# AlgoLab/PIntron

Measured on AMD Instinct MI355X. Metric: ESTs aligned/sec (whole node) + DP Mcells/s; bit-exact factorizations vs ref, higher is better.
Workload: dtype u8/int32

## Files before the change

### pintron_amd/estfact.py

```python
import ctypes as C
import os

ROOT = os.path.dirname(os.path.dirname(os.path.abspath(__file__)))
OUTPUT_FILES = ("raw-multifasta-out.txt", "processed-ests.txt", "megs.txt", "processed-megs.txt",
                "processed-megs-info.txt", "meg-edges.txt")


class KernelStat(C.Structure):
    _fields_ = [("name", C.c_char * 48), ("ms", C.c_double), ("launches", C.c_size_t),
                ("jobs", C.c_size_t), ("cells", C.c_ulonglong), ("algo_bytes", C.c_ulonglong)]


class SchedStats(C.Structure):
    _fields_ = [(n, C.c_size_t) for n in ("threads", "units", "aligned", "dp_batches", "dp_jobs",
                                          "pairing_batches", "pairing_requests")] + \
               [(n, C.c_double) for n in ("load_s", "index_s", "prefetch_s", "workers_s", "host_s",
                                          "pairing_s", "dp_s")] + \
               [("n_kernels", C.c_int), ("kernels", KernelStat * 64), ("dp_busy_union_ms", C.c_double),
                ("suspensions_per_unit", C.c_double)]


def load_host_lib(path=None):
    path = path or os.environ.get("PINTRON_ESTFACT_LIB") or os.path.join(ROOT, "pintron_amd", "lib", "libestfact.so")
    if not os.path.exists(path):
        raise RuntimeError("%s missing: run __graft_entry__.build() (there is no CPU fallback)" % path)
    L = C.CDLL(path)
    L.ef_session_open.restype = C.c_void_p
    L.ef_session_open.argtypes = [C.c_int, C.POINTER(C.c_char_p)]
    L.ef_session_step.argtypes = [C.c_void_p, C.POINTER(SchedStats)]
    L.ef_session_output.restype = C.c_void_p
    L.ef_session_output.argtypes = [C.c_void_p, C.c_int, C.POINTER(C.c_size_t)]
    L.ef_session_n_ests.restype = C.c_size_t
    L.ef_session_n_ests.argtypes = [C.c_void_p]
    L.ef_session_write_outputs.argtypes = [C.c_void_p]
    L.ef_session_close.argtypes = [C.c_void_p]
    return L


class Session:

    def __init__(self, L, directory):
        self.L, self.dir = L, directory
        cwd = os.getcwd()
        os.chdir(directory)
        try:
            argv = (C.c_char_p * 2)(b"est-fact", None)
            self.h = L.ef_session_open(1, argv)
        finally:
            os.chdir(cwd)
        if not self.h:
            raise RuntimeError("est-fact session could not start (no MI355X / libpintron_gpu.so?)")

    def step(self) -> SchedStats:
        st = SchedStats()
        if self.L.ef_session_step(self.h, C.byref(st)) != 0:
            raise RuntimeError("est-fact step failed")
        return st

    def n_ests(self) -> int:
        return int(self.L.ef_session_n_ests(self.h))

    def output(self, which: int) -> bytes:
        n = C.c_size_t()
        p = self.L.ef_session_output(self.h, which, C.byref(n))
        data = C.string_at(p, n.value)
        C.CDLL(None).free(C.c_void_p(p))
        return data

    def records(self) -> bytes:
        return self.output(0)

    def output_tensor(self, which: int):
        import torch
        n = C.c_size_t()
        p = self.L.ef_session_output(self.h, which, C.byref(n))
        try:
            if n.value == 0:
                return torch.empty(0, dtype=torch.uint8)
            view = (C.c_ubyte * n.value).from_address(p)
            return torch.frombuffer(view, dtype=torch.uint8).clone()
        finally:
            C.CDLL(None).free(C.c_void_p(p))

    def close(self):
        if self.h:
            self.L.ef_session_close(self.h)
            self.h = None


RECORDS = 6


def parse_factorization_records(data: bytes):
    import struct
    out, pos = [], 0
    while pos < len(data):
        est_index, n_fact = struct.unpack_from("<II", data, pos)
        pos += 8
        facts = []
        for _ in range(n_fact):
            polya, polyad, n_exons = struct.unpack_from("<BBH", data, pos)
            pos += 4
            exons = [struct.unpack_from("<4i", data, pos + 16 * k) for k in range(n_exons)]
            pos += 16 * n_exons
            facts.append((polya, polyad, exons))
        out.append((est_index, facts))
    return out


def format_raw_multifasta(records, processed_ests: bytes, genomic_seq: bytes) -> bytes:
    ests = []
    lines = processed_ests.split(b"\n")
    for k in range(0, len(lines) - 1, 2):
        ests.append((lines[k][1:], lines[k + 1]))
    out = []
    for (est_index, facts), (header, seq) in zip(records, ests):
        for polya, polyad, exons in facts:
            out.append(b">" + header + b"\n#polya=%d\n#polyad=%d\n" % (polya, polyad))
            for es, ee, gs, ge in exons:
                out.append(b"%d %d %d %d %s %s\n" % (es, ee, gs, ge, seq[es - 1:ee], genomic_seq[gs - 1:ge]))
    return b"".join(out)


def read_multifasta_records(path):
    recs, cur = [], []
    with open(path, "rb") as f:
        for line in f:
            if line.startswith(b">") and cur:
                recs.append(b"".join(cur))
                cur = []
            if line.strip() or cur:
                cur.append(line)
    if cur:
        recs.append(b"".join(cur))
    return recs


def partition(weights, world):
    total, n = sum(weights), len(weights)
    bounds, acc, i = [0], 0, 0
    for r in range(1, world):
        while i < n and acc * world < total * r:
            acc += weights[i]
            i += 1
        bounds.append(i)
    bounds.append(n)
    return [(bounds[r], bounds[r + 1]) for r in range(world)]


def gather_tensor(t, dist, rank, world, device):
    import torch
    n = torch.tensor([t.numel()], dtype=torch.int64, device=device)
    sizes = [torch.zeros_like(n) for _ in range(world)]
    dist.all_gather(sizes, n)
    sizes = [int(s.item()) for s in sizes]
    pad = torch.empty(max(max(sizes), 1), dtype=torch.uint8, device=device)
    pad[: t.numel()] = t.to(device)
    outl = [torch.empty_like(pad) for _ in range(world)] if rank == 0 else None
    dist.gather(pad, outl, dst=0)
    if rank != 0:
        return None
    return [o[: sizes[r]] for r, o in enumerate(outl)]


def gather_bytes(data: bytes, dist, rank, world, device):
    import torch
    t = torch.frombuffer(bytearray(data), dtype=torch.uint8) if data else torch.empty(0, dtype=torch.uint8)
    parts = gather_tensor(t, dist, rank, world, device)
    if parts is None:
        return None
    return [bytes(o.cpu().numpy().tobytes()) for o in parts]


def run_sharded(directory, workdir, dist, rank, world, device, L=None, files=(0, 1)):
    import shutil
    L = L or load_host_lib()
    recs = read_multifasta_records(os.path.join(directory, "ests.txt"))
    lo, hi = partition([len(r) for r in recs], world)[rank]
    os.makedirs(workdir, exist_ok=True)
    shutil.copy(os.path.join(directory, "genomic.txt"), os.path.join(workdir, "genomic.txt"))
    if os.path.exists(os.path.join(directory, "config.ini")):
        shutil.copy(os.path.join(directory, "config.ini"), os.path.join(workdir, "config.ini"))
    with open(os.path.join(workdir, "ests.txt"), "wb") as f:
        f.write(b"".join(recs[lo:hi]))
    texts = {k: b"" for k in files}
    stats = {"ests": 0, "aligned": 0, "dp_jobs": 0}
    error = None
    if hi > lo:
        try:
            sess = Session(L, workdir)
            try:
                st = sess.step()
                for k in files:
                    texts[k] = sess.output(k)
                stats = {"ests": hi - lo, "aligned": int(st.aligned), "dp_jobs": int(st.dp_jobs)}
            finally:
                sess.close()
        except Exception as e:
            error = e
    import torch
    ok = torch.tensor([0 if error else 1], dtype=torch.int32, device=device)
    dist.all_reduce(ok, op=dist.ReduceOp.MIN)
    if int(ok.item()) == 0:
        raise RuntimeError("est-fact failed on rank %d: %s" % (rank, error) if error
                           else "est-fact failed on another rank")
    for k in files:
        parts = gather_bytes(texts[k], dist, rank, world, device)
        if rank == 0:
            with open(os.path.join(directory, OUTPUT_FILES[k]), "wb") as f:
                f.write(b"".join(parts))
    return stats
```

### pintron_amd/host/ef_fact.c

```c
#include <math.h>
#include <stdlib.h>
#include <string.h>

#include "estfact.h"

typedef struct { int p, t, l; } ptl;

static size_t view_len(const char* s, int index, int length) {
  if (length <= 0) return 0;
  const char* z = (const char*)memchr(s + index, 0, (size_t)length);
  return z ? (size_t)(z - (s + index)) : (size_t)length;
}

char* ef_real_substring(int index, int length, const char* s) {
  if (index < 0) { length += index; index = 0; }
  if (length < 0) length = 0;
  char* r = (char*)malloc((size_t)length + 1);
  strncpy(r, s + index, (size_t)length);
  r[length] = '\0';
  return r;
}

static ef_factor* factor_new(int es, int ee, int gs, int ge) {
  ef_factor* f = (ef_factor*)malloc(sizeof(ef_factor));
  f->EST_start = es; f->EST_end = ee; f->GEN_start = gs; f->GEN_end = ge;
  return f;
}

void ef_factorization_free(void* fact) { efl_free((ef_list*)fact, free); }

void ef_est_free(ef_est* e) {
  if (!e) return;
  efl_free(e->factorizations, ef_factorization_free);
  efl_free(e->polyA_signals, NULL);
  efl_free(e->polyadenil_signals, NULL);
  free(e);
}

static void ahead_note(ef_ahead* ah, const ef_dp_req* q) {
  for (int k = 0; k < ah->n_pending; ++k) if (ef_req_same(&ah->q[ah->n + k], q)) return;
  if (ah->n + ah->n_pending < EF_AHEAD_MAX) ah->q[ah->n + ah->n_pending++] = *q;
}

int ef_dp_many_ahead(ef_backend* be, const ef_dp_req* reqs, ef_dp_res* res, size_t n) {
  ef_ahead* ah = be->ahead;
  enum { CAP = 32 };
  if (n > CAP) return ah->collecting ? EF_DP_PENDING : ef_backend_ask(be, reqs, res, n);
  size_t miss[CAP], nm = 0;
  for (size_t k = 0; k < n; ++k) {
    const int32_t* v = ef_ahead_find(ah, &reqs[k]);
    if (v) memcpy(res[k].v, v, sizeof res[k].v);
    else miss[nm++] = k;
  }
  if (ef_prof_on) { ef_prof.ahead_hits += n - nm; ef_prof.ahead_misses += ah->collecting ? 0 : nm; }
  if (nm == 0) return 0;
  if (ah->collecting) {
    for (size_t k = 0; k < nm; ++k) if (ef_req_keepable(&reqs[miss[k]])) ahead_note(ah, &reqs[miss[k]]);
    return EF_DP_PENDING;
  }
  if (nm == n) return ef_backend_ask(be, reqs, res, n);
  ef_dp_req mq[CAP]; ef_dp_res mr[CAP];
  for (size_t k = 0; k < nm; ++k) mq[k] = reqs[miss[k]];
  memset(mr, 0, nm * sizeof(ef_dp_res));
  const int rc = ef_backend_ask(be, mq, mr, nm);
  if (rc != 0) return rc;
  for (size_t k = 0; k < nm; ++k) res[miss[k]] = mr[k];
  return 0;
}

int ef_ahead_flush(ef_backend* be) {
  ef_ahead* ah = be->ahead;
  if (!ah || ah->n_pending == 0) return 0;
  const bool was = ah->collecting;
  ah->collecting = false;
  const int np = ah->n_pending;
  ef_dp_res r[EF_AHEAD_MAX];
  memset(r, 0, (size_t)np * sizeof(ef_dp_res));
  const int rc = ef_backend_ask(be, ah->q + ah->n, r, (size_t)np);
  if (rc == 0)
    for (int k = 0; k < np; ++k) ef_ahead_keep_next(ah, r[k].v);
  if (ef_prof_on) ef_prof.ahead_asked += (unsigned long long)np;
  ah->n_pending = 0;
  ah->collecting = was;
  return rc;
}

static int run_dp(ef_backend* be, int kind, const char* a, size_t la, const char* b, size_t lb,
                  uint32_t p0, uint32_t p1, uint32_t p2, uint32_t tail, bool temp, ef_dp_res* res) {
  ef_dp_req rq = { kind, a, la, b, lb, p0, p1, p2, tail, temp ? 1u : 0u };
  const int rc = ef_dp_one(be, &rq, res);
  if (rc != 0 && rc != EF_DP_PENDING) {
    fprintf(stderr, "* FATAL dynamic-programming backend failed (kind %d, %zu x %zu)\n", kind, la, lb);
    abort();
  }
  return rc;
}

uint32_t ef_edit_distance(ef_backend* be, const char* a, size_t la, const char* b, size_t lb) {
  ef_dp_res r;
  run_dp(be, EF_DP_ED, a, la, b, lb, 0, 0, 0, 0, true, &r);
  return (uint32_t)r.v[0];
}

uint32_t ef_compute_edit_distance(ef_backend* be, const char* a, size_t la, const char* b, size_t lb) {
  if (la == lb && strncmp(a, b, la) == 0) return 0;
  return ef_edit_distance(be, a, la, b, lb);
}

typedef struct { uint32_t n; ptl e[]; } emb;
static emb* emb_new(uint32_t n) { emb* x = (emb*)malloc(sizeof(emb) + (size_t)n * sizeof(ptl)); x->n = n; return x; }
static void embedding_free(void* e) { free(e); }

static emb* embedding_copy(const emb* e) {
  emb* c = emb_new(e->n);
  memcpy(c->e, e->e, (size_t)e->n * sizeof(ptl));
  return c;
}

static emb* update_embedding(const emb* embedding, const ef_pairing* node, const char* GEN,
                             const ef_config* cfg) {
  const ptl* head = &embedding->e[0];
  if (head->p == EF_SINK_START) {
    if (node->p < 0) return NULL;
    emb* e = emb_new(1);
    e->e[0].p = node->p; e->e[0].t = node->t; e->e[0].l = node->l;
    return e;
  }
  if (node->p < 0) return embedding_copy(embedding);
  const int small_delta = (head->p + head->l) - node->p;
  const int big_delta = (head->t + head->l) - node->t;
  const int min_fl = (int)cfg->min_factor_len;
  const int fl = 2 * min_fl;
  if (!(small_delta >= fl && big_delta >= fl)) return NULL;
  if (!(small_delta - (node->l + head->l) <= fl)) return NULL;
  if (!(small_delta - big_delta <= fl)) return NULL;
  int head_l, head_p, head_t, node_l;
  if (small_delta >= (node->l + head->l) && big_delta >= (node->l + head->l)) {
    head_p = head->p; head_t = head->t; head_l = head->l; node_l = node->l;
  } else {
    const int ref_delta = small_delta < big_delta ? small_delta : big_delta;
    int len_node = ref_delta / 2;
    int len_head = ref_delta - len_node;
    if (len_node > node->l) { len_node = node->l; len_head = ref_delta - len_node; }
    else if (len_head > head->l) { len_head = head->l; len_node = ref_delta - len_head; }
    head_l = len_head;
    head_p = head->p + head->l - head_l;
    head_t = head->t + head->l - head_l;
    node_l = len_node;
  }
  const bool overlap_on_p = small_delta < (node->l + head->l);
  const int gap_on_p = head_p - node->p - node_l - 1;
  const int gap_on_t = head_t - node->t - node_l - 1;
  const int intron_len = gap_on_t - (gap_on_p > 0 ? gap_on_p : 0);
  const bool intron_on_t = intron_len >= 0 && (cfg->min_intron_length == 0 || intron_len >= cfg->min_intron_length);
  if (overlap_on_p && intron_on_t) {
    int best_freq = -1, best_cut = 0;
    const int lo = (node->p + min_fl > head->p) ? node->p + min_fl : head->p;
    const int hi = (head->p + head->l - min_fl < node->p + node->l) ? head->p + head->l - min_fl : node->p + node->l;
    for (int cut = lo; cut <= hi; ++cut) {
      const int f = ef_burset_adaptor(GEN, (size_t)(cut - node->p + node->t), (size_t)(cut - head->p + head->t));
      if (f >= best_freq) { best_freq = f; best_cut = cut; }
    }
    const int dH = best_cut - head->p;
    head_l = head->l - dH; head_p = head->p + dH; head_t = head->t + dH;
    node_l = node->l - (node->p + node->l - best_cut);
  }
  if (!(gap_on_t <= fl || intron_on_t)) return NULL;
  emb* c = emb_new(embedding->n + 1);
  c->e[0].p = node->p; c->e[0].t = node->t; c->e[0].l = node_l;
  c->e[1].p = head_p; c->e[1].t = head_t; c->e[1].l = head_l;
  memcpy(c->e + 2, embedding->e + 1, (size_t)(embedding->n - 1) * sizeof(ptl));
  return c;
}

static bool pair_inside(const ptl* inner, const ptl* outer) {
  if (inner->p < outer->p || (inner->p + inner->l > outer->p + outer->l)) return false;
  if (inner->t < outer->t || (inner->t + inner->l > outer->t + outer->l)) return false;
  return true;
}

static int maximality_relation(const emb* add, const emb* cmp) {
  if (add->n > cmp->n) {
    bool check = true;
    for (uint32_t i = 0; i < cmp->n && check; ++i) check = pair_inside(&cmp->e[i], &add->e[i]);
    return check ? 2 : 1;
  }
  if (add->n < cmp->n) {
    bool check = true;
    for (uint32_t i = 0; i < add->n && check; ++i) check = pair_inside(&add->e[i], &cmp->e[i]);
    return check ? 0 : 1;
  }
  bool check = true;
  for (uint32_t i = 0; i < add->n && check; ++i) check = pair_inside(&add->e[i], &cmp->e[i]);
  if (check) return 0;
  check = true;
  for (uint32_t i = 0; i < add->n && check; ++i) check = pair_inside(&cmp->e[i], &add->e[i]);
  return check ? 2 : 1;
}

#define EF_WORK_PER_SECOND 1000000ull
typedef struct { unsigned long long used, limit; } ef_work;
static unsigned long long work_high_water;
unsigned long long ef_work_high_water(void) { return __atomic_load_n(&work_high_water, __ATOMIC_RELAXED); }
extern unsigned long long ef_work_budget_override;
static unsigned long long work_limit(const ef_config* cfg) {
  if (ef_work_budget_override) return ef_work_budget_override;
  return cfg->max_single_factorization_time ? (unsigned long long)cfg->max_single_factorization_time * EF_WORK_PER_SECOND : ~0ull;
}

static ef_list* subtree_embeddings(ef_pairing* root, const ef_config* cfg, const char* GEN, ef_work* wk) {
  if (root->emb_memo) return root->emb_memo;
  if (++wk->used > wk->limit) return NULL;
  ef_list* out = efl_new();
  root->visited = true;
  if (efl_empty(root->adjs)) {
    emb* e = emb_new(1);
    e->e[0].p = root->p; e->e[0].t = root->t; e->e[0].l = root->l;
    efl_push_front(out, e);
  } else {
    ef_iter ai = efl_begin(root->adjs);
    while (efi_has_next(&ai)) {
      ef_pairing* adj = (ef_pairing*)efi_next(&ai);
      ef_list* sub = subtree_embeddings(adj, cfg, GEN, wk);
      if (!sub) { efl_free(out, embedding_free); return NULL; }
      ef_iter si = efl_begin(sub);
      while (efi_has_next(&si)) {
        emb* add = update_embedding((const emb*)efi_next(&si), root, GEN, cfg);
        if (!add) continue;
        if (++wk->used > wk->limit) { embedding_free(add); efl_free(out, embedding_free); return NULL; }
        int is_max = 2;
        ef_iter ci = efl_begin(out);
        while (efi_has_next(&ci) && is_max >= 1) {
          const emb* cmp = (const emb*)efi_next(&ci);
          is_max = maximality_relation(add, cmp);
          if (is_max == 2) efi_remove(&ci, embedding_free);
        }
        if (is_max >= 1) efl_push_back(out, add); else embedding_free(add);
      }
    }
  }
  root->emb_memo = out;
  return out;
}

static ef_list* factorizations_from_embeddings(ef_list* embeddings, const ef_config* cfg) {
  ef_list* out = efl_new();
  const int fl = 2 * (int)cfg->min_factor_len;
  ef_iter ei = efl_begin(embeddings);
  while (efi_has_next(&ei)) {
    const emb* em = (const emb*)efi_next(&ei);
    ef_list* fact = efl_new();
    ef_factor* last = NULL;
    for (uint32_t q = 0; q < em->n; ++q) {
      const ptl* x = &em->e[q];
      if (efl_empty(fact) || (x->t - last->GEN_end - 1) > fl) {
        last = factor_new(x->p, x->p + x->l - 1, x->t, x->t + x->l - 1);
        efl_push_back(fact, last);
      } else {
        last = (ef_factor*)efl_tail(fact);
        last->EST_end = x->p + x->l - 1;
        last->GEN_end = x->t + x->l - 1;
      }
    }
    efl_push_back(out, fact);
  }
  return out;
}

static bool not_source_sink(ef_list* fact, int est_len) {
  if (efl_size(fact) > 1) return true;
  const ef_factor* h = (const ef_factor*)efl_head(fact);
  return !(h->EST_start < 0 || h->EST_start >= est_len);
}

static bool exon_start_end_ok(ef_list* fact) {
  int prev_e = -1, prev_g = -1;
  ef_iter it = efl_begin(fact);
  while (efi_has_next(&it)) {
    const ef_factor* x = (const ef_factor*)efi_next(&it);
    if (x->EST_start > x->EST_end || x->GEN_start > x->GEN_end) return false;
    if (x->EST_start < prev_e || x->GEN_start < prev_g) return false;
    prev_e = x->EST_end; prev_g = x->GEN_end;
  }
  return true;
}

static void endpoint_head_apply(ef_list* fact, ef_factor* head, const ef_dp_res* r) {
  const char* ea = r->s0; const char* ga = r->s1;
  const int dim = r->v[1];
  int j = 0, matches = 0, cut_factor = head->EST_start, cut_exon = head->GEN_start;
  bool stop = false;
  while (j < dim && !stop) {
    if (matches > 5) stop = true;
    else {
      if (ea[j] == ga[j]) { ++cut_factor; ++cut_exon; ++matches; }
      else { if (ea[j] != '-') ++cut_factor; if (ga[j] != '-') ++cut_exon; matches = 0; }
      ++j;
    }
  }
  if (!stop) free(efl_pop_front(fact));
  else { head->EST_start = cut_factor - matches; head->GEN_start = cut_exon - matches; }
}

static void endpoint_tail_apply(ef_list* fact, ef_factor* tail, const ef_dp_res* r) {
  char* ea = r->s0; char* ga = r->s1;
  const int dim = r->v[1];
  int j = dim - 1, matches = 0, cut_factor = tail->EST_end, cut_exon = tail->GEN_end;
  bool stop = false;
  while (j >= 0 && !stop) {
    if (matches > 10) stop = true;
    else {
      if (ea[j] == ga[j]) { --cut_factor; --cut_exon; ++matches; }
      else { if (ea[j] != '-') --cut_factor; if (ga[j] != '-') --cut_exon; matches = 0; }
      --j;
    }
  }
  int est_cleavage = cut_factor + matches, gen_cleavage = cut_exon + matches;
  int cursor = j + matches + 1;
  stop = false;
  while (((ea[cursor] == '-' || ga[cursor] == '-') && cursor < dim - 1) && !stop) {
    if (ea[cursor] == '-') {
      int tr = cursor + 1;
      while (ea[tr] == '-') ++tr;
      if (tr < dim && ea[tr] == ga[cursor]) { ea[cursor] = ea[tr]; ea[tr] = '-'; ++est_cleavage; ++gen_cleavage; }
      else stop = true;
    } else {
      int tr = cursor + 1;
      while (ga[tr] == '-') ++tr;
      if (tr < dim && ga[tr] == ea[cursor]) { ga[cursor] = ga[tr]; ga[tr] = '-'; ++est_cleavage; ++gen_cleavage; }
      else stop = true;
    }
    ++cursor;
  }
  if (gen_cleavage >= tail->GEN_start) { tail->EST_end = est_cleavage; tail->GEN_end = gen_cleavage; }
  else free(efl_pop_back(fact));
}

static void endpoint_request(ef_dp_req* q, const ef_factor* x, const char* gen, const char* est) {
  const ef_dp_req r = { EF_DP_ALIGN, est + x->EST_start, view_len(est, x->EST_start, x->EST_end - x->EST_start + 1),
                        gen + x->GEN_start, view_len(gen, x->GEN_start, x->GEN_end - x->GEN_start + 1), 0, 0, 0, 0, 0 };
  *q = r;
}
static void endpoint_release(ef_dp_req* q, ef_dp_res* r) {
  (void)q;
  ef_dp_res_release(r);
}

static unsigned max_edit_for_exon(size_t exon_length);
static bool exon_check_request(ef_dp_req* q, const ef_factor* x, const char* gen, const char* est, const ef_config* cfg) {
  if (x->GEN_start > x->GEN_end) return false;
  uint32_t w[2];
  memcpy(w, &cfg->complexity_threshold, 8);
  const ef_dp_req r = { EF_DP_KBAND, gen + x->GEN_start, view_len(gen, x->GEN_start, x->GEN_end - x->GEN_start + 1),
                        est + x->EST_start, view_len(est, x->EST_start, x->EST_end - x->EST_start + 1),
                        max_edit_for_exon((size_t)(x->GEN_end - x->GEN_start + 1)), w[0], w[1], 1, 0 };
  *q = r;
  return true;
}

static ef_list* handle_endpoints(ef_list* fact, const char* gen, const char* est, const ef_config* cfg, ef_backend* be) {
  ef_factor* head = (ef_factor*)efl_head(fact);
  ef_dp_req q[2]; ef_dp_res r[2];
  if (efl_size(fact) >= 2) {
    ef_factor* tail = (ef_factor*)efl_tail(fact);
    enum { INNER_MAX = 22 };
    ef_dp_req qq[2 + INNER_MAX]; ef_dp_res rr[2 + INNER_MAX]; size_t nq = 2;
    endpoint_request(&qq[0], head, gen, est);
    endpoint_request(&qq[1], tail, gen, est);
    if (be->ahead && ef_endpoint_checks) {
      uint32_t w[2];
      memcpy(w, &cfg->complexity_threshold, 8);
      qq[0].p0 = 1; qq[0].p1 = w[0]; qq[0].p2 = w[1];
      qq[1].p0 = 2; qq[1].p1 = w[0]; qq[1].p2 = w[1];
    }
    if (be->ahead && efl_size(fact) >= 3 && efl_size(fact) <= INNER_MAX) {
      ef_iter it = efl_begin(fact);
      efi_next(&it);
      while (efi_has_next(&it)) {
        const ef_factor* x = (const ef_factor*)efi_next(&it);
        if (x == tail) break;
        if (exon_check_request(&qq[nq], x, gen, est, cfg)) ++nq;
      }
    }
    if (ef_dp_many(be, qq, rr, nq) != 0) { fprintf(stderr, "* FATAL alignment backend failed\n"); abort(); }
    for (size_t k = 2; k < nq; ++k) ef_ahead_put(be->ahead, &qq[k], rr[k].v);
    if (be->ahead) {
      for (int k = 0; k < 2; ++k) {
        const int32_t* v = rr[k].v;
        if (!(v[4] & 8)) continue;
        const ef_factor* x = k == 0 ? head : tail;
        ef_factor y = *x;
        if (k == 0) { y.EST_start += v[2]; y.GEN_start += v[3]; }
        else { y.EST_end = y.EST_start + v[2] - 1; y.GEN_end = y.GEN_start + v[3] - 1; }
        ef_dp_req cq;
        if (y.EST_start > y.EST_end || !exon_check_request(&cq, &y, gen, est, cfg) || cq.p0 != ((uint32_t)v[4] >> 8)) continue;
        if (cq.la != (size_t)(y.GEN_end - y.GEN_start + 1) || cq.lb != (size_t)(y.EST_end - y.EST_start + 1)) continue;
        const int32_t answer[6] = { v[4] & 1, 0, (v[4] >> 1) & 3, 0, 0, 0 };
        ef_ahead_put(be->ahead, &cq, answer);
        if (ef_prof_on) ++ef_prof.ahead_asked;
      }
    }
    endpoint_head_apply(fact, head, &rr[0]);
    endpoint_tail_apply(fact, tail, &rr[1]);
    endpoint_release(&qq[0], &rr[0]); endpoint_release(&qq[1], &rr[1]);
    return fact;
  }
  endpoint_request(&q[0], head, gen, est);
  if (ef_dp_many(be, q, r, 1) != 0) { fprintf(stderr, "* FATAL alignment backend failed\n"); abort(); }
  endpoint_head_apply(fact, head, &r[0]);
  endpoint_release(&q[0], &r[0]);
  if (efl_empty(fact)) return fact;
  ef_factor* tail = (ef_factor*)efl_tail(fact);
  endpoint_request(&q[0], tail, gen, est);
  if (ef_dp_many(be, q, r, 1) != 0) { fprintf(stderr, "* FATAL alignment backend failed\n"); abort(); }
  endpoint_tail_apply(fact, tail, &r[0]);
  endpoint_release(&q[0], &r[0]);
  return fact;
}

static bool is_ch(char c, char up) { return c == up || c == (char)(up + 32); }

ef_list* ef_clean_external_exons(ef_list* fact, const char* gen, const char* est, ef_backend* be) {
  if (efl_empty(fact)) return fact;
  ef_factor* head = (ef_factor*)efl_pop_front(fact);
  const int hl = head->GEN_end - head->GEN_start + 1;
  bool ok = hl >= 10;
  if (ok && hl < 20) {
    if (!is_ch(gen[head->GEN_end + 1], 'G')) ok = false;
    else if (!is_ch(gen[head->GEN_end + 2], 'T') && !is_ch(gen[head->GEN_end + 2], 'C')) ok = false;
    else if (efl_size(fact) >= 1) {
      const ef_factor* nx = (const ef_factor*)efl_head(fact);
      if (!is_ch(gen[nx->GEN_start - 2], 'A')) ok = false;
      else if (!is_ch(gen[nx->GEN_start - 1], 'G')) ok = false;
    } else ok = false;
    if (ok) {
      char* g = ef_real_substring(head->GEN_start, head->GEN_end - head->GEN_start + 1, gen);
      char* e = ef_real_substring(head->EST_start, head->EST_end - head->EST_start + 1, est);
      if ((int)ef_edit_distance(be, g, strlen(g), e, strlen(e)) > 0) ok = false;
      free(g); free(e);
    }
  }
  if (ok) efl_push_front(fact, head); else free(head);
  if (efl_empty(fact)) return fact;
  ef_factor* tail = (ef_factor*)efl_pop_back(fact);
  const int tl = tail->GEN_end - tail->GEN_start + 1;
  ok = tl >= 10;
  if (ok && tl < 20) {
    if (!is_ch(gen[tail->GEN_start - 2], 'A')) ok = false;
    else if (!is_ch(gen[tail->GEN_start - 1], 'G')) ok = false;
    else if (efl_size(fact) >= 1) {
      const ef_factor* pv = (const ef_factor*)efl_tail(fact);
      if (!is_ch(gen[pv->GEN_end + 1], 'G')) ok = false;
      else if (!is_ch(gen[pv->GEN_end + 2], 'T') && !is_ch(gen[pv->GEN_end + 2], 'C')) ok = false;
    } else ok = false;
    if (ok) {
      char* g = ef_real_substring(tail->GEN_start, tail->GEN_end - tail->GEN_start + 1, gen);
      char* e = ef_real_substring(tail->EST_start, tail->EST_end - tail->EST_start + 1, est);
      if ((int)ef_edit_distance(be, g, strlen(g), e, strlen(e)) > 0) ok = false;
      free(g); free(e);
    }
  }
  if (ok) efl_push_back(fact, tail); else free(tail);
  return fact;
}

static ef_list* keep_best_run(ef_list* fact, const int* split_idx, int n_split) {
  if (n_split == 0) return fact;
  int best_l = -1, best_r = -1, best_cover = -1;
  ef_iter fi = efl_begin(fact);
  int left = 1;
  for (int k = 0; k < n_split; ++k) {
    const int right = split_idx[k];
    const ef_factor* le = (const ef_factor*)efi_next(&fi);
    const ef_factor* re = le;
    if (left < right) {
      for (int times = right - left - 1; times > 0; --times) re = (const ef_factor*)efi_next(&fi);
      const int cover = re->EST_end - le->EST_start + 1;
      if (cover > best_cover) { best_l = left; best_r = right - 1; best_cover = cover; }
      efi_next(&fi);
    }
    left = right + 1;
  }
  const int size = (int)efl_size(fact);
  if (left <= size) {
    const ef_factor* le = (const ef_factor*)efi_next(&fi);
    const ef_factor* re = le;
    for (int times = size - left; times > 0; --times) re = (const ef_factor*)efi_next(&fi);
    const int cover = re->EST_end - le->EST_start + 1;
    if (cover > best_cover) { best_l = left; best_r = size; best_cover = cover; }
  }
  if (best_l == -1 || best_r == -1) {
    for (int k = size; k > 0; --k) free(efl_pop_back(fact));
  } else {
    for (int k = best_l - 1; k > 0; --k) free(efl_pop_front(fact));
    for (int k = best_r + 1; k <= size; ++k) free(efl_pop_back(fact));
  }
  return fact;
}

static unsigned max_edit_for_exon(size_t exon_length) {
  const double rate = exon_length > 100 ? 0.030 : (exon_length > 50 ? 0.035 : 0.040);
  const double c = ceil(exon_length * rate);
  return (unsigned)(c > 1.0 ? c : 1.0);
}

ef_list* ef_clean_noisy_exons(ef_list* fact, const char* gen, const char* est, bool only_internals, ef_backend* be) {
  const size_t size = efl_size(fact);
  enum { SMALL = 24 };
  int idx_small[SMALL], slot_small[SMALL]; ef_dp_req rq_small[SMALL]; ef_dp_res rs_small[SMALL];
  const bool small = size < SMALL;
  int* idx = small ? idx_small : (int*)malloc((size + 1) * sizeof(int));
  ef_dp_req* rq = small ? rq_small : (ef_dp_req*)malloc((size + 1) * sizeof(ef_dp_req));
  ef_dp_res* rs = small ? rs_small : (ef_dp_res*)malloc((size + 1) * sizeof(ef_dp_res));
  int* slot = small ? slot_small : (int*)malloc((size + 1) * sizeof(int));
  size_t nrq = 0, nvis = 0;
  int index = only_internals ? 2 : 1;
  const int first_index = index;
  const int last = only_internals ? (int)(size - 1) : (int)size;
  ef_iter it = efl_begin(fact);
  if (only_internals) efi_next(&it);
  while (efi_has_next(&it) && index <= last) {
    const ef_factor* x = (const ef_factor*)efi_next(&it);
    const unsigned max_err = max_edit_for_exon((size_t)(x->GEN_end - x->GEN_start + 1));
    slot[nvis] = -1;
    if (x->GEN_start <= x->GEN_end) {
      const ef_dp_req q = { EF_DP_KBAND, gen + x->GEN_start, view_len(gen, x->GEN_start, x->GEN_end - x->GEN_start + 1),
                            est + x->EST_start, view_len(est, x->EST_start, x->EST_end - x->EST_start + 1), max_err, 0, 0, 0, 0 };
      slot[nvis] = (int)nrq;
      rq[nrq++] = q;
    }
    ++nvis; ++index;
  }
  if (ef_dp_many(be, rq, rs, nrq) != 0) { fprintf(stderr, "* FATAL dynamic-programming backend failed (K-band)\n"); abort(); }
  int n = 0;
  for (size_t v = 0; v < nvis; ++v) {
    const bool ok = slot[v] >= 0 && rs[slot[v]].v[0] != 0;
    if (!ok) idx[n++] = first_index + (int)v;
  }
  fact = keep_best_run(fact, idx, n);
  if (!small) { free(idx); free(rq); free(rs); free(slot); }
  return fact;
}

static bool est_coverage_ok(ef_list* fact, const char* est) {
  const size_t len = strlen(est);
  const ef_factor* h = (const ef_factor*)efl_head(fact);
  const ef_factor* t = (const ef_factor*)efl_tail(fact);
  const double cov = (double)(t->EST_end - h->EST_start + 1) / (double)len;
  return cov >= 0.35f;
}

static int relaxed_factor_compare(const ef_factor* p1, const ef_factor* p2, int cfr_type, int allowed, ef_list* l1) {
  if (p1->GEN_start < p2->GEN_start && p1->GEN_end < p2->GEN_start) return 1;
  if (p2->GEN_start < p1->GEN_start && p2->GEN_end < p1->GEN_start) return 1;
  const int max_unconf = 20;
  if (cfr_type == 0) {
    if (abs(p1->GEN_end - p2->GEN_end) <= allowed && abs(p1->GEN_start - p2->GEN_start) <= allowed) return 0;
  }
  if (abs(cfr_type) == 2) {
    if (abs(p1->GEN_end - p2->GEN_end) <= allowed) {
      if (cfr_type == 2) {
        if (p1->GEN_start - p2->GEN_start > max_unconf) return 1;
        if (p1->GEN_start - p2->GEN_start > 0) {
          int tot = 0; bool stop = false;
          ef_iter it = efl_begin(l1);
          while (efi_has_next(&it) && !stop) {
            const ef_factor* f = (const ef_factor*)efi_next(&it);
            if (p1->GEN_start == f->GEN_start) stop = true; else tot += f->GEN_end - f->GEN_start + 1;
          }
          if (abs(p1->GEN_start - p2->GEN_start - tot) < 10) return 1;
        }
      }
      return 0;
    }
  }
  if (abs(cfr_type) == 1) {
    if (abs(p1->GEN_start - p2->GEN_start) <= allowed) {
      if (cfr_type == 1) {
        if (p2->GEN_end - p1->GEN_end > max_unconf) return 1;
        if (p2->GEN_end - p1->GEN_end > 0) {
          int tot = 0; bool stop = false;
          ef_iter it = efl_end(l1);
          while (efi_has_prev(&it) && !stop) {
            const ef_factor* f = (const ef_factor*)efi_prev(&it);
            if (p1->GEN_start == f->GEN_start) stop = true; else tot += f->GEN_end - f->GEN_start + 1;
          }
          if (abs(p2->GEN_end - p1->GEN_end - tot) < 20) return 1;
        }
      }
      return 0;
    }
  }
  return 1;
}

static int relaxed_list_compare(ef_list* l1, ef_list* l2, int allowed_diff) {
  if (efl_size(l1) != efl_size(l2) || efl_size(l1) == 1) return 0;
  ef_iter i1 = efl_begin(l1), i2 = efl_begin(l2);
  const int actual = allowed_diff == -1 ? 0 : allowed_diff;
  int count = 1;
  while (efi_has_next(&i1) && efi_has_next(&i2)) {
    const int type = allowed_diff == -1 ? 0 : (count == 1 ? -2 : (count == (int)efl_size(l1) ? -1 : 0));
    if (relaxed_factor_compare((const ef_factor*)i1.next->el, (const ef_factor*)i2.next->el, type, actual, l1) != 0) return 0;
    efi_next(&i1); efi_next(&i2);
    ++count;
  }
  return -2;
}

static int relaxed_list_contained(ef_list* l1, ef_list* l2, int allowed_diff) {
  if (efl_size(l1) == efl_size(l2)) return relaxed_list_compare(l1, l2, allowed_diff);
  if (efl_size(l1) == 1 || efl_size(l2) == 1) return 0;
  const int actual = allowed_diff == -1 ? 0 : allowed_diff;
  ef_iter i1 = efl_begin(l1), i2 = efl_begin(l2);
  bool found = false;
  int type = allowed_diff == -1 ? 0 : -2;
  unsigned count_long = 1;
  const bool l1_longer = efl_size(l1) > efl_size(l2);
  ef_list* lng = l1_longer ? l1 : l2;
  ef_iter* il = l1_longer ? &i1 : &i2;
  ef_iter* is = l1_longer ? &i2 : &i1;
  while (efi_has_next(il) && !found) {
    if (relaxed_factor_compare((const ef_factor*)il->next->el, (const ef_factor*)is->next->el, type, actual, lng) == 0) { found = true; efi_next(is); }
    else ++count_long;
    efi_next(il);
    if (type == -2) type = 2;
  }
  if (!found) return 0;
  unsigned count_factors = 1;
  bool stop = false;
  const size_t short_size = l1_longer ? efl_size(l2) : efl_size(l1);
  const size_t long_size = l1_longer ? efl_size(l1) : efl_size(l2);
  while (efi_has_next(&i1) && efi_has_next(&i2) && !stop) {
    type = allowed_diff == -1 ? 0 : ((count_factors + 1 == short_size) ? ((count_long + 1 == long_size) ? -1 : 1) : 0);
    if (relaxed_factor_compare((const ef_factor*)il->next->el, (const ef_factor*)is->next->el, type, actual, lng) == 0) { efi_next(&i1); efi_next(&i2); }
    else stop = true;
    ++count_factors; ++count_long;
  }
  if (stop) return 0;
  if (efl_size(l1) >= efl_size(l2)) return count_factors == efl_size(l2) ? 1 : 0;
  return count_factors == efl_size(l1) ? -1 : 0;
}

ef_list* ef_add_if_not_exists(ef_list* to_add, ef_list* list, const ef_config* cfg, bool* added) {
  ef_iter ci = efl_begin(list);
  bool found = false;
  while (efi_has_next(&ci) && !found) {
    ef_list* cmp = (ef_list*)efi_next(&ci);
    int res = 0;
    if (efl_size(cmp) == efl_size(to_add) && efl_size(cmp) == 1) {
      const ef_factor* h1 = (const ef_factor*)efl_head(to_add); const ef_factor* h2 = (const ef_factor*)efl_head(cmp);
      if (h1->GEN_start == h2->GEN_start && h1->GEN_end == h2->GEN_end) res = -2;
      else if (h1->GEN_start >= h2->GEN_start && h1->GEN_end <= h2->GEN_end) res = -1;
      else if (h1->GEN_start <= h2->GEN_start && h1->GEN_end >= h2->GEN_end) res = 1;
    } else {
      res = relaxed_list_contained(to_add, cmp, (int)cfg->max_site_difference);
    }
    if (res < 0) {
      if (res == -2) {
        const ef_factor* h1 = (const ef_factor*)efl_head(to_add); ef_factor* h2 = (ef_factor*)efl_head(cmp);
        if (h1->EST_start < h2->EST_start) { h2->EST_start = h1->EST_start; h2->GEN_start = h1->GEN_start; }
        const ef_factor* t1 = (const ef_factor*)efl_tail(to_add); ef_factor* t2 = (ef_factor*)efl_tail(cmp);
        if (t1->EST_end > t2->EST_end) { t2->EST_end = t1->EST_end; t2->GEN_end = t1->GEN_end; }
      }
      found = true;
    } else if (res == 1) {
      efi_remove(&ci, ef_factorization_free);
    }
  }
  if (!found) efl_push_back(list, to_add);
  *added = !found;
  return list;
}

static double coverage_of(ef_list* fact, unsigned length) {
  const ef_factor* h = (const ef_factor*)efl_head(fact); const ef_factor* t = (const ef_factor*)efl_tail(fact);
  const int cover = (int)length - (h->EST_start + ((int)length - t->EST_end - 1));
  return ((double)cover) / (double)length;
}

static int gap_length_of(ef_list* fact) {
  if (efl_size(fact) == 1) return 0;
  int g = 0;
  ef_iter it = efl_begin(fact);
  const ef_factor* d = (const ef_factor*)efi_next(&it);
  while (efi_has_next(&it)) { const ef_factor* a = (const ef_factor*)efi_next(&it); g += a->EST_start - d->EST_end - 1; d = a; }
  return g;
}

static bool check_gap_errors(ef_list* fact, const char* est, const char* gen, const ef_config* cfg, ef_backend* be) {
  (void)cfg;
  const unsigned threshold_ed = 20;
  unsigned tot = 0;
  bool ok = true;
  ef_iter it = efl_begin(fact);
  ef_factor* d = (ef_factor*)efi_next(&it);
  while (efi_has_next(&it) && ok) {
    ef_factor* a = (ef_factor*)efi_next(&it);
    const size_t gapP = (size_t)(a->EST_start - d->EST_end - 1);
    if (gapP > 0) {
      const size_t gapT = (size_t)(a->GEN_start - d->GEN_end - 1);
      const int max_errs = (int)gapP;
      char *pc = NULL, *tc = NULL;
      const char* p = est + d->EST_end + 1;
      const char* t = gen + d->GEN_end + 1;
      if (d->EST_end + 1 < 0 || view_len(est, d->EST_end + 1, (int)gapP) != gapP) p = pc = ef_real_substring(d->EST_end + 1, (int)gapP, est);
      if (d->GEN_end + 1 < 0 || (int)gapT < 0 || (size_t)(d->GEN_end + 1) + gapT > ef_genomic_len(gen)) t = tc = ef_real_substring(d->GEN_end + 1, (int)gapT, gen);
      ef_dp_res r;
      const int asked = run_dp(be, EF_DP_BORDERS, p, gapP, t, gapT, 0, (uint32_t)gapP, (uint32_t)max_errs, 0, pc || tc, &r);
      free(pc); free(tc);
      if (asked == EF_DP_PENDING) { d = a; continue; }
      if (ef_collecting(be)) { d = a; continue; }
      ok = r.v[0] != 0;
      if (ok) {
        tot += (unsigned)r.v[4];
        d->EST_end += r.v[1];
        a->EST_start = d->EST_end + 1;
        d->GEN_end += r.v[2];
        a->GEN_start -= (int)gapT - r.v[3];
      }
    }
    d = a;
  }
  if (ef_collecting(be)) return true;
  if (ok && tot > threshold_ed) ok = false;
  if (ok) {
    it = efl_begin(fact);
    d = (ef_factor*)efi_next(&it);
    while (efi_has_next(&it)) {
      ef_factor* a = (ef_factor*)efi_next(&it);
      if (a->GEN_start - d->GEN_end - 1 <= 3) { d->EST_end = a->EST_end; d->GEN_end = a->GEN_end; efi_remove(&it, free); }
      else d = a;
    }
  }
  return ok;
}

static void correct_tail(ef_list* fact, const char* gen, const char* est) {
  ef_factor* tail = (ef_factor*)efl_tail(fact);
  size_t i = (size_t)(tail->EST_end + 1), j = (size_t)(tail->GEN_end + 1);
  const size_t el = strlen(est), gl = ef_genomic_len(gen);
  while (i < el && j < gl && gen[j] == est[i]) { ++i; ++j; }
  tail->EST_end = (int)i - 1; tail->GEN_end = (int)j - 1;
}

static bool detect_polyA(ef_list* fact, const char* gen, const char* est, bool* polyadenil) {
  const ef_factor* tail = (const ef_factor*)efl_tail(fact);
  const size_t el = strlen(est);
  const char* cl = est + tail->EST_end + 1;
  const int cll = (tail->EST_end + 1 <= (int)el) ? (int)(el - (size_t)tail->EST_end - 1) : 0;
  int i = 0, matches = 0;
  bool stop = false;
  while (i < cll && !stop) {
    if (cl[i] == 'a' || cl[i] == 'A') { if (matches >= 8) stop = true; else { ++matches; ++i; } }
    else { if (matches >= 8) stop = true; else i = cll; }
  }
  *polyadenil = false;
  if (stop) {
    i = tail->GEN_end - 39 > 0 ? tail->GEN_end - 39 : 0;
    while (i <= tail->GEN_end && !*polyadenil) {
      if (gen[i] == 'a' || gen[i] == 'A') {
        char pas[8];
        const size_t pl = view_len(gen, i, 6);
        memcpy(pas, gen + i, pl); pas[pl] = '\0';
        if (!strcmp(pas, "aataaa") || !strcmp(pas, "AATAAA") || !strcmp(pas, "attaaa") || !strcmp(pas, "ATTAAA")) *polyadenil = true;
      }
      ++i;
    }
    i = tail->GEN_end - 9 > 0 ? tail->GEN_end - 9 : 0;
    matches = 0;
    while (i <= tail->GEN_end + 10 && stop && gen[i] != '\0') {
      if (matches >= 6) stop = false;
      else { if (gen[i] == 'a' || gen[i] == 'A') ++matches; else matches = 0; ++i; }
    }
    if (stop) {
      i = tail->GEN_end + 1;
      int count = 0;
      while (i <= tail->GEN_end + 10 && stop && gen[i] != '\0') {
        if (count >= 7) stop = false;
        else { if (gen[i] == 'a' || gen[i] == 'A') ++count; ++i; }
      }
    }
  }
  return stop;
}

static ef_list* clean_complexity_and_noise(ef_list* fact, const char* gen, const char* est, const ef_config* cfg, ef_backend* be) {
  const size_t size = efl_size(fact);
  enum { SMALL = 24 };
  const ef_factor* x_small[SMALL]; int slot_small[SMALL], idx_small[SMALL]; ef_dp_req rq_small[SMALL]; ef_dp_res rs_small[SMALL];
  const bool small = size < SMALL;
  const ef_factor** xs = small ? x_small : (const ef_factor**)malloc((size + 1) * sizeof(ef_factor*));
  int* slot = small ? slot_small : (int*)malloc((size + 1) * sizeof(int));
  int* idx = small ? idx_small : (int*)malloc((size + 1) * sizeof(int));
  ef_dp_req* rq = small ? rq_small : (ef_dp_req*)malloc((size + 1) * sizeof(ef_dp_req));
  ef_dp_res* rs = small ? rs_small : (ef_dp_res*)malloc((size + 1) * sizeof(ef_dp_res));
  size_t nx = 0, nrq = 0;
  ef_iter it = efl_begin(fact);
  while (efi_has_next(&it)) {
    const ef_factor* x = (const ef_factor*)efi_next(&it);
    xs[nx] = x;
    slot[nx] = exon_check_request(&rq[nrq], x, gen, est, cfg) ? (int)nrq++ : -1;
    ++nx;
  }
  if (ef_dp_many(be, rq, rs, nrq) != 0) { fprintf(stderr, "* FATAL dynamic-programming backend failed (exon checks)\n"); abort(); }
  int n = 0;
  for (size_t v = 0; v < nx; ++v) if (slot[v] >= 0 && rs[slot[v]].v[2] != 0) idx[n++] = (int)v + 1;
  fact = keep_best_run(fact, idx, n);
  if (!efl_empty(fact)) {
    ef_phase(EFP_NOISY);
    n = 0;
    int index = 1;
    size_t v = 0;
    it = efl_begin(fact);
    while (efi_has_next(&it)) {
      const ef_factor* x = (const ef_factor*)efi_next(&it);
      while (v < nx && xs[v] != x) ++v;
      const bool ok = v < nx && slot[v] >= 0 && rs[slot[v]].v[0] != 0;
      if (!ok) idx[n++] = index;
      ++index;
    }
    fact = keep_best_run(fact, idx, n);
  }
  if (!small) { free(xs); free(slot); free(idx); free(rq); free(rs); }
  return fact;
}

static ef_list* clean_candidates(ef_list* cands, ef_list* flist, unsigned est_len, const char* GEN, const char* EST,
                                 const ef_config* cfg, ef_backend* be) {
  ef_iter ci = efl_begin(cands);
  while (efi_has_next(&ci)) {
    ef_list* f = (ef_list*)efi_next(&ci);
    bool ok = not_source_sink(f, (int)est_len);
    if (ok) ok = exon_start_end_ok(f);
    if (ok) { ef_phase(EFP_ENDPOINTS); f = handle_endpoints(f, GEN, EST, cfg, be); if (efl_empty(f)) ok = false; }
    if (ok) { ef_phase(EFP_EXTERNAL); f = ef_clean_external_exons(f, GEN, EST, be); if (efl_empty(f)) ok = false; }
    if (ok) { ef_phase(EFP_DUST); f = clean_complexity_and_noise(f, GEN, EST, cfg, be); if (efl_empty(f)) ok = false; }
    ef_phase(EFP_ADD);
    if (ok) ok = est_coverage_ok(f, EST);
    if (ok) {
      bool added;
      flist = ef_add_if_not_exists(f, flist, cfg, &added);
      if (!added) ef_factorization_free(f);
    } else {
      ef_factorization_free(f);
    }
  }
  efl_free(cands, NULL);
  return flist;
}

static bool chain_embedding(const void* rec, const ef_config* cfg, const char* GEN, ef_work* wk, emb** out) {
  const uint32_t* head = (const uint32_t*)rec;
  const uint32_t nv = head[0];
  if (nv < 2 || nv > 64) return false;
  const int32_t* vt = (const int32_t*)((const char*)rec + 16);
  const uint16_t* first = (const uint16_t*)((const char*)rec + 16 + 12 * (size_t)nv);
  const uint8_t* tgt = (const uint8_t*)rec + 16 + 12 * (size_t)nv + 2 * ((size_t)nv + 1);
  if (vt[0] != EF_SOURCE_START) return false;
  uint8_t path[64];
  uint64_t seen = 0;
  uint32_t k = 0, n = 0;
  for (;;) {
    if (seen >> k & 1u) return false;
    seen |= 1ull << k; path[n++] = (uint8_t)k;
    const uint32_t deg = (uint32_t)first[k + 1] - first[k];
    if (deg == 0) break;
    if (deg != 1) return false;
    k = tgt[first[k]];
    if (k >= nv) return false;
  }
  if (n != nv || vt[3 * (size_t)path[n - 1]] != EF_SINK_START) return false;
  wk->used += nv;
  ef_pairing node;
  memset(&node, 0, sizeof node);
  emb* e = emb_new(1);
  { const int32_t* s3 = vt + 3 * (size_t)path[n - 1]; e->e[0].p = s3[0]; e->e[0].t = s3[1]; e->e[0].l = s3[2]; }
  for (uint32_t q = n - 1; q-- > 0 && e;) {
    const int32_t* v3 = vt + 3 * (size_t)path[q];
    node.p = v3[0]; node.t = v3[1]; node.l = v3[2];
    emb* nx = update_embedding(e, &node, GEN, cfg);
    embedding_free(e);
    e = nx;
    if (e) ++wk->used;
  }
  *out = e;
  return true;
}

unsigned ef_chain_candidate(const void* rec, const ef_config* cfg, const char* GEN, ef_factor* out_exons, size_t cap,
                            unsigned* n_exons, unsigned* n_pairs, unsigned* work) {
  *n_exons = 0; *n_pairs = 0; *work = 0;
  if (((const uint32_t*)rec)[2] & 3u) return 0;
  ef_work wk = { 0, ~0ull };
  emb* chain = NULL;
  if (!chain_embedding(rec, cfg, GEN, &wk, &chain)) return 1;
  *work = (unsigned)wk.used;
  if (!chain) return 2;
  *n_pairs = chain->n;
  ef_list* embs = efl_new();
  efl_push_back(embs, chain);
  ef_list* cands = factorizations_from_embeddings(embs, cfg);
  efl_free(embs, embedding_free);
  ef_list* fact = (ef_list*)efl_head(cands);
  ef_iter it = efl_begin(fact);
  while (efi_has_next(&it)) {
    const ef_factor* x = (const ef_factor*)efi_next(&it);
    if (*n_exons < cap) out_exons[*n_exons] = *x;
    ++*n_exons;
  }
  ef_factorization_free(fact);
  efl_free(cands, NULL);
  return 3;
}

static ef_list* filter_and_refine(ef_list* flist, unsigned est_len, const ef_seq* est_info, const ef_seq* gen_info,
                                  const ef_config* cfg, ef_backend* be) {
  const char* GEN = gen_info->seq;
  const char* EST = est_info->seq;
  ef_phase(EFP_FILTERS);
  {
    const size_t nf = efl_size(flist);
    double cov_small[32];
    double* cov = nf < 32 ? cov_small : (double*)malloc((nf + 1) * sizeof(double));
    double max_cov = 0.0;
    size_t k = 0;
    ef_iter it = efl_begin(flist);
    while (efi_has_next(&it)) {
      ef_list* f = (ef_list*)efi_next(&it);
      bool src_sink = false;
      if (efl_size(f) == 1) {
        const ef_factor* h = (const ef_factor*)efl_head(f);
        if (h->EST_start < 0 || h->EST_start >= (int)est_len) { cov[k] = -1.0; src_sink = true; }
      }
      if (!src_sink) { cov[k] = coverage_of(f, est_len); if (max_cov < cov[k]) max_cov = cov[k]; }
      ++k;
    }
    k = 0;
    it = efl_begin(flist);
    const int slen = (int)strlen(EST);
    while (efi_has_next(&it)) {
      efi_next(&it);
      const double c = cov[k++];
      if (c == -1.0 || max_cov - c > cfg->max_coverage_diff) efi_remove(&it, ef_factorization_free);
      else if ((max_cov - c) * slen > 100) efi_remove(&it, ef_factorization_free);
    }
    if (cov != cov_small) free(cov);
  }
  {
    const size_t nf = efl_size(flist);
    int gl_small[32];
    int* gl = nf < 32 ? gl_small : (int*)malloc((nf + 1) * sizeof(int));
    int min_gl = -1;
    size_t k = 0;
    ef_iter it = efl_begin(flist);
    while (efi_has_next(&it)) {
      gl[k] = gap_length_of((ef_list*)efi_next(&it));
      if (min_gl == -1 || min_gl > gl[k]) min_gl = gl[k];
      ++k;
    }
    k = 0;
    it = efl_begin(flist);
    while (efi_has_next(&it)) {
      efi_next(&it);
      const int g = gl[k++];
      if (cfg->max_gapLength_diff != -1 && g - min_gl > cfg->max_gapLength_diff) efi_remove(&it, ef_factorization_free);
    }
    if (gl != gl_small) free(gl);
  }
  ef_phase(EFP_GAPERR);
  if (be->ahead) {
    ef_ahead_collect(be, true);
    ef_iter it = efl_begin(flist);
    while (efi_has_next(&it)) check_gap_errors((ef_list*)efi_next(&it), EST, GEN, cfg, be);
    ef_ahead_collect(be, false);
    if (ef_ahead_flush(be) != 0) { fprintf(stderr, "* FATAL dynamic-programming backend failed\n"); abort(); }
  }
  {
    ef_iter it = efl_begin(flist);
    while (efi_has_next(&it)) {
      ef_list* f = (ef_list*)efi_next(&it);
      if (!check_gap_errors(f, EST, GEN, cfg, be)) efi_remove(&it, ef_factorization_free);
    }
  }
  if (cfg->max_number_of_factorizations != 0 && (int)efl_size(flist) > cfg->max_number_of_factorizations) {
    efl_free(flist, ef_factorization_free);
    flist = efl_new();
  }
  ef_phase(EFP_INTRON);
  {
    enum { GAP_AHEAD_MAX = 24 };
    ef_gap_ahead* pre = NULL; size_t n_pre = 0;
    if (be->ahead && be->dp_many) {
      size_t total = 0;
      ef_iter it = efl_begin(flist);
      while (efi_has_next(&it)) { const size_t k = efl_size((ef_list*)efi_next(&it)); total += k ? k - 1 : 0; }
      if (total >= 2 && total <= GAP_AHEAD_MAX) {
        pre = (ef_gap_ahead*)malloc(total * sizeof(ef_gap_ahead));
        ef_dp_req rq[GAP_AHEAD_MAX]; ef_dp_res rs[GAP_AHEAD_MAX];
        it = efl_begin(flist);
        while (efi_has_next(&it)) {
          ef_list* f = (ef_list*)efi_next(&it);
          if (efl_empty(f)) continue;
          ef_iter fi = efl_begin(f);
          const ef_factor* donor = (const ef_factor*)efi_next(&fi);
          while (efi_has_next(&fi)) {
            const ef_factor* acc = (const ef_factor*)efi_next(&fi);
            ef_gap_window_build(cfg, gen_info, est_info, donor, acc, &pre[n_pre].w);
            pre[n_pre].donor = *donor; pre[n_pre].acceptor = *acc;
            const ef_dp_req q = { EF_DP_GAP, pre[n_pre].w.seq_est, pre[n_pre].w.le, pre[n_pre].w.seq_gen, pre[n_pre].w.lg, 0, 0, 0, 0, 1 };
            rq[n_pre++] = q;
            donor = acc;
          }
        }
        memset(rs, 0, n_pre * sizeof(ef_dp_res));
        if (be->dp_many(be->self, rq, rs, n_pre) != 0) { fprintf(stderr, "* FATAL gap alignment backend failed\n"); abort(); }
        for (size_t k = 0; k < n_pre; ++k) pre[k].res = rs[k];
        if (ef_prof_on) ef_prof.ahead_asked += n_pre;
      }
    }
    size_t at = 0;
    ef_iter it = efl_begin(flist);
    while (efi_has_next(&it)) {
      ef_list* f = (ef_list*)efi_next(&it);
      if (efl_empty(f)) continue;
      ef_iter fi = efl_begin(f);
      ef_factor* donor = (ef_factor*)efi_next(&fi);
      bool first = true;
      while (efi_has_next(&fi)) {
        ef_factor* acc = (ef_factor*)efi_next(&fi);
        ef_refine_intron(cfg, gen_info, est_info, donor, acc, first, be, pre && at < n_pre ? &pre[at] : NULL);
        ++at;
        first = false;
        donor = acc;
      }
      fi = efl_begin(f);
      const ef_factor* e1 = (const ef_factor*)efi_next(&fi);
      if (efi_has_next(&fi)) {
        const ef_factor* e2 = (const ef_factor*)efi_next(&fi);
        if (e1->EST_start == e2->EST_start) free(efl_pop_front(f));
      }
    }
    for (size_t k = 0; k < n_pre; ++k) { ef_gap_window_release(&pre[k].w); ef_dp_res_release(&pre[k].res); }
    free(pre);
  }
  return flist;
}

unsigned ef_chain_factorization(const void* rec, const ef_config* cfg, const char* EST, const char* GEN, ef_backend* be,
                                ef_factor* out_exons, size_t cap, unsigned* n_exons) {
  *n_exons = 0;
  if (((const uint32_t*)rec)[2] & 3u) return 0;
  ef_work wk = { 0, ~0ull };
  emb* chain = NULL;
  if (!chain_embedding(rec, cfg, GEN, &wk, &chain)) return 0;
  if (!chain) return 1;
  ef_seq est_info, gen_info;
  memset(&est_info, 0, sizeof est_info); memset(&gen_info, 0, sizeof gen_info);
  est_info.seq = est_info.original_seq = (char*)EST;
  gen_info.seq = gen_info.original_seq = (char*)GEN;
  const unsigned est_len = (unsigned)strlen(EST);
  ef_list* embs = efl_new();
  efl_push_back(embs, chain);
  ef_list* cands = factorizations_from_embeddings(embs, cfg);
  efl_free(embs, embedding_free);
  ef_list* flist = clean_candidates(cands, efl_new(), est_len, GEN, EST, cfg, be);
  flist = filter_and_refine(flist, est_len, &est_info, &gen_info, cfg, be);
  unsigned outcome = 1;
  if (!efl_empty(flist)) {
    outcome = 2;
    ef_iter it = efl_begin((ef_list*)efl_head(flist));
    while (efi_has_next(&it)) {
      const ef_factor* x = (const ef_factor*)efi_next(&it);
      if (*n_exons < cap) out_exons[*n_exons] = *x;
      ++*n_exons;
    }
  }
  efl_free(flist, ef_factorization_free);
  return outcome;
}

ef_est* ef_get_est_factorizations(const ef_seq* est_info, ef_meg* V, const ef_config* cfg,
                                  const ef_seq* gen_info, ef_backend* be) {
  ef_phase(EFP_EMBED);
  ef_est* est = (ef_est*)calloc(1, sizeof(ef_est));
  est->info = est_info;
  const char* GEN = gen_info->seq;
  const char* EST = est_info->seq;
  const unsigned est_len = (unsigned)V->n - 2;
  ef_list* flist = efl_new();
  ef_work wk = { 0, work_limit(cfg) };
  emb* chain = NULL;
  if (V->rec && !V->v && ef_chain_fast_path && chain_embedding(V->rec, cfg, GEN, &wk, &chain)) {
    if (ef_prof_on) ++ef_prof.chain_graphs;
    if (wk.used > wk.limit) {
      if (chain) embedding_free(chain);
      efl_free(flist, ef_factorization_free);
      free(est);
      return NULL;
    }
    if (chain) {
      ef_list* embs = efl_new();
      efl_push_back(embs, chain);
      ef_list* cands = factorizations_from_embeddings(embs, cfg);
      efl_free(embs, embedding_free);
      flist = clean_candidates(cands, flist, est_len, GEN, EST, cfg, be);
    }
  } else {
  if (ef_prof_on) ++ef_prof.other_graphs;
  V = ef_meg_lists(V);
  EF_MEG_FOR_POS(V, i, 0, V->n) {
    ef_iter it = efl_begin(V->v[i]);
    while (efi_has_next(&it)) { ef_pairing* p = (ef_pairing*)efi_next(&it); p->visited = false; p->emb_memo = NULL; }
  }
  EF_MEG_FOR_POS(V, i, 0, V->n) {
    ef_iter it = efl_begin(V->v[i]);
    while (efi_has_next(&it)) {
      ef_pairing* root = (ef_pairing*)efi_next(&it);
      if (root->visited) continue;
      ef_phase(EFP_EMBED);
      ef_list* embs = subtree_embeddings(root, cfg, GEN, &wk);
      if (!embs) {
        EF_MEG_FOR_POS(V, j, 0, V->n) {
          ef_iter jt = efl_begin(V->v[j]);
          while (efi_has_next(&jt)) { ef_pairing* q = (ef_pairing*)efi_next(&jt); if (q->emb_memo) { efl_free(q->emb_memo, embedding_free); q->emb_memo = NULL; } }
        }
        efl_free(flist, ef_factorization_free);
        free(est);
        return NULL;
      }
      flist = clean_candidates(factorizations_from_embeddings(embs, cfg), flist, est_len, GEN, EST, cfg, be);
    }
  }
  EF_MEG_FOR_POS(V, i, 0, V->n) {
    ef_iter it = efl_begin(V->v[i]);
    while (efi_has_next(&it)) { ef_pairing* p = (ef_pairing*)efi_next(&it); if (p->emb_memo) { efl_free(p->emb_memo, embedding_free); p->emb_memo = NULL; } }
  }
  }
  {
    unsigned long long hw = __atomic_load_n(&work_high_water, __ATOMIC_RELAXED);
    while (wk.used > hw && !__atomic_compare_exchange_n(&work_high_water, &hw, wk.used, true, __ATOMIC_RELAXED, __ATOMIC_RELAXED)) { }
  }

  flist = filter_and_refine(flist, est_len, est_info, gen_info, cfg, be);
  ef_phase(EFP_TAIL);
  est->polyA_signals = efl_new();
  est->polyadenil_signals = efl_new();
  {
    ef_iter it = efl_begin(flist);
    while (efi_has_next(&it)) {
      ef_list* f = (ef_list*)efi_next(&it);
      correct_tail(f, GEN, est_info->original_seq);
      bool polyadenil = false;
      const bool polyA = detect_polyA(f, GEN, est_info->original_seq, &polyadenil);
      efl_push_back(est->polyA_signals, polyA ? (void*)1 : (void*)2);
      efl_push_back(est->polyadenil_signals, polyadenil ? (void*)1 : (void*)2);
    }
  }
  est->factorizations = flist;
  return est;
}
```

### pintron_amd/host/ef_sched.c

```c
#define _GNU_SOURCE
#include <malloc.h>
#include <pthread.h>
#include <sys/uio.h>
#include <errno.h>
#include <sys/prctl.h>
#include <sys/syscall.h>
#include <linux/futex.h>
#include <sys/resource.h>
#include <sched.h>
#include <dirent.h>
#include <time.h>
#include <stdlib.h>
#include <string.h>
#include <stdint.h>
#include <ucontext.h>
#include <sys/mman.h>

#if defined(__x86_64__) && !defined(EF_USE_UCONTEXT)
typedef struct { void* sp; } ef_ctx;
void ef_ctx_switch(void** save_sp, void* new_sp);
void ef_ctx_entry(void);
__asm__(
  ".text\n"
  ".globl ef_ctx_switch\n.type ef_ctx_switch,@function\n"
  "ef_ctx_switch:\n"
  "  pushq %rbp\n  pushq %rbx\n  pushq %r12\n  pushq %r13\n  pushq %r14\n  pushq %r15\n"
  "  movq %rsp, (%rdi)\n  movq %rsi, %rsp\n"
  "  popq %r15\n  popq %r14\n  popq %r13\n  popq %r12\n  popq %rbx\n  popq %rbp\n"
  "  ret\n"
  ".size ef_ctx_switch,.-ef_ctx_switch\n"
  ".globl ef_ctx_entry\n.type ef_ctx_entry,@function\n"
  "ef_ctx_entry:\n"
  "  movq %r12, %rdi\n  callq *%r13\n  ud2\n"
  ".size ef_ctx_entry,.-ef_ctx_entry\n");
static inline void ctx_switch(ef_ctx* from, ef_ctx* to) { ef_ctx_switch(&from->sp, to->sp); }
static void ctx_make(ef_ctx* c, char* stack, size_t size, void (*fn)(void*), void* arg) {
  uintptr_t top = ((uintptr_t)stack + size) & ~(uintptr_t)15;
  void** S = (void**)(top - 16);
  S[-1] = (void*)ef_ctx_entry;
  S[-2] = NULL;
  S[-3] = NULL;
  S[-4] = arg;
  S[-5] = (void*)fn;
  S[-6] = NULL;
  S[-7] = NULL;
  c->sp = (void*)(S - 7);
}
#else
typedef struct { ucontext_t uc; } ef_ctx;
static inline void ctx_switch(ef_ctx* from, ef_ctx* to) { swapcontext(&from->uc, &to->uc); }
static void ctx_tramp(unsigned fh, unsigned fl, unsigned ah, unsigned al) {
  void (*fn)(void*) = (void (*)(void*))(((uintptr_t)fh << 32) | (uintptr_t)fl);
  fn((void*)(((uintptr_t)ah << 32) | (uintptr_t)al));
}
static void ctx_make(ef_ctx* c, char* stack, size_t size, void (*fn)(void*), void* arg) {
  getcontext(&c->uc);
  c->uc.uc_stack.ss_sp = stack; c->uc.uc_stack.ss_size = size; c->uc.uc_link = NULL;
  const uintptr_t f = (uintptr_t)fn, a = (uintptr_t)arg;
  makecontext(&c->uc, (void (*)(void))ctx_tramp, 4, (unsigned)(f >> 32), (unsigned)(f & 0xffffffffu), (unsigned)(a >> 32), (unsigned)(a & 0xffffffffu));
}
#endif
#if defined(__SANITIZE_THREAD__)
void* __tsan_get_current_fiber(void);
void* __tsan_create_fiber(unsigned flags);
void __tsan_destroy_fiber(void* fiber);
void __tsan_switch_to_fiber(void* fiber, unsigned flags);
#define EF_TSAN 1
#else
#define EF_TSAN 0
#endif
#include <unistd.h>

#include "estfact.h"
#include "ef_gpu.h"
#include "ef_sched.h"

enum { F_RUNNABLE, F_WAIT_DP, F_WAIT_PAIR, F_DONE };

#if EF_TSAN
static inline void tsan_to(void* fiber) { __tsan_switch_to_fiber(fiber, 0); }
#else
static inline void tsan_to(void* fiber) { (void)fiber; }
#endif

static double now_s(void) { struct timespec ts; clock_gettime(CLOCK_MONOTONIC, &ts); return ts.tv_sec + 1e-9 * ts.tv_nsec; }

struct worker;
#define EF_N_OUT 7

typedef struct fiber {
  ef_ctx ctx;
  void* tsan;
  char* stack; bool guarded;
  struct worker* w;
  int state;
  size_t unit;
  size_t cur_entry;
  int lane;
  int phase;
  const ef_dp_req* reqs; ef_dp_res* ress; size_t nreq;
  ef_dp_req req1; int rc;
  const char* pat; size_t pat_len; unsigned pat_L; double pat_rate; ef_triple** pat_out; size_t* pat_n;
  ef_backend be;
  struct fiber* pool_next;
  ef_sink out[EF_N_OUT];
} fiber;

static const char FIBER_SENTINEL[16] = "pintron-fibre-s";

static inline void fiber_prefetch(const fiber* f) {
#if defined(__x86_64__) && !defined(EF_USE_UCONTEXT)
  const char* sp = (const char*)f->ctx.sp;
  for (int k = 0; k < 12; ++k) __builtin_prefetch(sp + 64 * k, 0, 3);
#endif
  __builtin_prefetch(f->ress, 0, 3);
  __builtin_prefetch(f->reqs, 0, 3);
}

#define EF_GUARD_BYTES 4096u
static char* stack_alloc(size_t size, bool* guarded) {
  void* m = mmap(NULL, size + EF_GUARD_BYTES, PROT_READ | PROT_WRITE, MAP_PRIVATE | MAP_ANONYMOUS | MAP_STACK, -1, 0);
  if (m != MAP_FAILED && mprotect(m, EF_GUARD_BYTES, PROT_NONE) == 0) { *guarded = true; return (char*)m + EF_GUARD_BYTES; }
  if (m != MAP_FAILED) munmap(m, size + EF_GUARD_BYTES);
  *guarded = false;
  return (char*)malloc(size);
}
static void stack_free(char* stack, size_t size, bool guarded) {
  if (!stack) return;
  if (guarded) munmap(stack - EF_GUARD_BYTES, size + EF_GUARD_BYTES); else free(stack);
}

typedef struct {
  size_t first; bool has_sibling;
  char* buf[EF_N_OUT]; size_t len[EF_N_OUT];
} unit;

typedef struct merged_batch {
  pgpu_dp_result* results; char* strings;
  int refs;
} merged_batch;

typedef struct dp_request {
  const pgpu_dp_job* jobs; size_t n; const char* arena; size_t arena_len;
  merged_batch* batch; size_t base;
  int rc;
  uint32_t done;
  uint32_t* wake;
  struct dp_request* next;
} dp_request;

static inline void request_publish(dp_request* rq) {
  uint32_t* wake = rq->wake;
  __atomic_store_n(&rq->done, 1u, __ATOMIC_RELEASE);
  __atomic_add_fetch(wake, 1u, __ATOMIC_RELEASE);
  syscall(SYS_futex, wake, FUTEX_WAKE_PRIVATE, 1, NULL, NULL, 0);
}
static inline void worker_sleep(uint32_t* wake, uint32_t seen) {
  syscall(SYS_futex, wake, FUTEX_WAIT_PRIVATE, seen, NULL, NULL, 0);
}

#define MAX_SERVICES 8
#define EF_MAX_WORKERS 256
typedef struct service_thread {
  pthread_t thread;
  struct service* sv;
  pgpu_ctx* ctx;
  ef_sched_stats stats;
  double* iv; size_t n_iv, cap_iv;
  double phase_s[6];
} service_thread;

typedef struct service {
  pthread_mutex_t mu;
  pthread_cond_t posted, finished;
  dp_request *head, *tail;
  bool stop;
  struct shared* sh;
  int n_threads;
  long coalesce_us;
  service_thread threads[MAX_SERVICES];
} service;

#define PRE_CHUNKS 16
typedef struct shared {
  ef_inputs* in;
  pgpu_index* idx;
  unit* units; size_t n_units; size_t units_cap;
  size_t next_unit;
  pthread_mutex_t mu;
  size_t max_fibers, stack_size;
  int n_pre;
  size_t pre_lo[PRE_CHUNKS + 1];
  pgpu_pairing* pre_tri[PRE_CHUNKS]; uint64_t* pre_first[PRE_CHUNKS];
  bool use_meg;
  pgpu_meg_params meg_prm;
  unsigned char* pre_meg[PRE_CHUNKS]; size_t pre_meg_cap[PRE_CHUNKS]; uint64_t* pre_meg_first[PRE_CHUNKS];
  unsigned char* pre_slab; size_t pre_slab_cap, pre_slab_used;
  bool pre_own[PRE_CHUNKS], pre_first_own[PRE_CHUNKS];
  char* up_stage; size_t up_stage_cap;
  size_t ready_entries;
  pthread_cond_t ready_cv;
  bool kernel_timing;
  size_t gen_len;
  int n_lanes;
  service svc;
  int failed;
  ef_sched_stats stats;
  fiber* fiber_pool;
  fiber* worker_pool[EF_MAX_WORKERS];
  struct out_chunk* chunks;
  struct out_chunk* spare_chunks;
  unsigned long long prof_cyc[EFP_N], prof_susp[EFP_N], prof_jobs[EFP_N];
  unsigned long long prof_ahead[5];
  double prof_t0; double prof_sleep_bins[64];
} shared;

typedef struct out_chunk { struct out_chunk* next; size_t cap, used; char data[]; } out_chunk;

#define MAX_LANES 16
typedef struct lane {
  fiber** fibers; size_t n_fibers;
  ef_jobbuf jb;
  dp_request rq; bool posted;
  fiber** inflight; size_t n_inflight;
} lane;

typedef struct worker {
  shared* sh;
  size_t index;
  double sleep_bins[64];
  size_t suspensions;
  ef_ctx sched;
  void* tsan_sched;
  fiber* free_fibers;
  out_chunk* chunk;
  lane lanes[MAX_LANES];
  uint32_t wake;
  pgpu_ctx* ctx;
  size_t held_unit; bool holding;
  ef_sched_stats stats;
} worker;

static void kstat_add(ef_sched_stats* st, const ef_kernel_stat* k) {
  for (int i = 0; i < st->n_kernels; ++i)
    if (!strcmp(st->kernels[i].name, k->name)) {
      st->kernels[i].ms += k->ms; st->kernels[i].launches += k->launches; st->kernels[i].jobs += k->jobs;
      st->kernels[i].cells += k->cells; st->kernels[i].algo_bytes += k->algo_bytes;
      return;
    }
  if (st->n_kernels < EF_MAX_KERNELS) st->kernels[st->n_kernels++] = *k;
}

static int fiber_dp_many(void* self, const ef_dp_req* reqs, ef_dp_res* res, size_t n) {
  fiber* f = (fiber*)self;
  if (n == 0) return 0;
  f->reqs = reqs; f->ress = res; f->nreq = n; f->state = F_WAIT_DP;
  ++f->w->suspensions;
  if (ef_prof_on) { ef_prof.susp[f->phase]++; ef_prof.jobs[f->phase] += n; }
  if (EF_TSAN) tsan_to(f->w->tsan_sched);
  ctx_switch(&f->ctx, &f->w->sched);
  return f->rc;
}

static int fiber_dp(void* self, const ef_dp_req* q, ef_dp_res* res) {
  fiber* f = (fiber*)self;
  f->req1 = *q;
  return fiber_dp_many(self, &f->req1, res, 1);
}

static int fiber_pairings(void* self, const char* pattern, size_t m, unsigned L, double rate, ef_triple** out, size_t* n) {
  fiber* f = (fiber*)self;
  const shared* sh = f->w->sh;
  int c = 0;
  if (sh->n_pre) while (f->cur_entry >= sh->pre_lo[c + 1]) ++c;
  if (sh->n_pre && sh->pre_tri[c] && L == sh->in->cfg.min_factor_len && rate == sh->in->cfg.min_string_depth_rate &&
      pattern == sh->in->list[f->cur_entry]->seq) {
    const size_t e = f->cur_entry - sh->pre_lo[c];
    const uint64_t a = sh->pre_first[c][e], b = sh->pre_first[c][e + 1];
    ef_triple* t = (ef_triple*)malloc((size_t)(b - a + 1) * sizeof(ef_triple));
    memcpy(t, sh->pre_tri[c] + a, (size_t)(b - a) * sizeof(ef_triple));
    *out = t; *n = (size_t)(b - a);
    return 0;
  }
  f->pat = pattern; f->pat_len = m; f->pat_L = L; f->pat_rate = rate; f->pat_out = out; f->pat_n = n;
  f->state = F_WAIT_PAIR;
  if (EF_TSAN) tsan_to(f->w->tsan_sched);
  ctx_switch(&f->ctx, &f->w->sched);
  return f->rc;
}

static const void* fiber_meg(void* self, const char* pattern, size_t m, const ef_config* cfg) {
  (void)m;
  fiber* f = (fiber*)self;
  const shared* sh = f->w->sh;
  if (!sh->use_meg || !sh->n_pre || cfg->min_factor_len != sh->in->cfg.min_factor_len ||
      cfg->min_string_depth_rate != sh->in->cfg.min_string_depth_rate || pattern != sh->in->list[f->cur_entry]->seq)
    return NULL;
  int c = 0;
  while (f->cur_entry >= sh->pre_lo[c + 1]) ++c;
  if (!sh->pre_meg[c]) return NULL;
  return sh->pre_meg[c] + sh->pre_meg_first[c][f->cur_entry - sh->pre_lo[c]];
}

static char* out_alloc(worker* w, size_t n) {
  out_chunk* c = w->chunk;
  if (!c || c->used + n > c->cap) {
    const size_t cap = n > (1u << 20) ? n : (1u << 20);
    shared* sh = w->sh;
    c = NULL;
    pthread_mutex_lock(&sh->mu);
    if (sh->spare_chunks && sh->spare_chunks->cap >= n) { c = sh->spare_chunks; sh->spare_chunks = c->next; }
    pthread_mutex_unlock(&sh->mu);
    if (!c) { c = (out_chunk*)malloc(sizeof(out_chunk) + cap); c->cap = cap; }
    c->used = 0;
    pthread_mutex_lock(&sh->mu);
    c->next = sh->chunks; sh->chunks = c;
    pthread_mutex_unlock(&sh->mu);
    w->chunk = c;
  }
  char* r = c->data + c->used;
  c->used += n;
  return r;
}

static void fiber_main(void* arg) {
  fiber* f = (fiber*)arg;
  shared* sh = f->w->sh;
  unit* u = &sh->units[f->unit];
  ef_sink* fs = f->out;
  for (int k = 0; k < EF_N_OUT; ++k) { fs[k].f = NULL; fs[k].len = 0; }
  ef_side_files side = { &fs[2], &fs[3], &fs[4], &fs[5] };
  const ef_inputs* in = sh->in;
  for (size_t k = u->first; k <= u->first + (u->has_sibling ? 1 : 0); ++k) {
    f->cur_entry = k;
    ef_est* fe = ef_compute_est_fact(in->gen, in->list[k], &f->be, &in->cfg, &side);
    const bool aligned = !efl_empty(fe->factorizations);
    ef_phase(EFP_OUTPUT);
    if (aligned) {
      ef_write_multifasta_output(in->gen, fe, &fs[0], in->cfg.retain_externals);
      ef_write_factorization_records(in->gen, fe, &fs[6], in->cfg.retain_externals, (uint32_t)f->unit);
      ef_write_single_est_info(&fs[1], fe->info);
    }
    ef_phase(EFP_FREE);
    ef_est_free(fe);
    ef_phase(EFP_OTHER);
    if (aligned) break;
  }
  ef_phase(EFP_OUTPUT);
  for (int k = 0; k < EF_N_OUT; ++k) {
    u->len[k] = fs[k].len;
    u->buf[k] = fs[k].len ? out_alloc(f->w, fs[k].len) : NULL;
    if (fs[k].len) memcpy(u->buf[k], fs[k].mem, fs[k].len);
  }
  f->state = F_DONE;
  if (EF_TSAN) tsan_to(f->w->tsan_sched);
  ctx_switch(&f->ctx, &f->w->sched);
}

static inline bool unit_ready(const shared* sh, size_t u) {
  if (!sh->n_pre) return true;
  const size_t last = sh->units[u].first + (sh->units[u].has_sibling ? 1 : 0);
  return last < __atomic_load_n(&sh->ready_entries, __ATOMIC_ACQUIRE);
}
static void wait_unit_ready(shared* sh, size_t u) {
  const size_t last = sh->units[u].first + (sh->units[u].has_sibling ? 1 : 0);
  const int was = ef_phase(EFP_WAIT_PREFETCH);
  pthread_mutex_lock(&sh->mu);
  while (last >= sh->ready_entries && !sh->failed) pthread_cond_wait(&sh->ready_cv, &sh->mu);
  pthread_mutex_unlock(&sh->mu);
  ef_phase(was);
}
static inline bool worker_has_work(const worker* w) {
  for (int k = 0; k < w->sh->n_lanes; ++k) if (w->lanes[k].n_fibers > 0 || w->lanes[k].posted) return true;
  return false;
}

enum { START_NONE = 0, START_OK = 1, START_LATER = 2 };
static int start_fiber(worker* w, int li) {
  shared* sh = w->sh;
  lane* ln = &w->lanes[li];
  fiber* f = w->free_fibers;
  size_t u;
  if (w->holding) u = w->held_unit;
  else {
    u = __atomic_fetch_add(&sh->next_unit, 1, __ATOMIC_RELAXED);
    if (u >= sh->n_units) return START_NONE;
  }
  if (!unit_ready(sh, u)) {
    if (worker_has_work(w)) { w->held_unit = u; w->holding = true; return START_LATER; }
    wait_unit_ready(sh, u);
  }
  w->holding = false;
  if (__atomic_load_n(&sh->failed, __ATOMIC_RELAXED)) return START_NONE;
  if (f) w->free_fibers = f->pool_next;
  else if (__atomic_load_n(&sh->fiber_pool, __ATOMIC_RELAXED)) {
    pthread_mutex_lock(&sh->mu);
    if (sh->fiber_pool) {
      f = sh->fiber_pool;
      fiber* last = f;
      for (int k = 0; k < 32 && last->pool_next; ++k) last = last->pool_next;
      sh->fiber_pool = last->pool_next;
      last->pool_next = NULL;
      w->free_fibers = f->pool_next; f->pool_next = NULL;
    }
    pthread_mutex_unlock(&sh->mu);
  }
  if (f) {
    char* st = f->stack;
    const bool gd = f->guarded;
    void* ts = f->tsan;
    ef_sink keep[EF_N_OUT];
    memcpy(keep, f->out, sizeof keep);
    memset(f, 0, sizeof(fiber));
    f->stack = st; f->guarded = gd; f->tsan = ts;
    memcpy(f->out, keep, sizeof keep);
  }
  else { f = (fiber*)calloc(1, sizeof(fiber)); f->stack = stack_alloc(sh->stack_size, &f->guarded); }
  f->w = w; f->unit = u; f->state = F_RUNNABLE; f->lane = li;
  f->be.self = f; f->be.pairings = fiber_pairings; f->be.dp = fiber_dp; f->be.dp_many = fiber_dp_many; f->be.meg = fiber_meg;
  memcpy(f->stack, FIBER_SENTINEL, sizeof FIBER_SENTINEL);
#if EF_TSAN
  if (f->tsan) __tsan_destroy_fiber(f->tsan);
  f->tsan = __tsan_create_fiber(0);
  w->tsan_sched = __tsan_get_current_fiber();
#endif
  ctx_make(&f->ctx, f->stack, sh->stack_size, fiber_main, f);
  ln->fibers[ln->n_fibers++] = f;
  return START_OK;
}

static int submit_pairings(worker* w, lane* ln) {
  fiber** wait = (fiber**)malloc((ln->n_fibers + 1) * sizeof(fiber*));
  size_t nw = 0;
  for (size_t i = 0; i < ln->n_fibers; ++i) if (ln->fibers[i]->state == F_WAIT_PAIR) wait[nw++] = ln->fibers[i];
  int rc = 0;
  while (nw > 0 && rc == 0) {
    const unsigned L = wait[0]->pat_L; const double rate = wait[0]->pat_rate;
    size_t ng = 0, total = 0;
    for (size_t i = 0; i < nw; ++i) if (wait[i]->pat_L == L && wait[i]->pat_rate == rate) { ++ng; total += wait[i]->pat_len; }
    char* blob = (char*)malloc(total + 1);
    uint64_t* off = (uint64_t*)malloc((ng + 1) * sizeof(uint64_t));
    fiber** grp = (fiber**)malloc(ng * sizeof(fiber*));
    size_t g = 0, pos = 0, rest = 0;
    for (size_t i = 0; i < nw; ++i) {
      fiber* f = wait[i];
      if (f->pat_L == L && f->pat_rate == rate) { off[g] = pos; memcpy(blob + pos, f->pat, f->pat_len); pos += f->pat_len; grp[g++] = f; }
      else wait[rest++] = f;
    }
    off[ng] = pos;
    pgpu_pairing_plan* plan = NULL;
    pgpu_pairing_params prm = { L, 0, rate };
    if (!w->ctx && pgpu_init(ef_gpu_device_from_env(), &w->ctx) != PGPU_OK) { free(blob); free(off); free(grp); free(wait); return 1; }
    rc = pgpu_pairing_plan_create(w->ctx, w->sh->idx, blob, off, ng, &plan);
    if (rc == PGPU_OK) rc = pgpu_pairing_plan_run(w->ctx, plan, &prm);
    if (rc == PGPU_OK) {
      const size_t cnt = (size_t)pgpu_pairing_plan_count(plan);
      pgpu_pairing* out = (pgpu_pairing*)malloc((cnt + 1) * sizeof(pgpu_pairing));
      uint64_t* first = (uint64_t*)malloc((ng + 1) * sizeof(uint64_t));
      rc = pgpu_pairing_plan_fetch(w->ctx, plan, out, cnt, first);
      if (rc == PGPU_OK) {
        for (size_t i = 0; i < ng; ++i) {
          const size_t n = (size_t)(first[i + 1] - first[i]);
          ef_triple* t = (ef_triple*)malloc((n + 1) * sizeof(ef_triple));
          memcpy(t, out + first[i], n * sizeof(ef_triple));
          *grp[i]->pat_out = t; *grp[i]->pat_n = n;
          grp[i]->rc = 0; grp[i]->state = F_RUNNABLE;
        }
        w->stats.pairing_batches++; w->stats.pairing_requests += ng;
      }
      free(out); free(first);
    }
    if (plan) pgpu_pairing_plan_destroy(w->ctx, plan);
    if (rc != PGPU_OK) fprintf(stderr, "* FATAL pairing batch failed: %s\n", pgpu_last_error(w->ctx));
    free(blob); free(off); free(grp);
    nw = rest;
  }
  free(wait);
  return rc;
}

static void kstat_add(ef_sched_stats* st, const ef_kernel_stat* k);

static void* service_main(void* arg) {
  pthread_setname_np(pthread_self(), "ef-gpu-service");
  prctl(PR_SET_TIMERSLACK, 1000UL, 0, 0, 0);
  service_thread* me = (service_thread*)arg;
  service* sv = me->sv;
  shared* sh = sv->sh;
  pgpu_dp_part* parts = NULL; size_t parts_cap = 0;
  for (;;) {
    pthread_mutex_lock(&sv->mu);
    const double t_idle = now_s();
    while (!sv->head && !sv->stop) pthread_cond_wait(&sv->posted, &sv->mu);
    me->phase_s[0] += now_s() - t_idle;
    if (sv->coalesce_us > 0 && sv->head && !sv->stop) {
      pthread_mutex_unlock(&sv->mu);
      struct timespec ts = { 0, sv->coalesce_us * 1000L };
      nanosleep(&ts, NULL);
      pthread_mutex_lock(&sv->mu);
    }
    dp_request* list = sv->head;
    sv->head = sv->tail = NULL;
    const bool stop = sv->stop;
    pthread_mutex_unlock(&sv->mu);
    if (!list) { if (stop) break; else continue; }
    size_t nj = 0; int nreq = 0;
    for (dp_request* r = list; r; r = r->next) ++nreq;
    if ((size_t)nreq > parts_cap) { parts_cap = (size_t)nreq * 2; parts = (pgpu_dp_part*)realloc(parts, parts_cap * sizeof(pgpu_dp_part)); }
    {
      size_t q = 0;
      for (dp_request* r = list; r; r = r->next, ++q) {
        r->base = nj;
        parts[q].jobs = r->jobs; parts[q].n_jobs = r->n; parts[q].arena = r->arena; parts[q].arena_len = r->arena_len;
        nj += r->n;
      }
    }
    merged_batch* mb = (merged_batch*)calloc(1, sizeof(merged_batch));
    mb->refs = nreq;
    mb->results = (pgpu_dp_result*)malloc((nj + 1) * sizeof(pgpu_dp_result));
    pgpu_dp_plan* plan = NULL;
    const double t_a = now_s();
    me->phase_s[1] += t_a - t_idle - 0;
    pgpu_range_push("dp batch (create, launch, sync, fetch)");
    int rc = pgpu_dp_plan_create_parts(me->ctx, sh->idx, parts, (size_t)nreq, &plan);
    const double t_b = now_s();
    if (rc == PGPU_OK) rc = pgpu_dp_plan_launch(me->ctx, plan);
    const double t_c = now_s();
    if (rc == PGPU_OK) rc = pgpu_dp_plan_sync(me->ctx, plan);
    const double t_d = now_s();
    me->phase_s[2] += t_b - t_a; me->phase_s[3] += t_c - t_b; me->phase_s[4] += t_d - t_c;
    if (rc == PGPU_OK) {
      const size_t sb = pgpu_dp_plan_string_bytes(plan);
      mb->strings = (char*)malloc(sb + 16);
      rc = pgpu_dp_plan_fetch(me->ctx, plan, mb->results, mb->strings, sb + 16);
    }
    if (rc == PGPU_OK && sh->kernel_timing) {
      const int ng = pgpu_dp_plan_n_groups(plan);
      for (int g = 0; g < ng; ++g) {
        pgpu_group_info gi;
        if (pgpu_dp_plan_group_info(plan, g, &gi) != PGPU_OK || gi.jobs == 0) continue;
        ef_kernel_stat ks; memset(&ks, 0, sizeof ks);
        snprintf(ks.name, sizeof ks.name, "%s", gi.name);
        ks.ms = gi.ms; ks.launches = 1; ks.jobs = gi.jobs; ks.cells = gi.cells; ks.algo_bytes = gi.algo_bytes;
        kstat_add(&me->stats, &ks);
        if (gi.t0_ms >= 0 && gi.ms > 0) {
          if (me->n_iv + 2 > me->cap_iv) { me->cap_iv = me->cap_iv ? me->cap_iv * 2 : 4096; me->iv = (double*)realloc(me->iv, me->cap_iv * sizeof(double)); }
          me->iv[me->n_iv++] = gi.t0_ms; me->iv[me->n_iv++] = gi.t0_ms + gi.ms;
        }
      }
    }
    if (plan) pgpu_dp_plan_destroy(me->ctx, plan);
    pgpu_range_pop();
    me->phase_s[5] += now_s() - t_d;
    if (rc != PGPU_OK) fprintf(stderr, "* FATAL DP batch failed: %s\n", pgpu_last_error(me->ctx));
    me->stats.dp_batches++; me->stats.dp_jobs += nj;
    for (dp_request* r = list; r;) { dp_request* nx = r->next; r->batch = mb; r->rc = rc; request_publish(r); r = nx; }
  }
  free(parts);
  return NULL;
}

static int launch_dp(worker* w, lane* ln) {
  shared* sh = w->sh;
  service* sv = &sh->svc;
  const char* gen = sh->in->gen->seq;
  ef_jobbuf_reset(&ln->jb);
  ln->n_inflight = 0;
  for (size_t i = 0; i < ln->n_fibers; ++i) {
    fiber* f = ln->fibers[i];
    if (f->state != F_WAIT_DP) continue;
    for (size_t k = 0; k < f->nreq; ++k) ef_jobbuf_add(&ln->jb, &f->reqs[k], gen, sh->gen_len);
    ln->inflight[ln->n_inflight++] = f;
  }
  if (ln->n_inflight == 0) return 0;
  dp_request* rq = &ln->rq;
  memset(rq, 0, sizeof *rq);
  rq->wake = &w->wake;
  rq->jobs = ln->jb.jobs; rq->n = ln->jb.n; rq->arena = ln->jb.arena; rq->arena_len = ln->jb.arena_len;
  pthread_mutex_lock(&sv->mu);
  if (sv->tail) sv->tail->next = rq; else sv->head = rq;
  sv->tail = rq;
  pthread_cond_signal(&sv->posted);
  pthread_mutex_unlock(&sv->mu);
  ln->posted = true;
  return 0;
}

static int collect_dp(worker* w, lane* ln) {
  if (!ln->posted) return 0;
  dp_request* rq = &ln->rq;
  for (;;) {
    const uint32_t seen = __atomic_load_n(&w->wake, __ATOMIC_ACQUIRE);
    if (__atomic_load_n(&rq->done, __ATOMIC_ACQUIRE)) break;
    ef_phase(EFP_SLEEP);
    worker_sleep(&w->wake, seen);
    ef_phase(EFP_SCHED_COLLECT);
  }
  ln->posted = false;
  const int rc = rq->rc;
  const bool tracing = ef_dp_trace_enabled() != 0;
  if (rc == PGPU_OK) {
    size_t j = rq->base;
    for (size_t i = 0; i < ln->n_inflight; ++i) {
      fiber* f = ln->inflight[i];
      f->rc = 0;
      for (size_t k = 0; k < f->nreq; ++k, ++j) {
        const int drc = ef_decode_result(f->reqs[k].kind, &rq->batch->results[j], rq->batch->strings, &f->ress[k]);
        if (drc != 0) {
          fprintf(stderr, "* FATAL DP job of kind %d (%zu x %zu) exceeds the device limits\n", f->reqs[k].kind, f->reqs[k].la, f->reqs[k].lb);
          f->rc = drc;
        }
        else if (tracing) ef_dp_trace(&f->reqs[k], &f->ress[k], (uint32_t)f->unit);
      }
      f->state = F_RUNNABLE;
    }
  }
  const bool last = __atomic_sub_fetch(&rq->batch->refs, 1, __ATOMIC_ACQ_REL) == 0;
  if (last) { free(rq->batch->results); free(rq->batch->strings); free(rq->batch); }
  ln->n_inflight = 0;
  return rc;
}

static void* worker_main(void* arg) {
  pthread_setname_np(pthread_self(), "ef-worker");
  worker* w = (worker*)arg;
  shared* sh = w->sh;
  const int n_lanes = sh->n_lanes;
  const size_t per_lane = sh->max_fibers / n_lanes ? sh->max_fibers / n_lanes : 1;
  for (int li = 0; li < n_lanes; ++li) {
    lane* ln = &w->lanes[li];
    ln->fibers = (fiber**)malloc(per_lane * sizeof(fiber*));
    ln->inflight = (fiber**)malloc(per_lane * sizeof(fiber*));
    ef_jobbuf_init(&ln->jb);
  }
  if (ef_prof_on) { memset(&ef_prof, 0, sizeof ef_prof); ef_prof.dummy = EFP_SCHED; ef_prof.last = ef_prof_now(); }
  if (w->index < EF_MAX_WORKERS) { w->free_fibers = sh->worker_pool[w->index]; sh->worker_pool[w->index] = NULL; }
  bool more = true;
  int cursor = 0;
  const bool prefetch_on = !getenv("PINTRON_NO_FIBER_PREFETCH");
  while (!sh->failed) {
    int li = -1, first_posted = -1;
    const bool can_start = more && (!w->holding || unit_ready(sh, w->held_unit));
    for (int k = 0; k < n_lanes; ++k) {
      const int idx = (cursor + k) % n_lanes;
      lane* c = &w->lanes[idx];
      if (c->posted) {
        if (__atomic_load_n(&c->rq.done, __ATOMIC_ACQUIRE)) { li = idx; break; }
        if (first_posted < 0) first_posted = idx;
      } else if (c->n_fibers > 0 || can_start) { li = idx; break; }
    }
    if (li < 0 && first_posted < 0 && more && w->holding) {
      wait_unit_ready(sh, w->held_unit);
      if (sh->failed) break;
      continue;
    }
    if (li < 0 && first_posted >= 0) {
      const double tw = now_s();
      ef_phase(EFP_SLEEP);
      for (;;) {
        const uint32_t seen = __atomic_load_n(&w->wake, __ATOMIC_ACQUIRE);
        for (int k = 0; k < n_lanes && li < 0; ++k) {
          const int idx = (cursor + k) % n_lanes;
          if (w->lanes[idx].posted && __atomic_load_n(&w->lanes[idx].rq.done, __ATOMIC_ACQUIRE)) li = idx;
        }
        if (li >= 0 || sh->failed) break;
        worker_sleep(&w->wake, seen);
      }
      w->stats.dp_s += now_s() - tw;
      if (ef_prof_on) {
        const double t1 = now_s();
        int b = (int)((tw - sh->prof_t0) / 0.005); if (b < 0) b = 0; if (b > 63) b = 63;
        w->sleep_bins[b] += t1 - tw;
      }
      ef_phase(EFP_SCHED);
      if (li < 0) break;
    }
    if (li < 0) break;
    cursor = (li + 1) % n_lanes;
    lane* ln = &w->lanes[li];
    double t0 = now_s();
    ef_phase(EFP_SCHED_COLLECT);
    if (collect_dp(w, ln) != 0) { sh->failed = 1; break; }
    w->stats.dp_s += now_s() - t0;
    ef_phase(EFP_SCHED_START);
    while (more && ln->n_fibers < per_lane) {
      const int sr = start_fiber(w, li);
      if (sr == START_LATER) break;
      more = sr == START_OK;
    }
    ef_phase(EFP_SCHED);
    if (ln->n_fibers > 0) {
      t0 = now_s();
      for (size_t i = 0; i < ln->n_fibers; ++i) {
        fiber* f = ln->fibers[i];
        if (prefetch_on && i + 2 < ln->n_fibers) fiber_prefetch(ln->fibers[i + 2]);
        if (f->state == F_RUNNABLE) {
          if (EF_TSAN) tsan_to(f->tsan);
          if (ef_prof_on) { ef_phase(EFP_SCHED); ef_prof.cur = &f->phase; }
          ctx_switch(&w->sched, &f->ctx);
          if (ef_prof_on) { ef_phase(f->phase); ef_prof.cur = NULL; ef_prof.dummy = EFP_SCHED; }
        }
      }
      size_t keep = 0;
      for (size_t i = 0; i < ln->n_fibers; ++i) {
        fiber* f = ln->fibers[i];
        if (f->state == F_DONE) {
          if (memcmp(f->stack, FIBER_SENTINEL, sizeof FIBER_SENTINEL) != 0) {
            fprintf(stderr, "* FATAL fibre stack overflow (raise PINTRON_FIBER_STACK_KB, now %zu)\n", sh->stack_size / 1024);
            abort();
          }
          f->pool_next = w->free_fibers; w->free_fibers = f; w->stats.units++;
        }
        else ln->fibers[keep++] = f;
      }
      ln->n_fibers = keep;
      w->stats.host_s += now_s() - t0;
      t0 = now_s();
      int brc = submit_pairings(w, ln);
      w->stats.pairing_s += now_s() - t0;
      t0 = now_s();
      ef_phase(EFP_SCHED_LAUNCH);
      if (brc == 0) brc = launch_dp(w, ln);
      ef_phase(EFP_SCHED);
      w->stats.dp_s += now_s() - t0;
      if (brc != 0) { sh->failed = 1; break; }
    }
  }
  for (int li = 0; li < n_lanes; ++li) {
    lane* ln = &w->lanes[li];
    collect_dp(w, ln);
    ef_jobbuf_free(&ln->jb);
    free(ln->fibers); free(ln->inflight);
  }
  if (w->ctx) pgpu_destroy(w->ctx);
  if (w->free_fibers && w->index < EF_MAX_WORKERS) { sh->worker_pool[w->index] = w->free_fibers; w->free_fibers = NULL; }
  if (w->free_fibers) {
    fiber* last = w->free_fibers;
    while (last->pool_next) last = last->pool_next;
    pthread_mutex_lock(&sh->mu);
    last->pool_next = sh->fiber_pool; sh->fiber_pool = w->free_fibers;
    pthread_mutex_unlock(&sh->mu);
    w->free_fibers = NULL;
  }
  ef_cell_release_all();
  if (ef_prof_on) {
    ef_phase(EFP_SCHED);
    pthread_mutex_lock(&sh->mu);
    for (int k = 0; k < EFP_N; ++k) { sh->prof_cyc[k] += ef_prof.cyc[k]; sh->prof_susp[k] += ef_prof.susp[k]; sh->prof_jobs[k] += ef_prof.jobs[k]; }
    for (int k = 0; k < 64; ++k) sh->prof_sleep_bins[k] += w->sleep_bins[k];
    sh->prof_ahead[0] += ef_prof.ahead_asked; sh->prof_ahead[1] += ef_prof.ahead_hits; sh->prof_ahead[2] += ef_prof.ahead_misses;
    sh->prof_ahead[3] += ef_prof.chain_graphs; sh->prof_ahead[4] += ef_prof.other_graphs;
    pthread_mutex_unlock(&sh->mu);
  }
  return NULL;
}

static bool env_flag(const char* name) {
  const char* v = getenv(name);
  return v && !(v[0] == '0' && v[1] == '\0');
}

static size_t env_size(const char* name, size_t dflt) {
  const char* v = getenv(name);
  return (v && atol(v) > 0) ? (size_t)atol(v) : dflt;
}

static size_t host_core_share(void) {
  long n = sysconf(_SC_NPROCESSORS_ONLN);
  cpu_set_t set;
  if (sched_getaffinity(0, sizeof set, &set) == 0 && CPU_COUNT(&set) > 0 && CPU_COUNT(&set) < n) n = CPU_COUNT(&set);
  long long quota = -1, period = 0;
  FILE* f = fopen("/sys/fs/cgroup/cpu.max", "r");
  if (f) {
    char q[32];
    if (fscanf(f, "%31s %lld", q, &period) == 2 && strcmp(q, "max") != 0) quota = atoll(q);
    fclose(f);
  } else if ((f = fopen("/sys/fs/cgroup/cpu/cpu.cfs_quota_us", "r")) != NULL) {
    if (fscanf(f, "%lld", &quota) != 1) quota = -1;
    fclose(f);
    if ((f = fopen("/sys/fs/cgroup/cpu/cpu.cfs_period_us", "r")) != NULL) {
      if (fscanf(f, "%lld", &period) != 1) period = 0;
      fclose(f);
    }
  }
  if (quota > 0 && period > 0) {
    const long q = (long)((quota + period - 1) / period);
    if (q < n) n = q;
  }
  const char* lws = getenv("LOCAL_WORLD_SIZE");
  if (lws && atol(lws) > 1) n /= atol(lws);
  if (n > 16) n = 16;
  return n > 0 ? (size_t)n : 1;
}

static size_t default_workers(void) {
  const size_t c = host_core_share();
  return c + c / 8;
}

static cpu_set_t numa_original;
static int numa_bound = -2;
static int open_sessions;

static int guess_gpu_numa_node(int dev) {
  if (getenv("HIP_VISIBLE_DEVICES") || getenv("ROCR_VISIBLE_DEVICES") || getenv("CUDA_VISIBLE_DEVICES")) return -1;
  int minors[64], n = 0;
  DIR* d = opendir("/dev/dri");
  if (!d) return -1;
  for (struct dirent* e; (e = readdir(d)) != NULL && n < 64;)
    if (strncmp(e->d_name, "renderD", 7) == 0) minors[n++] = atoi(e->d_name + 7);
  closedir(d);
  for (int i = 1; i < n; ++i) for (int j = i; j > 0 && minors[j - 1] > minors[j]; --j) { const int t = minors[j]; minors[j] = minors[j - 1]; minors[j - 1] = t; }
  if (dev < 0 || dev >= n) return -1;
  char path[96];
  snprintf(path, sizeof path, "/sys/class/drm/renderD%d/device/numa_node", minors[dev]);
  FILE* f = fopen(path, "r");
  if (!f) return -1;
  int node = -1;
  if (fscanf(f, "%d", &node) != 1) node = -1;
  fclose(f);
  return node;
}

static void restore_affinity(void) {
  if (numa_bound >= -1) sched_setaffinity(0, sizeof numa_original, &numa_original);
  numa_bound = -2;
}

static void bind_to_numa_node(int node) {
  const char* sw = getenv("PINTRON_NUMA");
  if (sw && sw[0] == '0' && sw[1] == '\0') return;
  const char* forced = getenv("PINTRON_NUMA_NODE");
  if (forced && forced[0]) node = atoi(forced);
  if (node < 0 || node == numa_bound) return;
  if (numa_bound == -2 && sched_getaffinity(0, sizeof numa_original, &numa_original) != 0) return;
  char path[96];
  snprintf(path, sizeof path, "/sys/devices/system/node/node%d/cpulist", node);
  FILE* f = fopen(path, "r");
  if (!f) return;
  cpu_set_t want;
  CPU_ZERO(&want);
  const char* lws = getenv("LOCAL_WORLD_SIZE");
  const bool several_ranks = (lws && atoi(lws) > 1) || env_flag("PINTRON_SMT");
  int lo, hi, n = 0;
  for (;;) {
    if (fscanf(f, "%d", &lo) != 1) break;
    hi = lo;
    int ch = fgetc(f);
    if (ch == '-') { if (fscanf(f, "%d", &hi) != 1) break; ch = fgetc(f); }
    for (int c = lo; c <= hi && c < CPU_SETSIZE; ++c) {
      if (!CPU_ISSET(c, &numa_original)) continue;
      if (several_ranks) { CPU_SET(c, &want); ++n; continue; }
      char sp[112];
      snprintf(sp, sizeof sp, "/sys/devices/system/cpu/cpu%d/topology/thread_siblings_list", c);
      FILE* sf = fopen(sp, "r");
      int first = c;
      if (sf) { if (fscanf(sf, "%d", &first) != 1) first = c; fclose(sf); }
      if (first != c && CPU_ISSET(first, &numa_original)) continue;
      CPU_SET(c, &want); ++n;
    }
    if (ch != ',') break;
  }
  fclose(f);
  if (numa_bound == -2) numa_bound = -1;
  if (n >= 2 && sched_setaffinity(0, sizeof want, &want) == 0) numa_bound = node;
}

static size_t default_fibers(const ef_inputs* in) {
  size_t total = 0;
  const size_t n = in->n < 4096 ? in->n : 4096;
  for (size_t k = 0; k < n; ++k) total += strlen(in->list[k]->seq);
  return (n && total / n < 300) ? 1024 : 768;
}

static struct {
  pthread_mutex_t mu;
  fiber* fibers; size_t stack_size;
  out_chunk* chunks;
  pgpu_ctx* ctx[2 * MAX_SERVICES + 2]; int ctx_device[2 * MAX_SERVICES + 2]; int n_ctx;
  unsigned char* pre_slab; size_t pre_slab_cap; char* up_stage; size_t up_stage_cap;
  void* units; size_t units_cap;
} kept = { PTHREAD_MUTEX_INITIALIZER, NULL, 0, NULL, { NULL }, { 0 }, 0, NULL, 0, NULL, 0, NULL, 0 };
static bool keep_on(void) { const char* e = getenv("PINTRON_KEEP"); return !(e && e[0] == '0' && e[1] == '\0'); }

static int ctx_take(int device, pgpu_ctx** out) {
  pthread_mutex_lock(&kept.mu);
  for (int k = 0; k < kept.n_ctx; ++k)
    if (kept.ctx_device[k] == device) {
      *out = kept.ctx[k];
      kept.ctx[k] = kept.ctx[kept.n_ctx - 1]; kept.ctx_device[k] = kept.ctx_device[kept.n_ctx - 1]; --kept.n_ctx;
      pthread_mutex_unlock(&kept.mu);
      return PGPU_OK;
    }
  pthread_mutex_unlock(&kept.mu);
  return pgpu_init(device, out);
}
static void ctx_give(pgpu_ctx* ctx, int device) {
  if (!ctx) return;
  if (keep_on()) {
    pthread_mutex_lock(&kept.mu);
    if (kept.n_ctx < (int)(sizeof kept.ctx / sizeof kept.ctx[0])) {
      kept.ctx[kept.n_ctx] = ctx; kept.ctx_device[kept.n_ctx] = device; ++kept.n_ctx;
      pthread_mutex_unlock(&kept.mu);
      return;
    }
    pthread_mutex_unlock(&kept.mu);
  }
  pgpu_destroy(ctx);
}

struct ef_session {
  ef_inputs in;
  pgpu_ctx* ctx0;
  shared sh;
  pgpu_pairing_plan* pplan[PRE_CHUNKS];
  pthread_t pre_thread;
  double pre_kernel_ms[6], pre_meg_ms, pre_t0, pre_wall;
  size_t nthreads;
  double load_s, index_s;
  int device;
  pthread_t pool_thread[2]; int n_pool_threads;
  struct pool_job { shared* sh; size_t count; } pool_job[2];
};

static void* pool_builder_main(void* arg) {
  pthread_setname_np(pthread_self(), "ef-fibre-pool");
  struct pool_job* job = (struct pool_job*)arg;
  shared* sh = job->sh;
  for (size_t i = 0; i < job->count && !sh->failed; ++i) {
    fiber* f = (fiber*)calloc(1, sizeof(fiber));
    if (!f) break;
    f->stack = stack_alloc(sh->stack_size, &f->guarded);
    if (!f->stack) { free(f); break; }
    memcpy(f->stack, FIBER_SENTINEL, sizeof FIBER_SENTINEL);
    ((volatile char*)f->stack)[sh->stack_size - 64] = 0;
    ((volatile char*)f->stack)[sh->stack_size - 4096 - 64] = 0;
    pthread_mutex_lock(&sh->mu);
    f->pool_next = sh->fiber_pool; sh->fiber_pool = f;
    pthread_mutex_unlock(&sh->mu);
  }
  return NULL;
}

typedef struct {
  pgpu_ctx* ctx; int rc; const char* gen; size_t gen_len; pgpu_index* idx; int idx_rc;
  int n_svc; pgpu_ctx* svc[MAX_SERVICES]; int svc_rc;
  double t_init, t_index, t_svc;
} gpu_boot;
static void boot_service_contexts(gpu_boot* b) {
  b->svc_rc = PGPU_OK;
  for (int k = 0; k < b->n_svc && b->svc_rc == PGPU_OK; ++k) {
    b->svc_rc = ctx_take(ef_gpu_device_from_env(), &b->svc[k]);
    if (b->svc_rc == PGPU_OK) pgpu_set_timing(b->svc[k], env_flag("PINTRON_KERNEL_TIMING") ? 1 : 0);
  }
}
static void* boot_service_contexts_main(void* arg) {
  gpu_boot* b = (gpu_boot*)arg;
  const double t0 = now_s();
  boot_service_contexts(b);
  b->t_svc = now_s() - t0;
  return NULL;
}
static void* genomic_tables_main(void* arg) {
  pthread_setname_np(pthread_self(), "ef-gene-tables");
  ef_prepare_genomic_tables((ef_inputs*)arg);
  return NULL;
}

static void* gpu_boot_main(void* arg) {
  pthread_setname_np(pthread_self(), "ef-gpu-boot");
  gpu_boot* b = (gpu_boot*)arg;
  const double tb0 = now_s();
  b->rc = ctx_take(ef_gpu_device_from_env(), &b->ctx);
  b->t_init = now_s() - tb0;
  if (b->rc == PGPU_OK) {
    pgpu_set_timing(b->ctx, env_flag("PINTRON_KERNEL_TIMING") ? 1 : 0);
    pthread_t svc_thread;
    const bool svc_started = pthread_create(&svc_thread, NULL, boot_service_contexts_main, b) == 0;
    const char* cache = getenv("PINTRON_INDEX_CACHE");
    char path[1200];
    bool loaded = false;
    const double tb1 = now_s();
    if (cache && cache[0]) {
      unsigned long long h = 1469598103934665603ull;
      for (size_t i = 0; i < b->gen_len; ++i) { h ^= (unsigned char)b->gen[i]; h *= 1099511628211ull; }
      snprintf(path, sizeof path, "%s/pintron-index-%016llx-%zu.bin", cache, h, b->gen_len);
      b->idx_rc = pgpu_index_load(b->ctx, path, b->gen, b->gen_len, &b->idx);
      loaded = b->idx_rc == PGPU_OK;
    }
    ef_info_mark("gst-construction-begin");
    if (!loaded) {
      b->idx_rc = pgpu_index_build(b->ctx, b->gen, b->gen_len, &b->idx);
      if (b->idx_rc == PGPU_OK && cache && cache[0] && ef_shard_rank == 0 && pgpu_index_save(b->ctx, b->idx, b->gen, path) != PGPU_OK)
        fprintf(stderr, "* WARN the index could not be saved to %s\n", path);
    }
    b->t_index = now_s() - tb1;
    ef_info_mark("gst-preprocessing-begin");
    if (svc_started) pthread_join(svc_thread, NULL); else boot_service_contexts_main(b);
    ef_info_mark("gst-preprocessing-end");
  }
  return NULL;
}

ef_session* ef_session_open(int argc, char** argv) {
  const double t_start = now_s();
  ef_info_mark("start");
  mallopt(M_TRIM_THRESHOLD, 512 << 20);
  mallopt(M_TOP_PAD, 16 << 20);
  bind_to_numa_node(guess_gpu_numa_node(ef_gpu_device_from_env()));
  ef_session* s = (ef_session*)calloc(1, sizeof(ef_session));
  ++open_sessions;
  pthread_mutex_init(&s->sh.mu, NULL);
  pthread_cond_init(&s->sh.ready_cv, NULL);
  pthread_mutex_init(&s->sh.svc.mu, NULL);
  pthread_cond_init(&s->sh.svc.posted, NULL);
  pthread_cond_init(&s->sh.svc.finished, NULL);
  int load_rc = ef_load_genomic_sequence(argc, argv, &s->in);
  if (load_rc != 0) { ef_session_close(s); return NULL; }
  gpu_boot boot;
  memset(&boot, 0, sizeof boot);
  boot.rc = boot.idx_rc = boot.svc_rc = PGPU_EDEVICE;
  boot.gen = s->in.gen->seq; boot.gen_len = strlen(s->in.gen->seq);
  {
    size_t dflt = host_core_share() * 3 / 8;
    if (dflt < 1) dflt = 1;
    if (dflt > 6) dflt = 6;
    boot.n_svc = (int)env_size("PINTRON_SERVICES", dflt);
  }
  if (boot.n_svc > MAX_SERVICES) boot.n_svc = MAX_SERVICES;
  pthread_t boot_thread;
  const bool booting = pthread_create(&boot_thread, NULL, gpu_boot_main, &boot) == 0;
  ef_parse_threads = (int)env_size("PINTRON_PARSE_THREADS", host_core_share());
  {
    pthread_t tab_thread;
    const bool tab_started = pthread_create(&tab_thread, NULL, genomic_tables_main, &s->in) == 0;
    if (!tab_started) ef_prepare_genomic_tables(&s->in);
    load_rc = ef_load_ests(&s->in);
    if (tab_started) pthread_join(tab_thread, NULL);
  }
  ef_classify_init();
  const double t_loaded = now_s();
  ef_info_mark("data-io-end");
  s->device = ef_gpu_device_from_env();
  size_t kept_fibers = 0;
  {
    const size_t stack_size = env_size("PINTRON_FIBER_STACK_KB", 256) * 1024;
    pthread_mutex_lock(&kept.mu);
    if (kept.fibers && kept.stack_size == stack_size) { s->sh.fiber_pool = kept.fibers; kept.fibers = NULL; }
    s->sh.spare_chunks = kept.chunks; kept.chunks = NULL;
    s->sh.pre_slab = kept.pre_slab; s->sh.pre_slab_cap = kept.pre_slab_cap; kept.pre_slab = NULL; kept.pre_slab_cap = 0;
    s->sh.up_stage = kept.up_stage; s->sh.up_stage_cap = kept.up_stage_cap; kept.up_stage = NULL; kept.up_stage_cap = 0;
    pthread_mutex_unlock(&kept.mu);
    for (fiber* f = s->sh.fiber_pool; f; f = f->pool_next) ++kept_fibers;
  }
  if (load_rc == 0 && !getenv("PINTRON_NO_FIBER_POOL")) {
    s->sh.stack_size = env_size("PINTRON_FIBER_STACK_KB", 256) * 1024;
    size_t want = env_size("PINTRON_THREADS", default_workers()) * env_size("PINTRON_FIBERS", default_fibers(&s->in));
    if (want > s->in.n) want = s->in.n;
    want = want > kept_fibers ? want - kept_fibers : 0;
    if (want >= 64) {
      for (int t = 0; t < 2; ++t) {
        s->pool_job[t].sh = &s->sh; s->pool_job[t].count = want / 2;
        if (pthread_create(&s->pool_thread[s->n_pool_threads], NULL, pool_builder_main, &s->pool_job[t]) == 0) ++s->n_pool_threads;
      }
    }
  }
  if (booting) pthread_join(boot_thread, NULL); else gpu_boot_main(&boot);
  const double t_booted = now_s();
  if (boot.rc == PGPU_OK) { s->ctx0 = boot.ctx; s->sh.idx = boot.idx_rc == PGPU_OK ? boot.idx : NULL; }
  for (int k = 0; k < boot.n_svc; ++k) s->sh.svc.threads[k].ctx = boot.svc[k];
  if (load_rc != 0) { ef_session_close(s); return NULL; }
  if (boot.rc != PGPU_OK) {
    fprintf(stderr, "* FATAL no usable MI355X (gfx950) device / libpintron_gpu.so: est-fact has no CPU fallback\n");
    ef_session_close(s); return NULL;
  }
  bind_to_numa_node(pgpu_device_numa_node(s->ctx0));
  ef_inputs* in = &s->in;
  shared* sh = &s->sh;
  sh->in = in;
  if (boot.idx_rc != PGPU_OK) {
    fprintf(stderr, "* FATAL pgpu_index_build: %s\n", pgpu_last_error(s->ctx0));
    ef_session_close(s); return NULL;
  }
  {
    pthread_mutex_lock(&kept.mu);
    if (kept.units && kept.units_cap >= in->n + 1) { sh->units = (unit*)kept.units; sh->units_cap = kept.units_cap; kept.units = NULL; kept.units_cap = 0; }
    pthread_mutex_unlock(&kept.mu);
    if (sh->units) memset(sh->units, 0, (in->n + 1) * sizeof(unit));
    else { sh->units = (unit*)calloc(in->n + 1, sizeof(unit)); sh->units_cap = in->n + 1; }
  }
  for (size_t k = 0; k < in->n;) {
    unit* u = &sh->units[sh->n_units++];
    u->first = k;
    u->has_sibling = in->has_rev ? in->has_rev[k] != 0 : !in->list[k]->fixed_strand;
    k += u->has_sibling ? 2 : 1;
  }
  if (!getenv("PINTRON_NO_PREFETCH") && in->n > 0) {
    size_t want = env_size("PINTRON_PRE_CHUNKS", 10);
    if (!getenv("PINTRON_PRE_CHUNKS")) { const size_t by_size = sh->n_units / 4096 + 1; if (by_size < want) want = by_size; }
    if (want > PRE_CHUNKS) want = PRE_CHUNKS;
    sh->n_pre = sh->n_units < want ? (int)sh->n_units : (int)want;
    double wts[PRE_CHUNKS]; int nw = 0;
    const char* ramp = getenv("PINTRON_PRE_RAMP");
    if (ramp && ramp[0]) {
      for (const char* q = ramp; *q && nw < PRE_CHUNKS;) {
        char* end = NULL;
        const double v = strtod(q, &end);
        if (end == q) break;
        if (v > 0) wts[nw++] = v;
        if (*end != ',' && *end != ':') break;
        q = end + 1;
      }
    }
    if (nw > 0 && (size_t)nw <= sh->n_units) sh->n_pre = nw;
    else { nw = sh->n_pre; for (int k = 0; k < nw; ++k) wts[k] = 1.0; }
    double tot = 0, acc = 0;
    for (int k = 0; k < nw; ++k) tot += wts[k];
    for (int cidx = 0; cidx <= sh->n_pre; ++cidx) {
      size_t u = cidx == sh->n_pre ? sh->n_units : (size_t)((double)sh->n_units * (acc / tot));
      if (cidx > 0 && cidx < sh->n_pre) {
        size_t prev_u = 0;
        while (prev_u < sh->n_units && sh->units[prev_u].first < sh->pre_lo[cidx - 1]) ++prev_u;
        if (u <= prev_u) u = prev_u + 1;
      }
      if (u > sh->n_units) u = sh->n_units;
      sh->pre_lo[cidx] = u < sh->n_units ? sh->units[u].first : in->n;
      if (cidx < sh->n_pre) acc += wts[cidx];
    }
  }
  sh->svc.n_threads = boot.n_svc;
  sh->svc.coalesce_us = getenv("PINTRON_COALESCE_US") ? atol(getenv("PINTRON_COALESCE_US")) : 0;
  if (boot.svc_rc != PGPU_OK) {
    fprintf(stderr, "* FATAL the GPU contexts of the service threads could not be created\n");
    ef_session_close(s); return NULL;
  }
  if (getenv("PINTRON_VERBOSE"))
    fprintf(stderr, "* open: load %.3fs, then GPU runtime + index + service contexts still %.3fs, rest %.3fs (GPU side: runtime + first context %.3fs, index %.3fs, service contexts %.3fs)\n",
            t_loaded - t_start, t_booted - t_loaded, now_s() - t_booted, boot.t_init, boot.t_index, boot.t_svc);
  s->nthreads = env_size("PINTRON_THREADS", default_workers());
  if (s->nthreads > sh->n_units) s->nthreads = sh->n_units ? sh->n_units : 1;
  sh->max_fibers = env_size("PINTRON_FIBERS", default_fibers(in));
  sh->stack_size = env_size("PINTRON_FIBER_STACK_KB", 256) * 1024;
  sh->kernel_timing = env_flag("PINTRON_KERNEL_TIMING");
  sh->gen_len = strlen(in->gen->seq);
  {
    const char* gm = getenv("PINTRON_GPU_MEG");
    sh->use_meg = !(gm && gm[0] == '0' && gm[1] == '\0');
    const ef_config* c = &in->cfg;
    const pgpu_meg_params mp = { c->min_factor_len, c->min_intron_length, c->max_intron_length, c->max_pairings_in_MEG,
                                 c->max_prefix_discarded_rate, c->max_suffix_discarded_rate, c->max_freq_shortest_pairing,
                                 c->trans_red ? 1u : 0u, c->short_edge_comp ? 1u : 0u };
    sh->meg_prm = mp;
  }
  sh->n_lanes = (int)env_size("PINTRON_LANES", 8);
  if (sh->n_lanes > MAX_LANES) sh->n_lanes = MAX_LANES;
  s->load_s = t_loaded - t_start;
  s->index_s = now_s() - t_loaded;
  return s;
}

static void merge_worker_pools(shared* sh) {
  for (size_t t = 0; t < EF_MAX_WORKERS; ++t) {
    fiber* f = sh->worker_pool[t];
    sh->worker_pool[t] = NULL;
    while (f) { fiber* nx = f->pool_next; f->pool_next = sh->fiber_pool; sh->fiber_pool = f; f = nx; }
  }
}

static void free_unit_buffers(shared* sh, bool release) {
  for (size_t u = 0; u < sh->n_units; ++u)
    for (int k = 0; k < EF_N_OUT; ++k) { sh->units[u].buf[k] = NULL; sh->units[u].len[k] = 0; }
  while (sh->chunks) { out_chunk* nx = sh->chunks->next; sh->chunks->next = sh->spare_chunks; sh->spare_chunks = sh->chunks; sh->chunks = nx; }
  if (release) while (sh->spare_chunks) { out_chunk* nx = sh->spare_chunks->next; free(sh->spare_chunks); sh->spare_chunks = nx; }
}

typedef struct { ef_session* s; int c; uint64_t* off; size_t total; char* blob; bool own_blob; int rc; pthread_t th; bool started; } stage_job;
static void* stage_main(void* arg) {
  stage_job* j = (stage_job*)arg;
  ef_session* s = j->s;
  shared* sh = &s->sh;
  ef_inputs* in = &s->in;
  const size_t lo = sh->pre_lo[j->c], hi = sh->pre_lo[j->c + 1];
  j->rc = PGPU_OK; j->blob = NULL; j->own_blob = false;
  j->off = (uint64_t*)malloc((hi - lo + 1) * sizeof(uint64_t));
  if (!j->off) { j->rc = PGPU_ENOMEM; return NULL; }
  size_t total = 0;
  for (size_t k = lo; k < hi; ++k) { j->off[k - lo] = total; total += strlen(in->list[k]->seq); }
  j->off[hi - lo] = total;
  j->total = total;
  if (total + 1 > sh->up_stage_cap) {
    if (sh->up_stage) pgpu_host_free(s->ctx0, sh->up_stage);
    sh->up_stage = NULL; sh->up_stage_cap = 0;
    void* q = NULL;
    const size_t want = total + total / 4 + 4096;
    if (pgpu_host_alloc(s->ctx0, want, &q) == PGPU_OK) { sh->up_stage = (char*)q; sh->up_stage_cap = want; }
  }
  j->blob = sh->up_stage ? sh->up_stage : (char*)malloc(total + 1);
  j->own_blob = j->blob != sh->up_stage;
  if (!j->blob) { j->rc = PGPU_ENOMEM; return NULL; }
  for (size_t k = lo; k < hi; ++k) memcpy(j->blob + j->off[k - lo], in->list[k]->seq, (size_t)(j->off[k - lo + 1] - j->off[k - lo]));
  return NULL;
}
static void stage_start(stage_job* j, ef_session* s, int c) {
  memset(j, 0, sizeof *j);
  j->s = s; j->c = c;
  j->started = pthread_create(&j->th, NULL, stage_main, j) == 0;
  if (!j->started) stage_main(j);
}
static int stage_finish(stage_job* j) {
  if (j->started) { pthread_join(j->th, NULL); j->started = false; }
  ef_session* s = j->s;
  int prc = j->rc;
  if (prc == PGPU_OK) {
    const size_t lo = s->sh.pre_lo[j->c], hi = s->sh.pre_lo[j->c + 1];
    prc = pgpu_pairing_plan_create_resident(s->ctx0, s->sh.idx, j->blob, j->off, hi - lo, &s->pplan[j->c]);
  }
  if (j->own_blob) free(j->blob);
  free(j->off);
  j->off = NULL; j->blob = NULL;
  return prc;
}

static void* prefetch_main(void* arg) {
  pthread_setname_np(pthread_self(), "ef-pairings");
  ef_session* s = (ef_session*)arg;
  shared* sh = &s->sh;
  pgpu_pairing_params prm = { s->in.cfg.min_factor_len, 0, s->in.cfg.min_string_depth_rate };
  stage_job stage; bool staging = false;
  memset(&stage, 0, sizeof stage);
  for (int c = 0; c < sh->n_pre; ++c) {
    char rname[48];
    snprintf(rname, sizeof rname, "prefetch chunk %d (pairings + MEGs)", c);
    pgpu_range_push(rname);
    const double tc0 = now_s();
    int prc = PGPU_OK;
    if (!s->pplan[c]) {
      if (!staging) { stage_start(&stage, s, c); staging = true; }
      prc = stage_finish(&stage);
      staging = false;
      if (prc == PGPU_OK && c + 1 < sh->n_pre && !s->pplan[c + 1]) { stage_start(&stage, s, c + 1); staging = true; }
    }
    const double tc1 = now_s();
    if (prc == PGPU_OK) prc = pgpu_pairing_plan_run(s->ctx0, s->pplan[c], &prm);
    const double tc2 = now_s();
    bool have_meg = false;
    if (prc == PGPU_OK && sh->use_meg) {
      const int mrc = pgpu_pairing_plan_run_meg(s->ctx0, s->pplan[c], &sh->meg_prm);
      if (mrc == PGPU_ENOSYS) sh->use_meg = false;
      else if (mrc != PGPU_OK) prc = mrc;
      else {
        const size_t bytes = (size_t)pgpu_pairing_plan_meg_bytes(s->pplan[c]);
        const size_t entries = sh->pre_lo[c + 1] - sh->pre_lo[c];
        if (!sh->pre_slab && c == 1 && sh->n_pre > 2) {
          const size_t per = (bytes + bytes / 4 + 4096 + (entries + 2) * sizeof(uint64_t) + 511) & ~(size_t)511;
          void* q = NULL;
          if (pgpu_host_alloc(s->ctx0, per * (size_t)(sh->n_pre - 1), &q) == PGPU_OK) { sh->pre_slab = (unsigned char*)q; sh->pre_slab_cap = per * (size_t)(sh->n_pre - 1); }
        }
        if (bytes > sh->pre_meg_cap[c] || !sh->pre_meg[c]) {
          if (sh->pre_meg[c] && sh->pre_own[c]) pgpu_host_free(s->ctx0, sh->pre_meg[c]);
          sh->pre_meg[c] = NULL; sh->pre_own[c] = false;
          sh->pre_meg_cap[c] = bytes + bytes / 8 + 4096;
          const size_t need = (sh->pre_meg_cap[c] + 255) & ~(size_t)255;
          if (sh->pre_slab && sh->pre_slab_used + need <= sh->pre_slab_cap) { sh->pre_meg[c] = sh->pre_slab + sh->pre_slab_used; sh->pre_slab_used += need; }
          else {
            void* q = NULL;
            if (pgpu_host_alloc(s->ctx0, sh->pre_meg_cap[c], &q) == PGPU_OK) { sh->pre_meg[c] = (unsigned char*)q; sh->pre_own[c] = true; }
          }
        }
        if (!sh->pre_meg_first[c]) {
          const size_t need = ((entries + 1) * sizeof(uint64_t) + 255) & ~(size_t)255;
          if (sh->pre_slab && sh->pre_slab_used + need <= sh->pre_slab_cap) { sh->pre_meg_first[c] = (uint64_t*)(sh->pre_slab + sh->pre_slab_used); sh->pre_slab_used += need; }
          else {
            void* q = NULL;
            if (pgpu_host_alloc(s->ctx0, (entries + 1) * sizeof(uint64_t), &q) == PGPU_OK) { sh->pre_meg_first[c] = (uint64_t*)q; sh->pre_first_own[c] = true; }
          }
        }
        if (!sh->pre_meg[c] || !sh->pre_meg_first[c]) prc = PGPU_ENOMEM;
        else prc = pgpu_pairing_plan_fetch_meg(s->ctx0, s->pplan[c], sh->pre_meg[c], sh->pre_meg_cap[c], sh->pre_meg_first[c]);
        have_meg = prc == PGPU_OK;
        s->pre_meg_ms += pgpu_pairing_plan_meg_ms(s->pplan[c]);
      }
    }
    if (prc == PGPU_OK && !have_meg) {
      const size_t cnt = (size_t)pgpu_pairing_plan_count(s->pplan[c]);
      sh->pre_tri[c] = (pgpu_pairing*)malloc((cnt + 1) * sizeof(pgpu_pairing));
      sh->pre_first[c] = (uint64_t*)malloc((sh->pre_lo[c + 1] - sh->pre_lo[c] + 1) * sizeof(uint64_t));
      prc = pgpu_pairing_plan_fetch(s->ctx0, s->pplan[c], sh->pre_tri[c], cnt, sh->pre_first[c]);
    }
    for (int k = 0; k < 6; ++k) s->pre_kernel_ms[k] += pgpu_pairing_plan_kernel_ms(s->pplan[c], k);
    if (getenv("PINTRON_VERBOSE") && atoi(getenv("PINTRON_VERBOSE")) >= 2)
      fprintf(stderr, "* prefetch chunk %d: at %.3fs of the step; plan + upload %.1f ms, pairings %.1f ms, MEGs + download %.1f ms\n", c,
              tc0 - s->pre_t0, 1e3 * (tc1 - tc0), 1e3 * (tc2 - tc1), 1e3 * (now_s() - tc2));
    pthread_mutex_lock(&sh->mu);
    if (prc != PGPU_OK) { fprintf(stderr, "* FATAL pairing prefetch failed: %s\n", pgpu_last_error(s->ctx0)); sh->failed = 1; }
    else __atomic_store_n(&sh->ready_entries, sh->pre_lo[c + 1], __ATOMIC_RELEASE);
    pthread_cond_broadcast(&sh->ready_cv);
    pthread_mutex_unlock(&sh->mu);
    pgpu_range_pop();
    if (prc != PGPU_OK) break;
  }
  if (staging) {
    if (stage.started) pthread_join(stage.th, NULL);
    if (stage.own_blob) free(stage.blob);
    free(stage.off);
  }
  s->pre_wall = now_s() - s->pre_t0;
  return NULL;
}

typedef struct { double wall, user, sys; long minflt; } run_mark;
static run_mark run_mark_now(void) {
  struct rusage ru;
  getrusage(RUSAGE_SELF, &ru);
  run_mark m = { now_s(), ru.ru_utime.tv_sec + 1e-6 * ru.ru_utime.tv_usec, ru.ru_stime.tv_sec + 1e-6 * ru.ru_stime.tv_usec, ru.ru_minflt };
  return m;
}

static int cmp_interval(const void* x, const void* y) {
  const double a = *(const double*)x, b = *(const double*)y;
  return a < b ? -1 : a > b ? 1 : 0;
}

int ef_session_step(ef_session* s, ef_sched_stats* stats_out) {
  shared* sh = &s->sh;
  const double t0 = now_s();
  pgpu_range_push("est-fact step");
  const bool step_rusage = getenv("PINTRON_STEP_RUSAGE") != NULL;
  run_mark ru0; if (step_rusage) ru0 = run_mark_now();
  free_unit_buffers(sh, false);
  for (int c = 0; c < PRE_CHUNKS; ++c) { free(sh->pre_tri[c]); free(sh->pre_first[c]); sh->pre_tri[c] = NULL; sh->pre_first[c] = NULL; }
  sh->next_unit = 0; sh->failed = 0; sh->ready_entries = 0;
  sh->prof_t0 = t0; memset(sh->prof_sleep_bins, 0, sizeof sh->prof_sleep_bins); memset(sh->prof_ahead, 0, sizeof sh->prof_ahead);
  memset(s->pre_kernel_ms, 0, sizeof s->pre_kernel_ms);
  s->pre_meg_ms = 0;
  s->pre_t0 = t0; s->pre_wall = 0;
  bool pre_started = false;
  if (sh->n_pre) {
    pre_started = pthread_create(&s->pre_thread, NULL, prefetch_main, s) == 0;
    if (!pre_started) prefetch_main(s);
  }
  const double t1 = now_s();
  service* sv = &sh->svc;
  sv->stop = false; sv->head = sv->tail = NULL; sv->sh = sh;
  for (int k = 0; k < sv->n_threads; ++k) {
    memset(&sv->threads[k].stats, 0, sizeof(ef_sched_stats));
    memset(sv->threads[k].phase_s, 0, sizeof sv->threads[k].phase_s);
    sv->threads[k].n_iv = 0;
    sv->threads[k].sv = sv;
  }
  int sv_started = 0;
  while (sv_started < sv->n_threads && pthread_create(&sv->threads[sv_started].thread, NULL, service_main, &sv->threads[sv_started]) == 0) ++sv_started;
  worker* ws = (worker*)calloc(s->nthreads, sizeof(worker));
  pthread_t* th = (pthread_t*)malloc(s->nthreads * sizeof(pthread_t));
  size_t w_started = 0;
  if (sv_started > 0)
    for (size_t t = 0; t < s->nthreads; ++t) { ws[w_started].sh = sh; ws[w_started].index = w_started; if (pthread_create(&th[w_started], NULL, worker_main, &ws[w_started]) == 0) ++w_started; }
  if (sv_started == 0 || w_started == 0) { fprintf(stderr, "* FATAL cannot start the service / worker threads\n"); sh->failed = 1; }
  const unsigned long long prof_c0 = ef_prof_now(); const double prof_t0 = now_s();
  memset(sh->prof_cyc, 0, sizeof sh->prof_cyc); memset(sh->prof_susp, 0, sizeof sh->prof_susp); memset(sh->prof_jobs, 0, sizeof sh->prof_jobs);
  for (size_t t = 0; t < w_started; ++t) pthread_join(th[t], NULL);
  if (ef_prof_on && w_started) {
    static const char* nm[EFP_N] = { "other", "meg", "embeddings", "endpoints", "external", "dust", "noisy", "add", "filters", "gap-errors",
                                     "refine-intron", "tail/polyA", "refinement", "output", "side-files", "free", "scheduler", "sleep",
                                     "ref:affixes", "ref:false-small", "ref:new-small", "ref:clean", "sched:launch", "sched:collect", "sched:start", "wait:prefetch",
                                     "new-small:prefix", "new-small:ask", "new-small:class", "new-small:search", "search:lookups", "search:decide", "search:end" };
    const double hz = (double)(ef_prof_now() - prof_c0) / (now_s() - prof_t0);
    unsigned long long ts = 0, tj = 0; double tot = 0;
    fprintf(stderr, "* profile (per worker thread, %zu workers, %zu units): phase, seconds, suspensions / unit, jobs / unit\n", w_started, sh->n_units);
    for (int k = 0; k < EFP_N; ++k) {
      const double sec = (double)sh->prof_cyc[k] / hz / (double)w_started;
      fprintf(stderr, "*   %-14s %8.4f s  %6.2f  %6.2f\n", nm[k], sec, (double)sh->prof_susp[k] / (double)sh->n_units, (double)sh->prof_jobs[k] / (double)sh->n_units);
      ts += sh->prof_susp[k]; tj += sh->prof_jobs[k]; if (k != EFP_SLEEP && k != EFP_WAIT_PREFETCH) tot += sec;
    }
    fprintf(stderr, "*   asked ahead: %.2f jobs / unit, found there %.2f, asked in turn (while answers were kept) %.2f\n",
            (double)sh->prof_ahead[0] / (double)sh->n_units, (double)sh->prof_ahead[1] / (double)sh->n_units, (double)sh->prof_ahead[2] / (double)sh->n_units);
    fprintf(stderr, "*   graphs that are one path (enumerated from the record): %llu of %llu\n", sh->prof_ahead[3], sh->prof_ahead[3] + sh->prof_ahead[4]);
    fprintf(stderr, "*   asleep waiting for batches, ms per worker in each 5 ms of the step:");
    for (int k = 0; k < 64 && k * 0.005 < now_s() - t0; ++k) fprintf(stderr, " %.1f", 1e3 * sh->prof_sleep_bins[k] / (double)w_started);
    fprintf(stderr, "\n");
    fprintf(stderr, "*   %-14s %8.4f s  %6.2f  %6.2f\n", "all but sleeps", tot, (double)ts / (double)sh->n_units, (double)tj / (double)sh->n_units);
  }
  if (pre_started) pthread_join(s->pre_thread, NULL);
  pthread_mutex_lock(&sv->mu); sv->stop = true; pthread_cond_broadcast(&sv->posted); pthread_mutex_unlock(&sv->mu);
  for (int k = 0; k < sv_started; ++k) pthread_join(sv->threads[k].thread, NULL);
  ef_sched_stats st;
  memset(&st, 0, sizeof st);
  st.threads = s->nthreads;
  for (int t = 0; t < sv_started; ++t) {
    const ef_sched_stats* ss = &sv->threads[t].stats;
    const double* ph = sv->threads[t].phase_s;
    if (getenv("PINTRON_VERBOSE"))
      fprintf(stderr, "* service %d: %zu batches, %zu jobs; idle %.3fs merge %.3fs create %.3fs launch %.3fs sync %.3fs fetch %.3fs\n",
              t, ss->dp_batches, ss->dp_jobs, ph[0], ph[1] - ph[0], ph[2], ph[3], ph[4], ph[5]);
    st.dp_batches += ss->dp_batches; st.dp_jobs += ss->dp_jobs;
    for (int k = 0; k < ss->n_kernels; ++k) kstat_add(&st, &ss->kernels[k]);
  }
  {
    size_t n = 0;
    for (int t = 0; t < sv_started; ++t) n += sv->threads[t].n_iv / 2;
    if (n) {
      double* a = (double*)malloc(2 * n * sizeof(double));
      size_t k = 0;
      for (int t = 0; t < sv_started; ++t) { memcpy(a + k, sv->threads[t].iv, sv->threads[t].n_iv * sizeof(double)); k += sv->threads[t].n_iv; }
      qsort(a, n, 2 * sizeof(double), cmp_interval);
      double busy = 0, lo = a[0], hi = a[1];
      for (size_t i = 1; i < n; ++i) {
        if (a[2 * i] > hi) { busy += hi - lo; lo = a[2 * i]; hi = a[2 * i + 1]; }
        else if (a[2 * i + 1] > hi) hi = a[2 * i + 1];
      }
      st.dp_busy_union_ms = busy + (hi - lo);
      free(a);
    }
  }
  for (size_t t = 0; t < w_started; ++t) {
    st.units += ws[t].stats.units;
    st.pairing_batches += ws[t].stats.pairing_batches; st.pairing_requests += ws[t].stats.pairing_requests;
    st.host_s += ws[t].stats.host_s; st.pairing_s += ws[t].stats.pairing_s; st.dp_s += ws[t].stats.dp_s;
    for (int k = 0; k < ws[t].stats.n_kernels; ++k) kstat_add(&st, &ws[t].stats.kernels[k]);
  }
  if (sh->n_pre) {
    static const char* nm[6] = { "pair_locate", "pair_chain", "pair_count+scan", "pair_fill", "pair_cross+scan", "pair_emit" };
    for (int k = 0; k < 6; ++k) {
      ef_kernel_stat ks; memset(&ks, 0, sizeof ks);
      snprintf(ks.name, sizeof ks.name, "%s", nm[k]);
      ks.ms = s->pre_kernel_ms[k]; ks.launches = (size_t)sh->n_pre; ks.jobs = s->in.n;
      if (k == 0 || k == 5) {
        unsigned long long positions = 0, pairs = 0;
        for (int c = 0; c < sh->n_pre; ++c) { positions += pgpu_pairing_plan_positions(s->pplan[c]); pairs += pgpu_pairing_plan_count(s->pplan[c]); }
        unsigned long long run = sh->gen_len / 65536ull + 1;
        unsigned lg = 0;
        while ((1ull << lg) < run + 1) ++lg;
        ks.algo_bytes = k == 0 ? positions * (1ull + 8ull + 2ull * 4ull * lg + 12ull) + pairs * 4ull : pairs * 12ull;
      }
      if (ks.ms > 0) kstat_add(&st, &ks);
    }
    if (s->pre_meg_ms > 0) {
      ef_kernel_stat ks; memset(&ks, 0, sizeof ks);
      snprintf(ks.name, sizeof ks.name, "meg_build+emit");
      ks.ms = s->pre_meg_ms; ks.launches = (size_t)sh->n_pre; ks.jobs = s->in.n;
      unsigned long long pairs = 0, rec = 0;
      for (int c = 0; c < sh->n_pre; ++c) { pairs += pgpu_pairing_plan_count(s->pplan[c]); rec += pgpu_pairing_plan_meg_bytes(s->pplan[c]); }
      ks.algo_bytes = pairs * 12ull + rec;
      kstat_add(&st, &ks);
    }
  }
  { size_t su = 0; for (size_t t = 0; t < w_started; ++t) su += ws[t].suspensions; st.suspensions_per_unit = sh->n_units ? (double)su / (double)sh->n_units : 0.0; }
  st.load_s = s->load_s; st.index_s = s->index_s; st.prefetch_s = s->pre_wall; st.workers_s = now_s() - t1;
  for (size_t u = 0; u < sh->n_units; ++u) if (sh->units[u].len[1]) ++st.aligned;
  if (stats_out) *stats_out = st;
  ef_dp_trace_flush();
  pgpu_range_pop();
  ef_info_mark("est-processing-end");
  free(ws); free(th);
  if (step_rusage) {
    const run_mark ru1 = run_mark_now();
    fprintf(stderr, "* step: %.3fs wall, user %.2fs sys %.2fs (all threads of the process), %ld page faults\n",
            ru1.wall - ru0.wall, ru1.user - ru0.user, ru1.sys - ru0.sys, ru1.minflt - ru0.minflt);
  }
  return sh->failed ? 1 : 0;
}

enum { WRITE_RANGES = 8, WRITE_THREADS_MAX = 16, WRITE_IOV = 512 };
typedef struct { int fd, k; size_t u0, u1; off_t at; } write_task;
typedef struct { shared* sh; write_task* tasks; int n_tasks; int next; int failed; } write_pool;
static void* write_pool_main(void* arg) {
  pthread_setname_np(pthread_self(), "ef-writer");
  write_pool* wp = (write_pool*)arg;
  struct iovec iov[WRITE_IOV];
  for (;;) {
    const int t = __atomic_fetch_add(&wp->next, 1, __ATOMIC_RELAXED);
    if (t >= wp->n_tasks) return NULL;
    const write_task* wt = &wp->tasks[t];
    off_t at = wt->at;
    size_t u = wt->u0;
    while (u < wt->u1) {
      int n = 0; size_t bytes = 0;
      for (; u < wt->u1 && n < WRITE_IOV; ++u) {
        const unit* un = &wp->sh->units[u];
        if (!un->len[wt->k]) continue;
        iov[n].iov_base = un->buf[wt->k]; iov[n].iov_len = un->len[wt->k]; bytes += un->len[wt->k]; ++n;
      }
      int first = 0;
      while (bytes) {
        const ssize_t w = pwritev(wt->fd, iov + first, n - first, at);
        if (w < 0 && errno == EINTR) continue;
        if (w <= 0) { __atomic_store_n(&wp->failed, 1, __ATOMIC_RELAXED); return NULL; }
        at += w; bytes -= (size_t)w;
        size_t left = (size_t)w;
        while (left && first < n) {
          if (left >= iov[first].iov_len) { left -= iov[first].iov_len; ++first; }
          else { iov[first].iov_base = (char*)iov[first].iov_base + left; iov[first].iov_len -= left; left = 0; }
        }
      }
    }
  }
}

typedef struct { shared* sh; FILE* f; int k; } file_writer;
static void* file_writer_main(void* arg) {
  file_writer* fw = (file_writer*)arg;
  setvbuf(fw->f, NULL, _IOFBF, 1 << 20);
  for (size_t u = 0; u < fw->sh->n_units; ++u)
    if (fw->sh->units[u].len[fw->k]) fwrite(fw->sh->units[u].buf[fw->k], 1, fw->sh->units[u].len[fw->k], fw->f);
  return NULL;
}

int ef_session_write_outputs(ef_session* s) {
  ef_outputs out;
  if (ef_open_outputs(&out)) return 1;
  shared* sh = &s->sh;
  FILE* dst[6] = { out.fout.f, out.fests.f, out.fmeg.f, out.fpmeg.f, out.ftmeg.f, out.fintronic.f };
  write_task tasks[6 * WRITE_RANGES];
  write_pool wp = { sh, tasks, 0, 0, 0 };
  for (int k = 0; k < 6; ++k) {
    fflush(dst[k]);
    off_t at = 0;
    for (int r = 0; r < WRITE_RANGES; ++r) {
      const size_t u0 = sh->n_units * (size_t)r / WRITE_RANGES, u1 = sh->n_units * (size_t)(r + 1) / WRITE_RANGES;
      size_t bytes = 0;
      for (size_t u = u0; u < u1; ++u) bytes += sh->units[u].len[k];
      if (bytes) { write_task wt = { fileno(dst[k]), k, u0, u1, at }; tasks[wp.n_tasks++] = wt; }
      at += (off_t)bytes;
    }
  }
  {
    size_t w[6] = {0};
    for (int k = 0; k < 6; ++k) for (size_t u = 0; u < sh->n_units; u += 64) w[k] += sh->units[u].len[k];
    for (int a = 1; a < wp.n_tasks; ++a) {
      const write_task t = tasks[a]; int b = a;
      while (b > 0 && w[tasks[b - 1].k] < w[t.k]) { tasks[b] = tasks[b - 1]; --b; }
      tasks[b] = t;
    }
  }
  {
    size_t nth = env_size("PINTRON_WRITE_THREADS", host_core_share());
    if (nth > WRITE_THREADS_MAX) nth = WRITE_THREADS_MAX;
    if (nth > (size_t)wp.n_tasks) nth = (size_t)wp.n_tasks;
    pthread_t th[WRITE_THREADS_MAX]; size_t started = 0;
    for (size_t t = 1; t < nth; ++t) if (pthread_create(&th[started], NULL, write_pool_main, &wp) == 0) ++started;
    write_pool_main(&wp);
    for (size_t t = 0; t < started; ++t) pthread_join(th[t], NULL);
  }
  const char* rec_path = getenv("PINTRON_RECORDS_FILE");
  int rec_rc = 0;
  if (rec_path && rec_path[0]) {
    FILE* rf = fopen(rec_path, "wb");
    if (!rf) { fprintf(stderr, "* cannot write %s\n", rec_path); rec_rc = 1; }
    else {
      file_writer rw = { sh, rf, 6 };
      file_writer_main(&rw);
      if (fclose(rf) != 0) rec_rc = 1;
    }
  }
  ef_close_outputs(&out);
  if (wp.failed) { fprintf(stderr, "* FATAL writing the output files failed\n"); return 1; }
  return rec_rc;
}

char* ef_session_output(ef_session* s, int which, size_t* len) {
  shared* sh = &s->sh;
  if (which < 0 || which >= EF_N_OUT) { *len = 0; return NULL; }
  size_t total = 0;
  for (size_t u = 0; u < sh->n_units; ++u) total += sh->units[u].len[which];
  char* r = (char*)malloc(total + 1);
  size_t pos = 0;
  for (size_t u = 0; u < sh->n_units; ++u) { memcpy(r + pos, sh->units[u].buf[which], sh->units[u].len[which]); pos += sh->units[u].len[which]; }
  r[pos] = '\0';
  *len = total;
  return r;
}

char* ef_session_records(ef_session* s, size_t* len) { return ef_session_output(s, 0, len); }

size_t ef_session_n_ests(const ef_session* s) { return s->sh.n_units; }
struct pgpu_ctx* ef_session_context(ef_session* s) { return s->ctx0; }
const void* ef_session_genomic(ef_session* s) { return s->in.gen; }

void ef_session_close(ef_session* s) {
  if (!s) return;
  shared* sh = &s->sh;
  const bool verbose = getenv("PINTRON_VERBOSE") != NULL;
  double tq[6]; tq[0] = now_s();
  for (int t = 0; t < s->n_pool_threads; ++t) pthread_join(s->pool_thread[t], NULL);
  s->n_pool_threads = 0;
  free_unit_buffers(sh, !keep_on());
  if (keep_on() && sh->spare_chunks) {
    pthread_mutex_lock(&kept.mu);
    out_chunk* last = sh->spare_chunks;
    while (last->next) last = last->next;
    last->next = kept.chunks; kept.chunks = sh->spare_chunks; sh->spare_chunks = NULL;
    pthread_mutex_unlock(&kept.mu);
  }
  merge_worker_pools(sh);
  if (getenv("PINTRON_STACK_STATS")) {
    size_t n = 0, sum = 0, mx = 0;
    for (fiber* f = sh->fiber_pool; f; f = f->pool_next) {
      size_t lo = sizeof FIBER_SENTINEL;
      while (lo < sh->stack_size && f->stack[lo] == 0) lo += 64;
      const size_t used = lo < sh->stack_size ? sh->stack_size - lo : 0;
      ++n; sum += used; if (used > mx) mx = used;
    }
    fprintf(stderr, "* fibre stacks: %zu fibres, %zu B used on average, %zu B at most (of %zu)\n", n, n ? sum / n : 0, mx, sh->stack_size);
  }
  if (keep_on() && sh->fiber_pool && sh->stack_size) {
    pthread_mutex_lock(&kept.mu);
    if (!kept.fibers || kept.stack_size == sh->stack_size) {
      fiber* last = sh->fiber_pool;
      while (last->pool_next) last = last->pool_next;
      last->pool_next = kept.fibers; kept.fibers = sh->fiber_pool; kept.stack_size = sh->stack_size;
      sh->fiber_pool = NULL;
    }
    pthread_mutex_unlock(&kept.mu);
  }
  while (sh->fiber_pool) {
    fiber* nx = sh->fiber_pool->pool_next;
    for (int k = 0; k < EF_N_OUT; ++k) free(sh->fiber_pool->out[k].mem);
    stack_free(sh->fiber_pool->stack, sh->stack_size, sh->fiber_pool->guarded); free(sh->fiber_pool);
    sh->fiber_pool = nx;
  }
  if (keep_on() && sh->units) {
    pthread_mutex_lock(&kept.mu);
    if (!kept.units || kept.units_cap < sh->units_cap) { free(kept.units); kept.units = sh->units; kept.units_cap = sh->units_cap; sh->units = NULL; }
    pthread_mutex_unlock(&kept.mu);
  }
  free(sh->units);
  tq[1] = now_s();
  for (int k = 0; k < MAX_SERVICES; ++k) { free(sh->svc.threads[k].iv); sh->svc.threads[k].iv = NULL; sh->svc.threads[k].n_iv = sh->svc.threads[k].cap_iv = 0; }
  for (int c = 0; c < PRE_CHUNKS && s->ctx0; ++c) {
    free(sh->pre_tri[c]); free(sh->pre_first[c]);
    if (sh->pre_meg[c] && sh->pre_own[c]) pgpu_host_free(s->ctx0, sh->pre_meg[c]);
    if (sh->pre_meg_first[c] && sh->pre_first_own[c]) pgpu_host_free(s->ctx0, sh->pre_meg_first[c]);
    if (s->pplan[c]) pgpu_pairing_plan_destroy(s->ctx0, s->pplan[c]);
  }
  if (keep_on() && s->ctx0) {
    pthread_mutex_lock(&kept.mu);
    if (sh->pre_slab && !kept.pre_slab) { kept.pre_slab = sh->pre_slab; kept.pre_slab_cap = sh->pre_slab_cap; sh->pre_slab = NULL; }
    if (sh->up_stage && !kept.up_stage) { kept.up_stage = sh->up_stage; kept.up_stage_cap = sh->up_stage_cap; sh->up_stage = NULL; }
    pthread_mutex_unlock(&kept.mu);
  }
  tq[2] = now_s();
  if (sh->pre_slab) pgpu_host_free(s->ctx0, sh->pre_slab);
  if (sh->up_stage) pgpu_host_free(s->ctx0, sh->up_stage);
  if (s->ctx0 && sh->idx) pgpu_index_destroy(s->ctx0, sh->idx);
  tq[3] = now_s();
  for (int k = 0; k < MAX_SERVICES; ++k) ctx_give(sh->svc.threads[k].ctx, s->device);
  ctx_give(s->ctx0, s->device);
  tq[4] = now_s();
  ef_free_inputs(&s->in);
  tq[5] = now_s();
  if (verbose)
    fprintf(stderr, "* close: unit buffers + fibres %.3fs, pairing plans %.3fs, index + slabs %.3fs, contexts %.3fs, inputs %.3fs\n",
            tq[1] - tq[0], tq[2] - tq[1], tq[3] - tq[2], tq[4] - tq[3], tq[5] - tq[4]);
  pthread_mutex_destroy(&sh->mu); pthread_cond_destroy(&sh->ready_cv);
  pthread_mutex_destroy(&sh->svc.mu); pthread_cond_destroy(&sh->svc.posted); pthread_cond_destroy(&sh->svc.finished);
  free(s);
  if (--open_sessions == 0) restore_affinity();
}

int ef_leave_without_cleanup = 0;

typedef struct { char* p; size_t len; } page_range;
typedef struct { page_range* r; size_t n; size_t next; } page_release;
static void* page_release_main(void* arg) {
  page_release* pr = (page_release*)arg;
  for (;;) {
    const size_t k = __atomic_fetch_add(&pr->next, 1, __ATOMIC_RELAXED);
    if (k >= pr->n) return NULL;
    madvise(pr->r[k].p, pr->r[k].len, MADV_DONTNEED);
  }
}
static void session_release_pages(ef_session* s) {
  shared* sh = &s->sh;
  merge_worker_pools(sh);
  size_t cap = 1024, n = 0;
  for (fiber* f = sh->fiber_pool; f; f = f->pool_next) ++cap;
  for (out_chunk* c = sh->chunks; c; c = c->next) ++cap;
  for (out_chunk* c = sh->spare_chunks; c; c = c->next) ++cap;
  void** ab = (void**)malloc(65536 * sizeof(void*)); size_t* al = (size_t*)malloc(65536 * sizeof(size_t));
  if (!ab || !al) { free(ab); free(al); return; }
  const size_t na = ef_record_arena_regions(s->in.arena, ab, al, 65536);
  page_range* r = (page_range*)malloc((cap + na) * 16 * sizeof(page_range));
  if (!r) { free(ab); free(al); return; }
  const size_t piece = (size_t)8 << 20, room = (cap + na) * 16;
#define ADD_RANGE(ptr, bytes) do { \
    uintptr_t a_ = ((uintptr_t)(ptr) + 4095) & ~(uintptr_t)4095, b_ = ((uintptr_t)(ptr) + (bytes)) & ~(uintptr_t)4095; \
    for (; a_ < b_ && n < room; a_ += piece) { r[n].p = (char*)a_; r[n].len = b_ - a_ < piece ? b_ - a_ : piece; ++n; } } while (0)
  for (size_t k = 0; k < na; ++k) ADD_RANGE(ab[k], al[k]);
  for (out_chunk* c = sh->chunks; c; c = c->next) ADD_RANGE(c->data, c->cap);
  for (out_chunk* c = sh->spare_chunks; c; c = c->next) ADD_RANGE(c->data, c->cap);
  for (fiber* f = sh->fiber_pool; f; f = f->pool_next) if (f->guarded) ADD_RANGE(f->stack, sh->stack_size);
  if (sh->units) ADD_RANGE(sh->units, (sh->n_units + 1) * sizeof(unit));
#undef ADD_RANGE
  page_release pr = { r, n, 0 };
  size_t nth = host_core_share();
  if (nth > 16) nth = 16;
  pthread_t th[16]; size_t started = 0;
  for (size_t t = 1; t < nth; ++t) if (pthread_create(&th[started], NULL, page_release_main, &pr) == 0) ++started;
  page_release_main(&pr);
  for (size_t t = 0; t < started; ++t) pthread_join(th[t], NULL);
  free(r); free(ab); free(al);
}

int ef_run_batched_stats(int argc, char** argv, ef_sched_stats* stats_out) {
  const run_mark m0 = run_mark_now();
  ef_session* s = ef_session_open(argc, argv);
  if (!s) return 1;
  ef_sched_stats st;
  const run_mark m1 = run_mark_now();
  int rc = ef_session_step(s, &st);
  const run_mark m2 = run_mark_now();
  if (rc == 0) rc = ef_session_write_outputs(s);
  const run_mark m3 = run_mark_now();
  if (stats_out) *stats_out = st;
  const bool leave = ef_leave_without_cleanup != 0;
  if (!leave) ef_session_close(s);
  else if (!getenv("PINTRON_NO_PAGE_RELEASE")) session_release_pages(s);
  ef_log_reference_timers(st.index_s, st.prefetch_s, st.workers_s, st.load_s + (m3.wall - m2.wall), now_s() - m0.wall);
  if (getenv("PINTRON_VERBOSE")) {
    fprintf(stderr, "* run: open %.3fs step %.3fs write %.3fs close %.3fs\n", m1.wall - m0.wall, m2.wall - m1.wall, m3.wall - m2.wall, now_s() - m3.wall);
    fprintf(stderr, "* cpu (all threads): open user %.2fs sys %.2fs, %ld page faults; step user %.2fs sys %.2fs, %ld page faults; write user %.2fs sys %.2fs\n",
            m1.user - m0.user, m1.sys - m0.sys, m1.minflt - m0.minflt, m2.user - m1.user, m2.sys - m1.sys, m2.minflt - m1.minflt,
            m3.user - m2.user, m3.sys - m2.sys);
  }
  return rc;
}

int ef_run_batched(int argc, char** argv) {
  ef_sched_stats st;
  const int rc = ef_run_batched_stats(argc, argv, &st);
  if (rc == 0 && getenv("PINTRON_VERBOSE")) {
    fprintf(stderr, "est-fact: %zu ESTs (%zu aligned), %zu threads, %zu pairing batches (%zu requests), %zu DP batches (%zu jobs); "
                    "load %.2fs index %.2fs prefetch %.2fs workers %.2fs [per-thread avg: host %.2fs pairing %.2fs dp %.2fs]\n",
            st.units, st.aligned, st.threads, st.pairing_batches, st.pairing_requests, st.dp_batches, st.dp_jobs,
            st.load_s, st.index_s, st.prefetch_s, st.workers_s, st.host_s / st.threads, st.pairing_s / st.threads, st.dp_s / st.threads);
    for (int k = 0; k < st.n_kernels; ++k)
      fprintf(stderr, "  kernel %-28s launches %6zu jobs %9zu  %9.3f ms  %8.1f algo-GB/s\n", st.kernels[k].name, st.kernels[k].launches,
              st.kernels[k].jobs, st.kernels[k].ms, st.kernels[k].ms > 0 ? st.kernels[k].algo_bytes / (st.kernels[k].ms * 1e-3) / 1e9 : 0.0);
  }
  return rc;
}
```

### pintron_amd/host/ef_sched.h

```cpp
#ifndef EF_SCHED_H
#define EF_SCHED_H
#include <stddef.h>

#define EF_MAX_KERNELS 64
typedef struct {
  char name[48];
  double ms;
  size_t launches, jobs;
  unsigned long long cells, algo_bytes;
} ef_kernel_stat;

typedef struct {
  size_t threads, units, aligned, dp_batches, dp_jobs, pairing_batches, pairing_requests;
  double load_s, index_s, prefetch_s, workers_s;
  double host_s, pairing_s, dp_s;
  int n_kernels;
  ef_kernel_stat kernels[EF_MAX_KERNELS];
  double dp_busy_union_ms;
  double suspensions_per_unit;
} ef_sched_stats;

typedef struct ef_session ef_session;
ef_session* ef_session_open(int argc, char** argv);
int ef_session_step(ef_session* s, ef_sched_stats* stats);
int ef_session_write_outputs(ef_session* s);
char* ef_session_records(ef_session* s, size_t* len);
char* ef_session_output(ef_session* s, int which, size_t* len);
size_t ef_session_n_ests(const ef_session* s);
void ef_session_close(ef_session* s);

int ef_main_multi(int argc, char** argv);
struct pgpu_ctx* ef_session_context(ef_session* s);
const void* ef_session_genomic(ef_session* s);

extern int ef_leave_without_cleanup;
int ef_run_batched(int argc, char** argv);
int ef_run_batched_stats(int argc, char** argv, ef_sched_stats* stats);

#endif
```

### pintron_amd/host/estfact.h

```cpp
#ifndef ESTFACT_H
#define ESTFACT_H

#include <limits.h>
#include <stdbool.h>
#include <stddef.h>
#include <stdint.h>
#include <stdio.h>
#include <string.h>

#include "ef_list.h"

typedef struct {
  unsigned min_factor_len;
  int min_intron_length, max_intron_length;
  double min_string_depth_rate;
  double max_prefix_discarded_rate, max_suffix_discarded_rate;
  int max_prefix_discarded, max_suffix_discarded;
  unsigned max_site_difference;
  int max_number_of_factorizations;
  double max_coverage_diff;
  int max_exonNUM_diff, max_gapLength_diff;
  char retain_externals;
  unsigned max_pairings_in_MEG;
  double max_freq_shortest_pairing;
  int suffpref_length_on_est, suffpref_length_for_intron, suffpref_length_on_gen;
  bool trans_red, short_edge_comp;
  unsigned max_single_factorization_time;
  double complexity_threshold;
  char config_file[512];
} ef_config;

void ef_config_defaults(ef_config* c);
int ef_config_load(ef_config* c, int argc, char** argv);

#define EF_POLYA_CHR '*'
#define EF_POLYT_CHR '#'

typedef struct {
  char* id;
  char* seq;
  char* original_seq;
  char* gb;
  char* chr;
  char strand_as_read[16];
  int strand;
  bool fixed_strand;
  int abs_start, abs_end;
  int pref_polyA_length, suff_polyA_length, pref_polyT_length, suff_polyT_length;
  int pref_N_length, suff_N_length;
  uint32_t* kmer_first;
  uint32_t* kmer_pos;
  uint32_t* other_first;
  uint32_t* other_pos;
  unsigned char* bps_memo;
  double* score5_tab[4];
  size_t score5_len;
  unsigned char* cls_start; unsigned char* cls_end;
  unsigned char in_arena;
} ef_seq;

extern unsigned ef_genomic_epoch;
static inline unsigned ef_genomic_epoch_now(void) { return __atomic_load_n(&ef_genomic_epoch, __ATOMIC_ACQUIRE); }
static inline void ef_genomic_epoch_bump(void) { __atomic_add_fetch(&ef_genomic_epoch, 1u, __ATOMIC_ACQ_REL); }
static inline size_t ef_genomic_len(const char* gen) {
  static _Thread_local const char* last; static _Thread_local size_t last_len; static _Thread_local unsigned last_epoch;
  const unsigned ep = ef_genomic_epoch_now();
  if (last != gen || last_epoch != ep) { last_len = strlen(gen); last = gen; last_epoch = ep; }
  return last_len;
}

typedef struct ef_record_arena ef_record_arena;
ef_record_arena* ef_record_arena_new(void);
void ef_record_arena_free(ef_record_arena* a);
size_t ef_record_arena_regions(ef_record_arena* a, void** base, size_t* len, size_t max);
void ef_record_arena_enter(ef_record_arena* a);
void ef_record_arena_leave(void);

long ef_read_multifasta(const char* path, ef_seq*** out);
long ef_read_multifasta_part(const char* path, int part, int parts, ef_seq*** out);
long ef_read_multifasta_arena(const char* path, int part, int parts, ef_record_arena* arena, ef_seq*** out);
extern int ef_parse_threads;
void ef_seq_free(ef_seq* s);
void ef_seq_index_kmers(ef_seq* gen);
void ef_parse_genomic_header(ef_seq* gen);
int  ef_ntails_removal(ef_seq* gen);
void ef_set_gb_identification(ef_seq* est);
void ef_set_strand_and_rc(ef_seq* est);
void ef_reverse_and_complement(ef_seq* est);
void ef_polyAT_substitution(ef_seq* est);
ef_seq* ef_copy_and_reverse(const ef_seq* est);

#define EF_SOURCE_START INT_MIN
#define EF_SINK_START   (INT_MAX - 200)
#define EF_SOURCE_LEN   200

typedef struct ef_pairing {
  int p, t, l;
  int id;
  bool visited;
  ef_list* adjs;
  ef_list* incs;
  ef_list* emb_memo;
} ef_pairing;

typedef struct ef_meg_s {
  size_t n;
  ef_list** v;
  size_t* act; size_t n_act;
  const void* rec;
  bool slab;
  struct ef_meg_s* lists;
  size_t diag_created, diag_peak_list;
} ef_meg;

static inline size_t ef_meg_act_from(const ef_meg* V, size_t lo) {
  size_t a = 0, b = V->n_act;
  while (a < b) { const size_t m = (a + b) / 2; if (V->act[m] < lo) a = m + 1; else b = m; }
  return a;
}
#define EF_MEG_FOR_POS(V, i, lo, hi) \
  for (size_t ef_k_ = ef_meg_act_from((V), (size_t)(lo)), i; \
       ef_k_ < (V)->n_act && (i = (V)->act[ef_k_]) < (size_t)(hi); ++ef_k_)

typedef struct { int32_t p, t, l; } ef_triple;

ef_meg* ef_meg_from_pairings(const ef_triple* tr, size_t n_tr, size_t pattern_len);
ef_meg* ef_meg_from_record(const void* rec, size_t pattern_len);
ef_meg* ef_meg_record_only(const void* rec, size_t pattern_len);
ef_meg* ef_meg_lists(ef_meg* V);
extern int ef_endpoint_checks;
extern int ef_chain_fast_path;
void ef_meg_free(ef_meg* V);
void ef_build_edge_set(ef_meg* V, const ef_config* cfg);
void ef_simplify_meg(ef_meg* V, const ef_config* cfg);
void ef_transitive_reduction(ef_meg* V);
void ef_compact_short_edges(ef_meg* V, const ef_config* cfg);
bool ef_is_too_complex_for_compaction(ef_meg* V);
bool ef_is_too_complex(ef_meg* V, const ef_config* cfg);
void ef_meg_stats(ef_meg* V, size_t* pairings, size_t* edges);
struct ef_sink;
void ef_meg_write(struct ef_sink* f, ef_meg* V);
void ef_intronic_edges_write(struct ef_sink* f, ef_meg* V);

typedef struct ef_sink { FILE* f; char* mem; size_t len, cap; } ef_sink;
static inline void ef_sink_write(ef_sink* s, const char* p, size_t n) {
  if (s->f) { fwrite(p, 1, n, s->f); return; }
  if (s->len + n > s->cap) { s->cap = (s->len + n) * 2 + 256; s->mem = (char*)realloc(s->mem, s->cap); }
  memcpy(s->mem + s->len, p, n); s->len += n;
}
static inline void ef_sink_puts(ef_sink* s, const char* str) { ef_sink_write(s, str, strlen(str)); }

typedef struct { ef_sink* s; char* p; char* end; char b[4096]; } ef_wbuf;
static inline void efw_room(ef_wbuf* w, size_t need);
static inline void efw_open(ef_wbuf* w, ef_sink* s) {
  w->s = s;
  if (s->f) { w->p = w->b; w->end = w->b + sizeof w->b; }
  else { w->p = w->end = NULL; efw_room(w, 128); }
}
static inline void efw_flush(ef_wbuf* w) {
  if (w->s->f) { if (w->p != w->b) { fwrite(w->b, 1, (size_t)(w->p - w->b), w->s->f); w->p = w->b; } }
  else if (w->p) w->s->len = (size_t)(w->p - w->s->mem);
}
static inline void efw_room(ef_wbuf* w, size_t need) {
  if (w->p && (size_t)(w->end - w->p) >= need) return;
  ef_sink* s = w->s;
  if (s->f) { efw_flush(w); return; }
  if (w->p) s->len = (size_t)(w->p - s->mem);
  if (s->len + need > s->cap) { s->cap = (s->len + need) * 2 + 256; s->mem = (char*)realloc(s->mem, s->cap); }
  w->p = s->mem + s->len; w->end = s->mem + s->cap;
}
static inline void efw_ch(ef_wbuf* w, char c) { efw_room(w, 1); *w->p++ = c; }
static inline void efw_mem(ef_wbuf* w, const char* s, size_t n) {
  if (w->s->f && n > 2048) { efw_flush(w); fwrite(s, 1, n, w->s->f); return; }
  efw_room(w, n);
  memcpy(w->p, s, n); w->p += n;
}
static inline void efw_str(ef_wbuf* w, const char* s) { efw_mem(w, s, strlen(s)); }
static inline void efw_strn(ef_wbuf* w, const char* s, int prec) {
  if (prec <= 0) return;
  const char* z = (const char*)memchr(s, 0, (size_t)prec);
  efw_mem(w, s, z ? (size_t)(z - s) : (size_t)prec);
}
static inline void efw_int(ef_wbuf* w, long long v) {
  char t[24]; int k = 0;
  unsigned long long u = v < 0 ? 0ull - (unsigned long long)v : (unsigned long long)v;
  do { t[k++] = (char)('0' + u % 10); u /= 10; } while (u);
  efw_room(w, 24);
  if (v < 0) *w->p++ = '-';
  while (k) *w->p++ = t[--k];
}

enum { EFP_OTHER = 0, EFP_MEG, EFP_EMBED, EFP_ENDPOINTS, EFP_EXTERNAL, EFP_DUST, EFP_NOISY, EFP_ADD, EFP_FILTERS,
       EFP_GAPERR, EFP_INTRON, EFP_TAIL, EFP_FACTREF, EFP_OUTPUT, EFP_SIDE, EFP_FREE, EFP_SCHED, EFP_SLEEP,
       EFP_REF_AFFIX, EFP_REF_FALSE_SMALL, EFP_REF_NEW_SMALL, EFP_REF_CLEAN, EFP_SCHED_LAUNCH, EFP_SCHED_COLLECT, EFP_SCHED_START, EFP_WAIT_PREFETCH,
       EFP_NS_PREFIX, EFP_NS_BETWEEN_ASK, EFP_NS_BETWEEN_CLASS, EFP_NS_BETWEEN_SEARCH, EFP_TMP1, EFP_TMP2, EFP_TMP3, EFP_N };
extern int ef_prof_on;
typedef struct { unsigned long long cyc[EFP_N], susp[EFP_N], jobs[EFP_N]; unsigned long long last; int dummy; int* cur;
                 unsigned long long ahead_hits, ahead_misses, ahead_asked, chain_graphs, other_graphs; } ef_prof_state;
extern _Thread_local ef_prof_state ef_prof;
static inline unsigned long long ef_prof_now(void) {
#if defined(__x86_64__)
  unsigned lo, hi; __asm__ volatile("rdtsc" : "=a"(lo), "=d"(hi)); return ((unsigned long long)hi << 32) | lo;
#else
  return 0;
#endif
}
static inline int ef_phase(int id) {
  if (!ef_prof_on) return 0;
  ef_prof_state* p = &ef_prof;
  int* cur = p->cur ? p->cur : &p->dummy;
  const unsigned long long t = ef_prof_now();
  const int was = *cur;
  p->cyc[was] += t - p->last; p->last = t; *cur = id;
  return was;
}

enum { EF_DP_ALIGN = 0, EF_DP_GAP = 1, EF_DP_ED = 2, EF_DP_KBAND = 3, EF_DP_LCF = 4,
       EF_DP_BORDERS = 5, EF_DP_AFFIX = 6 };
typedef struct {
  int kind;
  const char* a; size_t la;
  const char* b; size_t lb;
  uint32_t p0, p1, p2, tail;
  uint32_t temp;
} ef_dp_req;
typedef struct {
  int32_t v[6];
  char* s0; char* s1;
} ef_dp_res;
#define EF_ROW_PAD 64
static inline void ef_dp_res_rows(ef_dp_res* r, size_t cap) {
  r->s0 = (char*)calloc(2 * (cap + EF_ROW_PAD), 1);
  r->s1 = r->s0 + cap + EF_ROW_PAD;
}
static inline void ef_dp_res_release(ef_dp_res* r) { free(r->s0); r->s0 = r->s1 = NULL; }

#define EF_AHEAD_MAX 96
#define EF_DP_PENDING 1
#define EF_AHEAD_SLOTS 256
typedef struct {
  int n, n_pending;
  bool collecting;
  unsigned char slot[EF_AHEAD_SLOTS];
  ef_dp_req q[EF_AHEAD_MAX]; int32_t v[EF_AHEAD_MAX][6];
} ef_ahead;
static inline void ef_ahead_init(ef_ahead* ah) { ah->n = ah->n_pending = 0; ah->collecting = false; memset(ah->slot, 0, sizeof ah->slot); }

typedef struct ef_backend {
  void* self;
  int (*pairings)(void* self, const char* pattern, size_t m, unsigned min_factor_len, double rate,
                  ef_triple** out, size_t* n);
  int (*dp)(void* self, const ef_dp_req* req, ef_dp_res* res);
  int (*dp_many)(void* self, const ef_dp_req* reqs, ef_dp_res* res, size_t n);
  const void* (*meg)(void* self, const char* pattern, size_t m, const ef_config* cfg);
  ef_ahead* ahead;
} ef_backend;

static inline bool ef_req_same(const ef_dp_req* x, const ef_dp_req* y) {
  return x->kind == y->kind && x->a == y->a && x->b == y->b && x->la == y->la && x->lb == y->lb &&
         x->p0 == y->p0 && x->p1 == y->p1 && x->p2 == y->p2 && x->tail == y->tail;
}
static inline bool ef_req_keepable(const ef_dp_req* q) { return q->temp == 0 && q->kind != EF_DP_ALIGN && q->kind != EF_DP_GAP; }
static inline unsigned ef_req_hash(const ef_dp_req* q) {
  uint64_t h = (uint64_t)(uintptr_t)q->a * 0x9E3779B97F4A7C15ull ^ (uint64_t)(uintptr_t)q->b * 0xC2B2AE3D27D4EB4Full;
  h ^= ((uint64_t)q->la << 32 | (uint64_t)q->lb) * 0x165667B19E3779F9ull + (uint64_t)q->kind;
  return (unsigned)(h >> 40) & (EF_AHEAD_SLOTS - 1);
}
static inline const int32_t* ef_ahead_find(const ef_ahead* ah, const ef_dp_req* q) {
  if (ah->n == 0 || !ef_req_keepable(q)) return NULL;
  for (unsigned s = ef_req_hash(q); ah->slot[s]; s = (s + 1) & (EF_AHEAD_SLOTS - 1))
    if (ef_req_same(&ah->q[ah->slot[s] - 1], q)) return ah->v[ah->slot[s] - 1];
  return NULL;
}
static inline unsigned ef_req_hash(const ef_dp_req* q);
static inline void ef_ahead_put(ef_ahead* ah, const ef_dp_req* q, const int32_t* v) {
  if (ah->n_pending || ah->n >= EF_AHEAD_MAX || !ef_req_keepable(q) || ef_ahead_find(ah, q)) return;
  ah->q[ah->n] = *q; memcpy(ah->v[ah->n], v, 6 * sizeof(int32_t));
  unsigned s = ef_req_hash(q);
  while (ah->slot[s]) s = (s + 1) & (EF_AHEAD_SLOTS - 1);
  ah->slot[s] = (unsigned char)(++ah->n);
}
static inline void ef_ahead_keep_next(ef_ahead* ah, const int32_t* v) {
  memcpy(ah->v[ah->n], v, 6 * sizeof(int32_t));
  unsigned s = ef_req_hash(&ah->q[ah->n]);
  while (ah->slot[s]) s = (s + 1) & (EF_AHEAD_SLOTS - 1);
  ah->slot[s] = (unsigned char)(++ah->n);
}
static inline int ef_backend_ask(ef_backend* be, const ef_dp_req* reqs, ef_dp_res* res, size_t n) {
  if (be->dp_many) return be->dp_many(be->self, reqs, res, n);
  for (size_t k = 0; k < n; ++k) { const int rc = be->dp(be->self, &reqs[k], &res[k]); if (rc != 0) return rc; }
  return 0;
}
int ef_dp_many_ahead(ef_backend* be, const ef_dp_req* reqs, ef_dp_res* res, size_t n);
static inline int ef_dp_many(ef_backend* be, const ef_dp_req* reqs, ef_dp_res* res, size_t n) {
  if (n == 0) return 0;
  memset(res, 0, n * sizeof(ef_dp_res));
  if (be->ahead && (be->ahead->n || be->ahead->collecting)) return ef_dp_many_ahead(be, reqs, res, n);
  return ef_backend_ask(be, reqs, res, n);
}
static inline int ef_dp_one(ef_backend* be, const ef_dp_req* req, ef_dp_res* res) { return ef_dp_many(be, req, res, 1); }
static inline void ef_ahead_collect(ef_backend* be, bool on) { if (be->ahead) be->ahead->collecting = on; }
static inline bool ef_collecting(const ef_backend* be) { return be->ahead && be->ahead->collecting; }
int ef_ahead_flush(ef_backend* be);
extern int ef_ahead_on;

typedef struct { int EST_start, EST_end, GEN_start, GEN_end; } ef_factor;
unsigned ef_chain_candidate(const void* rec, const ef_config* cfg, const char* GEN, ef_factor* out_exons, size_t cap,
                            unsigned* n_exons, unsigned* n_pairs, unsigned* work);
unsigned ef_chain_factorization(const void* rec, const ef_config* cfg, const char* EST, const char* GEN, struct ef_backend* be,
                                ef_factor* out_exons, size_t cap, unsigned* n_exons);

typedef struct {
  const ef_seq* info;
  ef_list* factorizations;
  ef_list* polyA_signals;
  ef_list* polyadenil_signals;
} ef_est;

void ef_factorization_free(void* fact);
void ef_est_free(ef_est* e);

unsigned long long ef_work_high_water(void);
ef_est* ef_get_est_factorizations(const ef_seq* est, ef_meg* V, const ef_config* cfg,
                                  const ef_seq* gen, ef_backend* be);
void ef_refine_est_factorizations(const ef_seq* gen, ef_est* e, const ef_config* cfg, ef_backend* be);
void ef_remove_factorizations_with_very_small_exons(ef_list* facts);
void ef_remove_duplicated_factorizations(ef_list* facts);
typedef struct {
  char* seq_est; char* seq_gen; size_t le, lg;
  int dsl_est, dsl_gen, deleted_intron_dim;
  char buf_e[512], buf_g[512];
} ef_gap_window;
typedef struct { ef_gap_window w; ef_dp_res res; ef_factor donor, acceptor; } ef_gap_ahead;
void ef_gap_window_build(const ef_config* cfg, const ef_seq* gen, const ef_seq* est, const ef_factor* donor,
                         const ef_factor* acceptor, ef_gap_window* w);
void ef_gap_window_release(ef_gap_window* w);
bool ef_refine_intron(const ef_config* cfg, const ef_seq* gen, const ef_seq* est, ef_factor* donor,
                      ef_factor* acceptor, bool first_intron, ef_backend* be, ef_gap_ahead* ahead);
int ef_classify_intron(const ef_seq* gen, int start, int end);
int ef_burset_frequency(const char* donor, const char* acceptor);
int ef_burset_adaptor(const char* t, size_t cut1, size_t cut2);
int ef_check_burset_patterns(const char* gen, int donor_left_on_gen, int acceptor_right_on_gen);
char* ef_real_substring(int index, int length, const char* s);
ef_list* ef_clean_noisy_exons(ef_list* fact, const char* gen, const char* est, bool only_internals, ef_backend* be);
ef_list* ef_clean_external_exons(ef_list* fact, const char* gen, const char* est, ef_backend* be);
ef_list* ef_add_if_not_exists(ef_list* to_add, ef_list* list, const ef_config* cfg, bool* added);
uint32_t ef_edit_distance(ef_backend* be, const char* a, size_t la, const char* b, size_t lb);
uint32_t ef_compute_edit_distance(ef_backend* be, const char* a, size_t la, const char* b, size_t lb);
void ef_write_multifasta_output(const ef_seq* gen, const ef_est* e, ef_sink* f, char retain_externals);
void ef_write_factorization_records(const ef_seq* gen, const ef_est* e, ef_sink* f, char retain_externals, uint32_t est_index);
int ef_raw_text_from_records(const ef_seq* gen, const void* rec, size_t rl, const char* pests, size_t pl, ef_sink* out);
typedef struct { ef_sink *fmeg, *fpmeg, *ftmeg, *fintronic; } ef_side_files;
ef_est* ef_compute_est_fact(const ef_seq* gen, const ef_seq* est, ef_backend* be, const ef_config* cfg,
                            const ef_side_files* side);

ef_meg* ef_build_meg(const ef_seq* est, ef_backend* be, const ef_config* shared_cfg, size_t* inc_pairing_len);

void ef_write_single_est_info(ef_sink* f, const ef_seq* s);

typedef struct { ef_config cfg; ef_seq* gen; ef_seq** list; size_t n; ef_record_arena* arena;
                 bool all_in_arena;
                 unsigned char* has_rev;
} ef_inputs;
typedef struct { FILE* flog; ef_sink fout, fests, fmeg, fpmeg, ftmeg, fintronic; ef_side_files side; } ef_outputs;
int ef_load_inputs(int argc, char** argv, ef_inputs* in);
int ef_load_genomic(int argc, char** argv, ef_inputs* in);
int ef_load_genomic_sequence(int argc, char** argv, ef_inputs* in);
void ef_prepare_genomic_tables(ef_inputs* in);
int ef_load_ests(ef_inputs* in);
extern int ef_shard_rank, ef_shard_world;
void ef_free_inputs(ef_inputs* in);
int ef_open_outputs(ef_outputs* o);
void ef_info_mark(const char* label);
void ef_close_outputs(ef_outputs* o);
void ef_classify_init(void);
void ef_classify_prepare(ef_seq* gen);

void ef_log_reference_timers(double suffix_tree_s, double algorithm_s, double compositions_s, double io_s, double total_s);
int ef_run(int argc, char** argv, ef_backend* (*open_backend)(const ef_seq* gen), void (*close_backend)(ef_backend*));

#endif
```

Baseline: 848,400.

## Serve per-EST factorizations from device kernels and run multiple prefetch lanes

Adds an optional device factorization stage (candidate, clean, gaps and chain kernels) whose per-EST answers (DONE, EMPTY or HOST fallback) let the host skip chain embedding and filter_and_refine for answered ESTs. It also splits the single prefetch thread into several lanes, each with its own GPU context and pinned staging buffer, so pairing-plan creation and staging overlap. The device path is gated on the PINTRON_DEVICE_FACT environment flag, so by default only one lane is used. It adds more contexts, pinned buffers, a mutex around pinned allocation, and the risk of mismatches with the host factorization.

Result: slower. 834,900 (-1.6%).

```diff
diff --git a/pintron_amd/estfact.py b/pintron_amd/estfact.py
--- a/pintron_amd/estfact.py
+++ b/pintron_amd/estfact.py
@@ -34,6 +34,8 @@
     L.ef_session_n_ests.argtypes = [C.c_void_p]
     L.ef_session_write_outputs.argtypes = [C.c_void_p]
     L.ef_session_close.argtypes = [C.c_void_p]
+    L.ef_session_fact_answers.restype = None
+    L.ef_session_fact_answers.argtypes = [C.c_void_p, C.POINTER(C.c_ulonglong * 3)]
     return L
 
 
@@ -59,6 +61,11 @@
 
     def n_ests(self) -> int:
         return int(self.L.ef_session_n_ests(self.h))
+
+    def fact_answers(self) -> dict:
+        a = (C.c_ulonglong * 3)()
+        self.L.ef_session_fact_answers(self.h, C.byref(a))
+        return {"host": int(a[0]), "empty": int(a[1]), "done": int(a[2])}
 
     def output(self, which: int) -> bytes:
         n = C.c_size_t()
diff --git a/pintron_amd/host/ef_fact.c b/pintron_amd/host/ef_fact.c
--- a/pintron_amd/host/ef_fact.c
+++ b/pintron_amd/host/ef_fact.c
@@ -1091,7 +1091,28 @@
   ef_list* flist = efl_new();
   ef_work wk = { 0, work_limit(cfg) };
   emb* chain = NULL;
-  if (V->rec && !V->v && ef_chain_fast_path && chain_embedding(V->rec, cfg, GEN, &wk, &chain)) {
+  ef_fact_answer fa;
+  bool answered = false;
+  if (V->rec && !V->v && ef_chain_fast_path && be->fact &&
+      (cfg->max_number_of_factorizations == 0 || cfg->max_number_of_factorizations >= 1) && be->fact(be->self, EST, cfg, &fa)) {
+    ++ef_prof.fact_answers[fa.outcome <= EF_FACT_DONE ? fa.outcome : EF_FACT_HOST];
+    answered = fa.outcome == EF_FACT_EMPTY || fa.outcome == EF_FACT_DONE;
+  }
+  if (answered) {
+    if (ef_prof_on) ++ef_prof.chain_graphs;
+    wk.used += fa.work;
+    if (wk.used > wk.limit) {
+      efl_free(flist, ef_factorization_free);
+      free(est);
+      return NULL;
+    }
+    if (fa.outcome == EF_FACT_DONE) {
+      ef_list* f = efl_new();
+      for (unsigned k = 0; k < fa.n_exons; ++k)
+        efl_push_back(f, factor_new(fa.exons[4 * k], fa.exons[4 * k + 1], fa.exons[4 * k + 2], fa.exons[4 * k + 3]));
+      efl_push_back(flist, f);
+    }
+  } else if (V->rec && !V->v && ef_chain_fast_path && chain_embedding(V->rec, cfg, GEN, &wk, &chain)) {
     if (ef_prof_on) ++ef_prof.chain_graphs;
     if (wk.used > wk.limit) {
       if (chain) embedding_free(chain);
@@ -1142,7 +1163,7 @@
     while (wk.used > hw && !__atomic_compare_exchange_n(&work_high_water, &hw, wk.used, true, __ATOMIC_RELAXED, __ATOMIC_RELAXED)) { }
   }
 
-  flist = filter_and_refine(flist, est_len, est_info, gen_info, cfg, be);
+  if (!answered) flist = filter_and_refine(flist, est_len, est_info, gen_info, cfg, be);
   ef_phase(EFP_TAIL);
   est->polyA_signals = efl_new();
   est->polyadenil_signals = efl_new();
diff --git a/pintron_amd/host/ef_sched.c b/pintron_amd/host/ef_sched.c
--- a/pintron_amd/host/ef_sched.c
+++ b/pintron_amd/host/ef_sched.c
@@ -182,6 +182,7 @@
 } service;
 
 #define PRE_CHUNKS 16
+#define PRE_LANES_MAX 8
 typedef struct shared {
   ef_inputs* in;
   pgpu_index* idx;
@@ -197,7 +198,16 @@
   unsigned char* pre_meg[PRE_CHUNKS]; size_t pre_meg_cap[PRE_CHUNKS]; uint64_t* pre_meg_first[PRE_CHUNKS];
   unsigned char* pre_slab; size_t pre_slab_cap, pre_slab_used;
   bool pre_own[PRE_CHUNKS], pre_first_own[PRE_CHUNKS];
-  char* up_stage; size_t up_stage_cap;
+  bool use_fact;
+  pgpu_cand_params cand_prm; pgpu_fact_params fact_prm;
+  unsigned char* pre_fblk[PRE_CHUNKS]; size_t pre_fblk_cap[PRE_CHUNKS]; size_t pre_fexons_cap[PRE_CHUNKS];
+  const pgpu_cand_result* pre_cand[PRE_CHUNKS]; const pgpu_fact_result* pre_fact[PRE_CHUNKS]; const pgpu_factor* pre_fexons[PRE_CHUNKS];
+  bool pre_done[PRE_CHUNKS];
+  int n_pre_lanes;
+  char* up_stage[PRE_LANES_MAX]; size_t up_stage_cap[PRE_LANES_MAX];
+  pthread_mutex_t alloc_mu;
+  double fact_kernel_ms[4];
+  unsigned long long fact_answers[3];
   size_t ready_entries;
   pthread_cond_t ready_cv;
   bool kernel_timing;
@@ -300,6 +310,41 @@
   while (f->cur_entry >= sh->pre_lo[c + 1]) ++c;
   if (!sh->pre_meg[c]) return NULL;
   return sh->pre_meg[c] + sh->pre_meg_first[c][f->cur_entry - sh->pre_lo[c]];
+}
+
+static FILE* fact_log;
+static pthread_mutex_t fact_log_mu = PTHREAD_MUTEX_INITIALIZER;
+
+#define EF_WEAK(f) extern __typeof__(f) f __attribute__((weak))
+EF_WEAK(pgpu_pairing_plan_run_candidates); EF_WEAK(pgpu_pairing_plan_candidate_exons); EF_WEAK(pgpu_pairing_plan_fetch_candidates);
+EF_WEAK(pgpu_pairing_plan_candidates_ms); EF_WEAK(pgpu_pairing_plan_run_factorizations); EF_WEAK(pgpu_pairing_plan_factorization_exons);
+EF_WEAK(pgpu_pairing_plan_fetch_factorizations); EF_WEAK(pgpu_pairing_plan_factorizations_ms);
+static bool fact_entries_present(void) {
+  return pgpu_pairing_plan_run_candidates && pgpu_pairing_plan_candidate_exons && pgpu_pairing_plan_fetch_candidates &&
+         pgpu_pairing_plan_candidates_ms && pgpu_pairing_plan_run_factorizations && pgpu_pairing_plan_factorization_exons &&
+         pgpu_pairing_plan_fetch_factorizations && pgpu_pairing_plan_factorizations_ms;
+}
+
+static int fiber_fact(void* self, const char* pattern, const ef_config* cfg, ef_fact_answer* out) {
+  fiber* f = (fiber*)self;
+  const shared* sh = f->w->sh;
+  if (!sh->use_fact || !sh->use_meg || !sh->n_pre || cfg->min_factor_len != sh->in->cfg.min_factor_len ||
+      cfg->min_string_depth_rate != sh->in->cfg.min_string_depth_rate || pattern != sh->in->list[f->cur_entry]->seq)
+    return 0;
+  int c = 0;
+  while (f->cur_entry >= sh->pre_lo[c + 1]) ++c;
+  if (!sh->pre_meg[c] || !sh->pre_fact[c]) return 0;
+  const size_t e = f->cur_entry - sh->pre_lo[c];
+  const pgpu_fact_result* r = &sh->pre_fact[c][e];
+  out->outcome = r->outcome; out->work = sh->pre_cand[c][e].work;
+  out->n_exons = r->outcome == PGPU_FACT_DONE ? r->n_exons : 0;
+  out->exons = r->outcome == PGPU_FACT_DONE ? &sh->pre_fexons[c][r->first_exon].EST_start : NULL;
+  if (fact_log) {
+    pthread_mutex_lock(&fact_log_mu);
+    fprintf(fact_log, "%zu %zu %u %u %u %u\n", f->unit, f->cur_entry, (unsigned)r->outcome, (unsigned)r->stage, out->work, (unsigned)r->detail);
+    pthread_mutex_unlock(&fact_log_mu);
+  }
+  return 1;
 }
 
 static char* out_alloc(worker* w, size_t n) {
@@ -418,6 +463,7 @@
   else { f = (fiber*)calloc(1, sizeof(fiber)); f->stack = stack_alloc(sh->stack_size, &f->guarded); }
   f->w = w; f->unit = u; f->state = F_RUNNABLE; f->lane = li;
   f->be.self = f; f->be.pairings = fiber_pairings; f->be.dp = fiber_dp; f->be.dp_many = fiber_dp_many; f->be.meg = fiber_meg;
+  f->be.fact = sh->use_fact ? fiber_fact : NULL;
   memcpy(f->stack, FIBER_SENTINEL, sizeof FIBER_SENTINEL);
 #if EF_TSAN
   if (f->tsan) __tsan_destroy_fiber(f->tsan);
@@ -634,6 +680,7 @@
     ef_jobbuf_init(&ln->jb);
   }
   if (ef_prof_on) { memset(&ef_prof, 0, sizeof ef_prof); ef_prof.dummy = EFP_SCHED; ef_prof.last = ef_prof_now(); }
+  memset(ef_prof.fact_answers, 0, sizeof ef_prof.fact_answers);
   if (w->index < EF_MAX_WORKERS) { w->free_fibers = sh->worker_pool[w->index]; sh->worker_pool[w->index] = NULL; }
   bool more = true;
   int cursor = 0;
@@ -743,6 +790,9 @@
     w->free_fibers = NULL;
   }
   ef_cell_release_all();
+  pthread_mutex_lock(&sh->mu);
+  for (int k = 0; k < 3; ++k) sh->fact_answers[k] += ef_prof.fact_answers[k];
+  pthread_mutex_unlock(&sh->mu);
   if (ef_prof_on) {
     ef_phase(EFP_SCHED);
     pthread_mutex_lock(&sh->mu);
@@ -878,9 +928,11 @@
   fiber* fibers; size_t stack_size;
   out_chunk* chunks;
   pgpu_ctx* ctx[2 * MAX_SERVICES + 2]; int ctx_device[2 * MAX_SERVICES + 2]; int n_ctx;
-  unsigned char* pre_slab; size_t pre_slab_cap; char* up_stage; size_t up_stage_cap;
+  unsigned char* pre_slab; size_t pre_slab_cap;
   void* units; size_t units_cap;
-} kept = { PTHREAD_MUTEX_INITIALIZER, NULL, 0, NULL, { NULL }, { 0 }, 0, NULL, 0, NULL, 0, NULL, 0 };
+  char* up_stage[PRE_LANES_MAX]; size_t up_stage_cap[PRE_LANES_MAX];
+  unsigned char* fblk[PRE_CHUNKS]; size_t fblk_cap[PRE_CHUNKS];
+} kept = { PTHREAD_MUTEX_INITIALIZER, NULL, 0, NULL, { NULL }, { 0 }, 0, NULL, 0, NULL, 0, { NULL }, { 0 }, { NULL }, { 0 } };
 static bool keep_on(void) { const char* e = getenv("PINTRON_KEEP"); return !(e && e[0] == '0' && e[1] == '\0'); }
 
 static int ctx_take(int device, pgpu_ctx** out) {
@@ -914,7 +966,8 @@
   pgpu_ctx* ctx0;
   shared sh;
   pgpu_pairing_plan* pplan[PRE_CHUNKS];
-  pthread_t pre_thread;
+  pgpu_ctx* lane_ctx[PRE_LANES_MAX];
+  struct pre_lane { struct ef_session* s; int k; pthread_t th; bool started; } pre_lane[PRE_LANES_MAX];
   double pre_kernel_ms[6], pre_meg_ms, pre_t0, pre_wall;
   size_t nthreads;
   double load_s, index_s;
@@ -945,6 +998,7 @@
 typedef struct {
   pgpu_ctx* ctx; int rc; const char* gen; size_t gen_len; pgpu_index* idx; int idx_rc;
   int n_svc; pgpu_ctx* svc[MAX_SERVICES]; int svc_rc;
+  int n_lane; pgpu_ctx* lane[PRE_LANES_MAX];
   double t_init, t_index, t_svc;
 } gpu_boot;
 static void boot_service_contexts(gpu_boot* b) {
@@ -952,6 +1006,10 @@
   for (int k = 0; k < b->n_svc && b->svc_rc == PGPU_OK; ++k) {
     b->svc_rc = ctx_take(ef_gpu_device_from_env(), &b->svc[k]);
     if (b->svc_rc == PGPU_OK) pgpu_set_timing(b->svc[k], env_flag("PINTRON_KERNEL_TIMING") ? 1 : 0);
+  }
+  for (int k = 0; k < b->n_lane && b->svc_rc == PGPU_OK; ++k) {
+    b->svc_rc = ctx_take(ef_gpu_device_from_env(), &b->lane[k]);
+    if (b->svc_rc == PGPU_OK) pgpu_set_timing(b->lane[k], env_flag("PINTRON_KERNEL_TIMING") ? 1 : 0);
   }
 }
 static void* boot_service_contexts_main(void* arg) {
@@ -1012,6 +1070,7 @@
   ++open_sessions;
   pthread_mutex_init(&s->sh.mu, NULL);
   pthread_cond_init(&s->sh.ready_cv, NULL);
+  pthread_mutex_init(&s->sh.alloc_mu, NULL);
   pthread_mutex_init(&s->sh.svc.mu, NULL);
   pthread_cond_init(&s->sh.svc.posted, NULL);
   pthread_cond_init(&s->sh.svc.finished, NULL);
@@ -1028,6 +1087,28 @@
     boot.n_svc = (int)env_size("PINTRON_SERVICES", dflt);
   }
   if (boot.n_svc > MAX_SERVICES) boot.n_svc = MAX_SERVICES;
+  {
+    const ef_config* c = &s->in.cfg;
+    const char* gm = getenv("PINTRON_GPU_MEG");
+    const int sp[3] = { c->suffpref_length_on_est, c->suffpref_length_for_intron, c->suffpref_length_on_gen };
+    bool ok = !(gm && gm[0] == '0' && gm[1] == '\0') && env_flag("PINTRON_DEVICE_FACT") && ef_chain_fast_path &&
+              !getenv("PINTRON_NO_PREFETCH") && c->min_factor_len >= 1 && c->min_factor_len <= (1u << 24);
+    for (int k = 0; k < 3; ++k) ok = ok && sp[k] >= 0 && sp[k] <= (1 << 24);
+    s->sh.use_fact = ok;
+    {
+      const char* lp = getenv("PINTRON_FACT_LOG");
+      pthread_mutex_lock(&fact_log_mu);
+      if (ok && lp && lp[0] && !fact_log) fact_log = fopen(lp, "w");
+      pthread_mutex_unlock(&fact_log_mu);
+    }
+    const pgpu_cand_params cp = { c->min_factor_len, c->min_intron_length };
+    const pgpu_fact_params fp = { c->complexity_threshold, sp[0], sp[1], sp[2], c->min_intron_length };
+    s->sh.cand_prm = cp; s->sh.fact_prm = fp;
+    boot.n_lane = (int)env_size("PINTRON_PRE_LANES", ok ? 4 : 1);
+    if (boot.n_lane > PRE_LANES_MAX) boot.n_lane = PRE_LANES_MAX;
+    if (getenv("PINTRON_NO_PREFETCH")) boot.n_lane = 0;
+    s->sh.n_pre_lanes = boot.n_lane;
+  }
   pthread_t boot_thread;
   const bool booting = pthread_create(&boot_thread, NULL, gpu_boot_main, &boot) == 0;
   ef_parse_threads = (int)env_size("PINTRON_PARSE_THREADS", host_core_share());
@@ -1049,7 +1130,8 @@
     if (kept.fibers && kept.stack_size == stack_size) { s->sh.fiber_pool = kept.fibers; kept.fibers = NULL; }
     s->sh.spare_chunks = kept.chunks; kept.chunks = NULL;
     s->sh.pre_slab = kept.pre_slab; s->sh.pre_slab_cap = kept.pre_slab_cap; kept.pre_slab = NULL; kept.pre_slab_cap = 0;
-    s->sh.up_stage = kept.up_stage; s->sh.up_stage_cap = kept.up_stage_cap; kept.up_stage = NULL; kept.up_stage_cap = 0;
+    for (int k = 0; k < PRE_LANES_MAX; ++k) { s->sh.up_stage[k] = kept.up_stage[k]; s->sh.up_stage_cap[k] = kept.up_stage_cap[k]; kept.up_stage[k] = NULL; kept.up_stage_cap[k] = 0; }
+    for (int k = 0; k < PRE_CHUNKS; ++k) { s->sh.pre_fblk[k] = kept.fblk[k]; s->sh.pre_fblk_cap[k] = kept.fblk_cap[k]; kept.fblk[k] = NULL; kept.fblk_cap[k] = 0; }
     pthread_mutex_unlock(&kept.mu);
     for (fiber* f = s->sh.fiber_pool; f; f = f->pool_next) ++kept_fibers;
   }
@@ -1069,6 +1151,7 @@
   const double t_booted = now_s();
   if (boot.rc == PGPU_OK) { s->ctx0 = boot.ctx; s->sh.idx = boot.idx_rc == PGPU_OK ? boot.idx : NULL; }
   for (int k = 0; k < boot.n_svc; ++k) s->sh.svc.threads[k].ctx = boot.svc[k];
+  for (int k = 0; k < boot.n_lane; ++k) s->lane_ctx[k] = boot.lane[k];
   if (load_rc != 0) { ef_session_close(s); return NULL; }
   if (boot.rc != PGPU_OK) {
     fprintf(stderr, "* FATAL no usable MI355X (gfx950) device / libpintron_gpu.so: est-fact has no CPU fallback\n");
@@ -1131,7 +1214,7 @@
   sh->svc.n_threads = boot.n_svc;
   sh->svc.coalesce_us = getenv("PINTRON_COALESCE_US") ? atol(getenv("PINTRON_COALESCE_US")) : 0;
   if (boot.svc_rc != PGPU_OK) {
-    fprintf(stderr, "* FATAL the GPU contexts of the service threads could not be created\n");
+    fprintf(stderr, "* FATAL the GPU contexts of the service threads and prefetch lanes could not be created\n");
     ef_session_close(s); return NULL;
   }
   if (getenv("PINTRON_VERBOSE"))
@@ -1146,6 +1229,7 @@
   {
     const char* gm = getenv("PINTRON_GPU_MEG");
     sh->use_meg = !(gm && gm[0] == '0' && gm[1] == '\0');
+    if (!sh->use_meg || !sh->n_pre) sh->use_fact = false;
     const ef_config* c = &in->cfg;
     const pgpu_meg_params mp = { c->min_factor_len, c->min_intron_length, c->max_intron_length, c->max_pairings_in_MEG,
                                  c->max_prefix_discarded_rate, c->max_suffix_discarded_rate, c->max_freq_shortest_pairing,
@@ -1174,12 +1258,26 @@
   if (release) while (sh->spare_chunks) { out_chunk* nx = sh->spare_chunks->next; free(sh->spare_chunks); sh->spare_chunks = nx; }
 }
 
-typedef struct { ef_session* s; int c; uint64_t* off; size_t total; char* blob; bool own_blob; int rc; pthread_t th; bool started; } stage_job;
+static void* pinned_alloc(ef_session* s, size_t bytes) {
+  void* q = NULL;
+  pthread_mutex_lock(&s->sh.alloc_mu);
+  if (pgpu_host_alloc(s->ctx0, bytes, &q) != PGPU_OK) q = NULL;
+  pthread_mutex_unlock(&s->sh.alloc_mu);
+  return q;
+}
+static void pinned_free(ef_session* s, void* q) {
+  if (!q) return;
+  pthread_mutex_lock(&s->sh.alloc_mu);
+  pgpu_host_free(s->ctx0, q);
+  pthread_mutex_unlock(&s->sh.alloc_mu);
+}
+typedef struct { ef_session* s; int c, lane; uint64_t* off; size_t total; char* blob; bool own_blob; int rc; pthread_t th; bool started; } stage_job;
 static void* stage_main(void* arg) {
   stage_job* j = (stage_job*)arg;
   ef_session* s = j->s;
   shared* sh = &s->sh;
   ef_inputs* in = &s->in;
+  char** up_stage = &sh->up_stage[j->lane]; size_t* up_stage_cap = &sh->up_stage_cap[j->lane];
   const size_t lo = sh->pre_lo[j->c], hi = sh->pre_lo[j->c + 1];
   j->rc = PGPU_OK; j->blob = NULL; j->own_blob = false;
   j->off = (uint64_t*)malloc((hi - lo + 1) * sizeof(uint64_t));
@@ -1188,22 +1286,22 @@
   for (size_t k = lo; k < hi; ++k) { j->off[k - lo] = total; total += strlen(in->list[k]->seq); }
   j->off[hi - lo] = total;
   j->total = total;
-  if (total + 1 > sh->up_stage_cap) {
-    if (sh->up_stage) pgpu_host_free(s->ctx0, sh->up_stage);
-    sh->up_stage = NULL; sh->up_stage_cap = 0;
-    void* q = NULL;
+  if (total + 1 > *up_stage_cap) {
+    pinned_free(s, *up_stage);
+    *up_stage = NULL; *up_stage_cap = 0;
     const size_t want = total + total / 4 + 4096;
-    if (pgpu_host_alloc(s->ctx0, want, &q) == PGPU_OK) { sh->up_stage = (char*)q; sh->up_stage_cap = want; }
-  }
-  j->blob = sh->up_stage ? sh->up_stage : (char*)malloc(total + 1);
-  j->own_blob = j->blob != sh->up_stage;
+    void* q = pinned_alloc(s, want);
+    if (q) { *up_stage = (char*)q; *up_stage_cap = want; }
+  }
+  j->blob = *up_stage ? *up_stage : (char*)malloc(total + 1);
+  j->own_blob = j->blob != *up_stage;
   if (!j->blob) { j->rc = PGPU_ENOMEM; return NULL; }
   for (size_t k = lo; k < hi; ++k) memcpy(j->blob + j->off[k - lo], in->list[k]->seq, (size_t)(j->off[k - lo + 1] - j->off[k - lo]));
   return NULL;
 }
-static void stage_start(stage_job* j, ef_session* s, int c) {
+static void stage_start(stage_job* j, ef_session* s, int c, int lane) {
   memset(j, 0, sizeof *j);
-  j->s = s; j->c = c;
+  j->s = s; j->c = c; j->lane = lane;
   j->started = pthread_create(&j->th, NULL, stage_main, j) == 0;
   if (!j->started) stage_main(j);
 }
@@ -1213,7 +1311,7 @@
   int prc = j->rc;
   if (prc == PGPU_OK) {
     const size_t lo = s->sh.pre_lo[j->c], hi = s->sh.pre_lo[j->c + 1];
-    prc = pgpu_pairing_plan_create_resident(s->ctx0, s->sh.idx, j->blob, j->off, hi - lo, &s->pplan[j->c]);
+    prc = pgpu_pairing_plan_create_resident(s->lane_ctx[j->lane], s->sh.idx, j->blob, j->off, hi - lo, &s->pplan[j->c]);
   }
   if (j->own_blob) free(j->blob);
   free(j->off);
@@ -1221,36 +1319,56 @@
   return prc;
 }
 
+static bool fact_block(ef_session* s, int c, size_t entries, size_t exons) {
+  shared* sh = &s->sh;
+  const size_t have = sh->pre_fblk[c] && sh->pre_fblk_cap[c] >= 32 * entries ? (sh->pre_fblk_cap[c] - 32 * entries) / 33 : 0;
+  if (!sh->pre_fblk[c] || sh->pre_fblk_cap[c] < 32 * entries || have < exons) {
+    pinned_free(s, sh->pre_fblk[c]);
+    const size_t cap = exons + exons / 4 + 256;
+    sh->pre_fblk_cap[c] = 32 * entries + 33 * cap;
+    sh->pre_fblk[c] = (unsigned char*)pinned_alloc(s, sh->pre_fblk_cap[c]);
+    if (!sh->pre_fblk[c]) { sh->pre_fblk_cap[c] = 0; return false; }
+  }
+  sh->pre_fexons_cap[c] = (sh->pre_fblk_cap[c] - 32 * entries) / 33;
+  return true;
+}
+
 static void* prefetch_main(void* arg) {
   pthread_setname_np(pthread_self(), "ef-pairings");
-  ef_session* s = (ef_session*)arg;
+  struct pre_lane* pl = (struct pre_lane*)arg;
+  ef_session* s = pl->s;
   shared* sh = &s->sh;
+  pgpu_ctx* const ctx = s->lane_ctx[pl->k];
+  const int n_lanes = sh->n_pre_lanes;
   pgpu_pairing_params prm = { s->in.cfg.min_factor_len, 0, s->in.cfg.min_string_depth_rate };
   stage_job stage; bool staging = false;
   memset(&stage, 0, sizeof stage);
-  for (int c = 0; c < sh->n_pre; ++c) {
-    char rname[48];
-    snprintf(rname, sizeof rname, "prefetch chunk %d (pairings + MEGs)", c);
+  double kernel_ms[6] = { 0, 0, 0, 0, 0, 0 }, meg_ms = 0, fact_ms[4] = { 0, 0, 0, 0 };
+  for (int c = pl->k; c < sh->n_pre; c += n_lanes) {
+    if (__atomic_load_n(&sh->failed, __ATOMIC_RELAXED)) break;
+    char rname[64];
+    snprintf(rname, sizeof rname, "prefetch chunk %d (pairings + MEGs + factorizations)", c);
     pgpu_range_push(rname);
     const double tc0 = now_s();
     int prc = PGPU_OK;
     if (!s->pplan[c]) {
-      if (!staging) { stage_start(&stage, s, c); staging = true; }
+      if (!staging) { stage_start(&stage, s, c, pl->k); staging = true; }
       prc = stage_finish(&stage);
       staging = false;
-      if (prc == PGPU_OK && c + 1 < sh->n_pre && !s->pplan[c + 1]) { stage_start(&stage, s, c + 1); staging = true; }
+      if (prc == PGPU_OK && c + n_lanes < sh->n_pre && !s->pplan[c + n_lanes]) { stage_start(&stage, s, c + n_lanes, pl->k); staging = true; }
     }
     const double tc1 = now_s();
-    if (prc == PGPU_OK) prc = pgpu_pairing_plan_run(s->ctx0, s->pplan[c], &prm);
+    if (prc == PGPU_OK) prc = pgpu_pairing_plan_run(ctx, s->pplan[c], &prm);
     const double tc2 = now_s();
     bool have_meg = false;
     if (prc == PGPU_OK && sh->use_meg) {
-      const int mrc = pgpu_pairing_plan_run_meg(s->ctx0, s->pplan[c], &sh->meg_prm);
-      if (mrc == PGPU_ENOSYS) sh->use_meg = false;
+      const int mrc = pgpu_pairing_plan_run_meg(ctx, s->pplan[c], &sh->meg_prm);
+      if (mrc == PGPU_ENOSYS) { sh->use_meg = false; sh->use_fact = false; }
       else if (mrc != PGPU_OK) prc = mrc;
       else {
         const size_t bytes = (size_t)pgpu_pairing_plan_meg_bytes(s->pplan[c]);
         const size_t entries = sh->pre_lo[c + 1] - sh->pre_lo[c];
+        pthread_mutex_lock(&sh->alloc_mu);
         if (!sh->pre_slab && c == 1 && sh->n_pre > 2) {
           const size_t per = (bytes + bytes / 4 + 4096 + (entries + 2) * sizeof(uint64_t) + 511) & ~(size_t)511;
           void* q = NULL;
@@ -1275,25 +1393,57 @@
             if (pgpu_host_alloc(s->ctx0, (entries + 1) * sizeof(uint64_t), &q) == PGPU_OK) { sh->pre_meg_first[c] = (uint64_t*)q; sh->pre_first_own[c] = true; }
           }
         }
+        pthread_mutex_unlock(&sh->alloc_mu);
         if (!sh->pre_meg[c] || !sh->pre_meg_first[c]) prc = PGPU_ENOMEM;
-        else prc = pgpu_pairing_plan_fetch_meg(s->ctx0, s->pplan[c], sh->pre_meg[c], sh->pre_meg_cap[c], sh->pre_meg_first[c]);
+        else prc = pgpu_pairing_plan_fetch_meg(ctx, s->pplan[c], sh->pre_meg[c], sh->pre_meg_cap[c], sh->pre_meg_first[c]);
         have_meg = prc == PGPU_OK;
-        s->pre_meg_ms += pgpu_pairing_plan_meg_ms(s->pplan[c]);
+        meg_ms += pgpu_pairing_plan_meg_ms(s->pplan[c]);
+      }
+    }
+    const double tc3 = now_s();
+    if (prc == PGPU_OK && have_meg && sh->use_fact) {
+      int frc = fact_entries_present() ? pgpu_pairing_plan_run_candidates(ctx, s->pplan[c], &sh->cand_prm) : PGPU_ENOSYS;
+      if (frc == PGPU_OK) frc = pgpu_pairing_plan_run_factorizations(ctx, s->pplan[c], &sh->fact_prm);
+      if (frc == PGPU_ENOSYS) sh->use_fact = false;
+      else if (frc != PGPU_OK) prc = frc;
+      else {
+        const size_t entries = sh->pre_lo[c + 1] - sh->pre_lo[c];
+        const size_t ce = (size_t)pgpu_pairing_plan_candidate_exons(s->pplan[c]), fe = (size_t)pgpu_pairing_plan_factorization_exons(s->pplan[c]);
+        if (!fact_block(s, c, entries, ce > fe ? ce : fe)) prc = PGPU_ENOMEM;
+        else {
+          const size_t cap = sh->pre_fexons_cap[c];
+          pgpu_cand_result* cand = (pgpu_cand_result*)sh->pre_fblk[c];
+          pgpu_fact_result* fact = (pgpu_fact_result*)(sh->pre_fblk[c] + 16 * entries);
+          pgpu_factor* fexons = (pgpu_factor*)(sh->pre_fblk[c] + 32 * entries);
+          pgpu_factor* cexons = fexons + cap;
+          uint8_t* steps = (uint8_t*)(cexons + cap);
+          prc = pgpu_pairing_plan_fetch_candidates(ctx, s->pplan[c], cand, cexons, cap);
+          if (prc == PGPU_OK) prc = pgpu_pairing_plan_fetch_factorizations(ctx, s->pplan[c], fact, fexons, steps, cap);
+          if (prc == PGPU_OK) { sh->pre_cand[c] = cand; sh->pre_fact[c] = fact; sh->pre_fexons[c] = fexons; }
+          fact_ms[0] += pgpu_pairing_plan_candidates_ms(s->pplan[c]);
+          for (int k = 1; k < 4; ++k) fact_ms[k] += pgpu_pairing_plan_factorizations_ms(s->pplan[c], k);
+        }
       }
     }
     if (prc == PGPU_OK && !have_meg) {
       const size_t cnt = (size_t)pgpu_pairing_plan_count(s->pplan[c]);
       sh->pre_tri[c] = (pgpu_pairing*)malloc((cnt + 1) * sizeof(pgpu_pairing));
       sh->pre_first[c] = (uint64_t*)malloc((sh->pre_lo[c + 1] - sh->pre_lo[c] + 1) * sizeof(uint64_t));
-      prc = pgpu_pairing_plan_fetch(s->ctx0, s->pplan[c], sh->pre_tri[c], cnt, sh->pre_first[c]);
-    }
-    for (int k = 0; k < 6; ++k) s->pre_kernel_ms[k] += pgpu_pairing_plan_kernel_ms(s->pplan[c], k);
+      prc = pgpu_pairing_plan_fetch(ctx, s->pplan[c], sh->pre_tri[c], cnt, sh->pre_first[c]);
+    }
+    for (int k = 0; k < 6; ++k) kernel_ms[k] += pgpu_pairing_plan_kernel_ms(s->pplan[c], k);
     if (getenv("PINTRON_VERBOSE") && atoi(getenv("PINTRON_VERBOSE")) >= 2)
-      fprintf(stderr, "* prefetch chunk %d: at %.3fs of the step; plan + upload %.1f ms, pairings %.1f ms, MEGs + download %.1f ms\n", c,
-              tc0 - s->pre_t0, 1e3 * (tc1 - tc0), 1e3 * (tc2 - tc1), 1e3 * (now_s() - tc2));
+      fprintf(stderr, "* prefetch chunk %d (lane %d): at %.3fs of the step; plan + upload %.1f ms, pairings %.1f ms, MEGs + download %.1f ms, "
+                      "factorizations + download %.1f ms\n", c, pl->k,
+              tc0 - s->pre_t0, 1e3 * (tc1 - tc0), 1e3 * (tc2 - tc1), 1e3 * (tc3 - tc2), 1e3 * (now_s() - tc3));
     pthread_mutex_lock(&sh->mu);
-    if (prc != PGPU_OK) { fprintf(stderr, "* FATAL pairing prefetch failed: %s\n", pgpu_last_error(s->ctx0)); sh->failed = 1; }
-    else __atomic_store_n(&sh->ready_entries, sh->pre_lo[c + 1], __ATOMIC_RELEASE);
+    if (prc != PGPU_OK) { fprintf(stderr, "* FATAL pairing prefetch failed: %s\n", pgpu_last_error(ctx)); sh->failed = 1; }
+    else {
+      sh->pre_done[c] = true;
+      int upto = 0;
+      while (upto < sh->n_pre && sh->pre_done[upto]) ++upto;
+      if (sh->pre_lo[upto] > sh->ready_entries) __atomic_store_n(&sh->ready_entries, sh->pre_lo[upto], __ATOMIC_RELEASE);
+    }
     pthread_cond_broadcast(&sh->ready_cv);
     pthread_mutex_unlock(&sh->mu);
     pgpu_range_pop();
@@ -1304,7 +1454,13 @@
     if (stage.own_blob) free(stage.blob);
     free(stage.off);
   }
-  s->pre_wall = now_s() - s->pre_t0;
+  pthread_mutex_lock(&sh->mu);
+  for (int k = 0; k < 6; ++k) s->pre_kernel_ms[k] += kernel_ms[k];
+  s->pre_meg_ms += meg_ms;
+  for (int k = 0; k < 4; ++k) sh->fact_kernel_ms[k] += fact_ms[k];
+  { const double wall = now_s() - s->pre_t0; if (wall > s->pre_wall) s->pre_wall = wall; }
+  pthread_mutex_unlock(&sh->mu);
+  ef_cell_release_all();
   return NULL;
 }
 
@@ -1334,11 +1490,15 @@
   memset(s->pre_kernel_ms, 0, sizeof s->pre_kernel_ms);
   s->pre_meg_ms = 0;
   s->pre_t0 = t0; s->pre_wall = 0;
-  bool pre_started = false;
-  if (sh->n_pre) {
-    pre_started = pthread_create(&s->pre_thread, NULL, prefetch_main, s) == 0;
-    if (!pre_started) prefetch_main(s);
-  }
+  memset(sh->pre_done, 0, sizeof sh->pre_done);
+  memset(sh->fact_kernel_ms, 0, sizeof sh->fact_kernel_ms); memset(sh->fact_answers, 0, sizeof sh->fact_answers);
+  for (int c = 0; c < PRE_CHUNKS; ++c) { sh->pre_cand[c] = NULL; sh->pre_fact[c] = NULL; sh->pre_fexons[c] = NULL; }
+  if (sh->n_pre)
+    for (int k = 0; k < sh->n_pre_lanes; ++k) {
+      s->pre_lane[k].s = s; s->pre_lane[k].k = k;
+      s->pre_lane[k].started = pthread_create(&s->pre_lane[k].th, NULL, prefetch_main, &s->pre_lane[k]) == 0;
+      if (!s->pre_lane[k].started) prefetch_main(&s->pre_lane[k]);
+    }
   const double t1 = now_s();
   service* sv = &sh->svc;
   sv->stop = false; sv->head = sv->tail = NULL; sv->sh = sh;
@@ -1380,7 +1540,8 @@
     fprintf(stderr, "\n");
     fprintf(stderr, "*   %-14s %8.4f s  %6.2f  %6.2f\n", "all but sleeps", tot, (double)ts / (double)sh->n_units, (double)tj / (double)sh->n_units);
   }
-  if (pre_started) pthread_join(s->pre_thread, NULL);
+  if (sh->n_pre)
+    for (int k = 0; k < sh->n_pre_lanes; ++k) if (s->pre_lane[k].started) { pthread_join(s->pre_lane[k].th, NULL); s->pre_lane[k].started = false; }
   pthread_mutex_lock(&sv->mu); sv->stop = true; pthread_cond_broadcast(&sv->posted); pthread_mutex_unlock(&sv->mu);
   for (int k = 0; k < sv_started; ++k) pthread_join(sv->threads[k].thread, NULL);
   ef_sched_stats st;
@@ -1443,12 +1604,24 @@
       ks.algo_bytes = pairs * 12ull + rec;
       kstat_add(&st, &ks);
     }
+    static const char* fnm[4] = { "cand", "clean", "gaps", "chain" };
+    for (int k = 0; k < 4; ++k)
+      if (sh->fact_kernel_ms[k] > 0) {
+        ef_kernel_stat ks; memset(&ks, 0, sizeof ks);
+        snprintf(ks.name, sizeof ks.name, "%s", fnm[k]);
+        ks.ms = sh->fact_kernel_ms[k]; ks.launches = (size_t)sh->n_pre; ks.jobs = s->in.n;
+        kstat_add(&st, &ks);
+      }
   }
   { size_t su = 0; for (size_t t = 0; t < w_started; ++t) su += ws[t].suspensions; st.suspensions_per_unit = sh->n_units ? (double)su / (double)sh->n_units : 0.0; }
   st.load_s = s->load_s; st.index_s = s->index_s; st.prefetch_s = s->pre_wall; st.workers_s = now_s() - t1;
   for (size_t u = 0; u < sh->n_units; ++u) if (sh->units[u].len[1]) ++st.aligned;
   if (stats_out) *stats_out = st;
   ef_dp_trace_flush();
+  if (fact_log) fflush(fact_log);
+  if (getenv("PINTRON_VERBOSE"))
+    fprintf(stderr, "* device factorizations served: %llu DONE, %llu EMPTY, %llu HOST (stage %s, %d prefetch lanes, %d ranges)\n",
+            sh->fact_answers[2], sh->fact_answers[1], sh->fact_answers[0], sh->use_fact ? "on" : "off", sh->n_pre_lanes, sh->n_pre);
   pgpu_range_pop();
   ef_info_mark("est-processing-end");
   free(ws); free(th);
@@ -1573,6 +1746,9 @@
 char* ef_session_records(ef_session* s, size_t* len) { return ef_session_output(s, 0, len); }
 
 size_t ef_session_n_ests(const ef_session* s) { return s->sh.n_units; }
+void ef_session_fact_answers(const ef_session* s, unsigned long long out[3]) {
+  for (int k = 0; k < 3; ++k) out[k] = s->sh.fact_answers[k];
+}
 struct pgpu_ctx* ef_session_context(ef_session* s) { return s->ctx0; }
 const void* ef_session_genomic(ef_session* s) { return s->in.gen; }
 
@@ -1630,20 +1806,25 @@
     free(sh->pre_tri[c]); free(sh->pre_first[c]);
     if (sh->pre_meg[c] && sh->pre_own[c]) pgpu_host_free(s->ctx0, sh->pre_meg[c]);
     if (sh->pre_meg_first[c] && sh->pre_first_own[c]) pgpu_host_free(s->ctx0, sh->pre_meg_first[c]);
-    if (s->pplan[c]) pgpu_pairing_plan_destroy(s->ctx0, s->pplan[c]);
+    if (s->pplan[c]) pgpu_pairing_plan_destroy(s->lane_ctx[c % sh->n_pre_lanes], s->pplan[c]);
   }
   if (keep_on() && s->ctx0) {
     pthread_mutex_lock(&kept.mu);
     if (sh->pre_slab && !kept.pre_slab) { kept.pre_slab = sh->pre_slab; kept.pre_slab_cap = sh->pre_slab_cap; sh->pre_slab = NULL; }
-    if (sh->up_stage && !kept.up_stage) { kept.up_stage = sh->up_stage; kept.up_stage_cap = sh->up_stage_cap; sh->up_stage = NULL; }
+    for (int k = 0; k < PRE_LANES_MAX; ++k)
+      if (sh->up_stage[k] && !kept.up_stage[k]) { kept.up_stage[k] = sh->up_stage[k]; kept.up_stage_cap[k] = sh->up_stage_cap[k]; sh->up_stage[k] = NULL; }
+    for (int c = 0; c < PRE_CHUNKS; ++c)
+      if (sh->pre_fblk[c] && !kept.fblk[c]) { kept.fblk[c] = sh->pre_fblk[c]; kept.fblk_cap[c] = sh->pre_fblk_cap[c]; sh->pre_fblk[c] = NULL; }
     pthread_mutex_unlock(&kept.mu);
   }
   tq[2] = now_s();
   if (sh->pre_slab) pgpu_host_free(s->ctx0, sh->pre_slab);
-  if (sh->up_stage) pgpu_host_free(s->ctx0, sh->up_stage);
+  for (int k = 0; k < PRE_LANES_MAX && s->ctx0; ++k) if (sh->up_stage[k]) pgpu_host_free(s->ctx0, sh->up_stage[k]);
+  for (int c = 0; c < PRE_CHUNKS && s->ctx0; ++c) if (sh->pre_fblk[c]) pgpu_host_free(s->ctx0, sh->pre_fblk[c]);
   if (s->ctx0 && sh->idx) pgpu_index_destroy(s->ctx0, sh->idx);
   tq[3] = now_s();
   for (int k = 0; k < MAX_SERVICES; ++k) ctx_give(sh->svc.threads[k].ctx, s->device);
+  for (int k = 0; k < PRE_LANES_MAX; ++k) ctx_give(s->lane_ctx[k], s->device);
   ctx_give(s->ctx0, s->device);
   tq[4] = now_s();
   ef_free_inputs(&s->in);
@@ -1651,7 +1832,10 @@
   if (verbose)
     fprintf(stderr, "* close: unit buffers + fibres %.3fs, pairing plans %.3fs, index + slabs %.3fs, contexts %.3fs, inputs %.3fs\n",
             tq[1] - tq[0], tq[2] - tq[1], tq[3] - tq[2], tq[4] - tq[3], tq[5] - tq[4]);
-  pthread_mutex_destroy(&sh->mu); pthread_cond_destroy(&sh->ready_cv);
+  pthread_mutex_lock(&fact_log_mu);
+  if (fact_log) { fclose(fact_log); fact_log = NULL; }
+  pthread_mutex_unlock(&fact_log_mu);
+  pthread_mutex_destroy(&sh->mu); pthread_cond_destroy(&sh->ready_cv); pthread_mutex_destroy(&sh->alloc_mu);
   pthread_mutex_destroy(&sh->svc.mu); pthread_cond_destroy(&sh->svc.posted); pthread_cond_destroy(&sh->svc.finished);
   free(s);
   if (--open_sessions == 0) restore_affinity();
diff --git a/pintron_amd/host/ef_sched.h b/pintron_amd/host/ef_sched.h
--- a/pintron_amd/host/ef_sched.h
+++ b/pintron_amd/host/ef_sched.h
@@ -27,6 +27,7 @@
 char* ef_session_records(ef_session* s, size_t* len);
 char* ef_session_output(ef_session* s, int which, size_t* len);
 size_t ef_session_n_ests(const ef_session* s);
+void ef_session_fact_answers(const ef_session* s, unsigned long long out[3]);
 void ef_session_close(ef_session* s);
 
 int ef_main_multi(int argc, char** argv);
diff --git a/pintron_amd/host/estfact.h b/pintron_amd/host/estfact.h
--- a/pintron_amd/host/estfact.h
+++ b/pintron_amd/host/estfact.h
@@ -196,7 +196,9 @@
        EFP_NS_PREFIX, EFP_NS_BETWEEN_ASK, EFP_NS_BETWEEN_CLASS, EFP_NS_BETWEEN_SEARCH, EFP_TMP1, EFP_TMP2, EFP_TMP3, EFP_N };
 extern int ef_prof_on;
 typedef struct { unsigned long long cyc[EFP_N], susp[EFP_N], jobs[EFP_N]; unsigned long long last; int dummy; int* cur;
-                 unsigned long long ahead_hits, ahead_misses, ahead_asked, chain_graphs, other_graphs; } ef_prof_state;
+                 unsigned long long ahead_hits, ahead_misses, ahead_asked, chain_graphs, other_graphs;
+                 unsigned long long fact_answers[3];
+               } ef_prof_state;
 extern _Thread_local ef_prof_state ef_prof;
 static inline unsigned long long ef_prof_now(void) {
 #if defined(__x86_64__)
@@ -246,6 +248,9 @@
 } ef_ahead;
 static inline void ef_ahead_init(ef_ahead* ah) { ah->n = ah->n_pending = 0; ah->collecting = false; memset(ah->slot, 0, sizeof ah->slot); }
 
+typedef struct ef_fact_answer { unsigned outcome, work, n_exons; const int32_t* exons; } ef_fact_answer;
+enum { EF_FACT_HOST = 0, EF_FACT_EMPTY = 1, EF_FACT_DONE = 2 };
+
 typedef struct ef_backend {
   void* self;
   int (*pairings)(void* self, const char* pattern, size_t m, unsigned min_factor_len, double rate,
@@ -253,6 +258,7 @@
   int (*dp)(void* self, const ef_dp_req* req, ef_dp_res* res);
   int (*dp_many)(void* self, const ef_dp_req* reqs, ef_dp_res* res, size_t n);
   const void* (*meg)(void* self, const char* pattern, size_t m, const ef_config* cfg);
+  int (*fact)(void* self, const char* pattern, const ef_config* cfg, struct ef_fact_answer* out);
   ef_ahead* ahead;
 } ef_backend;
 
```
